# jluttine/junction-tree

Hardware: AMD Instinct MI355X
Metric: clique-potential GB/s (algorithmic bytes per propagate / time; messages/sec alongside), synthetic width-20 tree (higher is better)
Workload: dtype f32; 1 GPU; BASELINE.json configs[3]: 256 cliques, width 20, cardinality 2 (2^20-entry f32 potentials), 10 shared variables per edge, balanced binary tree; evidence_sets_per_rank=1, multiset=False, parallelism=1 GPU, launch_mode=flow, idle_plans=0, library=jtprop 0.6.0 (gfx950, HIP, RCCL p2p) src:c327fe1ab271

## Files before the change

include/jtprop.h:

```cpp
#ifndef JTPROP_H
#define JTPROP_H

#include <stddef.h>
#include <stdint.h>

#ifdef __cplusplus
extern "C" {
#endif

#define JTP_OK 0
#define JTP_EINVAL (-1)
#define JTP_EHIP (-2)
#define JTP_ECOMM (-3)
#define JTP_ENOMEM (-4)
#define JTP_EUNSUPPORTED (-5)

#define JTP_F32 0
#define JTP_F64 1

#define JTP_PLAN_ONLY 1u
#define JTP_KEEP_ROOT 4u
#define JTP_SPLIT_VARIANTS 2u

#define JTP_LEVEL_LAUNCHES 8u

#define JTP_FLOW_TICKETS 16u

#define JTP_SHARE_POTENTIALS 32u

#define JTP_MULTISET 64u

#define JTP_NO_COMPACT 128u

typedef struct jtp_plan jtp_plan;

typedef struct jtp_tree_desc {
    int32_t struct_size;
    int32_t n_vars;
    const int32_t *var_card;
    int32_t n_cliques;
    int32_t n_nodes;
    const int32_t *node_var_off;
    const int32_t *node_var_ids;
    const int32_t *parent_clique;
    const int32_t *parent_sep;
    int32_t dtype;
    int32_t device;
    int32_t n_batch;
    int32_t n_ranks;
    int32_t rank;
    const int32_t *clique_owner;
    uint32_t flags;
    int32_t lds_budget;
    int32_t block_log2;
    int32_t layout_policy;
    const int32_t *cover_off;
    const int32_t *cover_ids;
    int32_t fold_n;
    int32_t fold_pad;
    const int32_t *fold_cliques;
    const int32_t *fold_var_off;
    const int32_t *fold_var_ids;
} jtp_tree_desc;

typedef struct jtp_stats {
    int32_t struct_size;
    int32_t n_launches;
    int32_t n_messages;
    int32_t n_tasks;
    double  algorithmic_bytes;
    double  collect_ms;
    double  distribute_ms;
    double  kernel_ms[32];
    double  kernel_bytes[32];
    int32_t kernel_launches[32];
    int32_t flow_fallbacks;
    int32_t launch_mode;
    int32_t tickets_used;
    int32_t flow_propagates;
    double  device_bytes;
    int32_t storage_dtype;
    int32_t foreign_seen;
    double  f64_flops;
    double  f64_insts;
    double  algorithmic_bytes_full;
    double  fixed_bytes;
    int32_t n_unit_cliques;
    int32_t n_static_tables;
    int32_t flight_board;
    int32_t lean_refused;
} jtp_stats;


int jtp_plan_create(const jtp_tree_desc *desc, jtp_plan **out);
void jtp_plan_destroy(jtp_plan *plan);

const char *jtp_plan_describe(jtp_plan *plan);


int jtp_set_potential(jtp_plan *plan, int32_t batch, int32_t node, const void *host,
                      const int64_t *shape, int32_t host_dtype);

typedef struct jtp_factor {
    const void *host;
    int32_t n_vars;
    int32_t dtype;
    const int32_t *var_ids;
    const int64_t *shape;
} jtp_factor;

int jtp_set_potential_product(jtp_plan *plan, int32_t batch, int32_t clique, int32_t n_factors,
                              const jtp_factor *factors);

int jtp_set_potential_products(jtp_plan *plan, int32_t batch, int32_t n_cliques, const int32_t *cliques,
                               const int32_t *factor_off, const jtp_factor *factors);

int jtp_fill_synthetic(jtp_plan *plan, int32_t batch, uint64_t seed, const double *scale);

int jtp_set_evidence(jtp_plan *plan, int32_t batch, int32_t n, const int32_t *var_ids, const int32_t *states);


int jtp_propagate(jtp_plan *plan, int32_t batch_begin, int32_t batch_end);
int jtp_sync(jtp_plan *plan);


int jtp_get_belief(jtp_plan *plan, int32_t batch, int32_t node, void *host, int32_t host_dtype);

int jtp_get_marginal(jtp_plan *plan, int32_t batch, int32_t clique, const int32_t *out_vars,
                     int32_t n_out, double *host);

int jtp_get_marginals(jtp_plan *plan, int32_t batch, int32_t n, const int32_t *cliques,
                      const int32_t *var_off, const int32_t *var_ids, const int64_t *out_off,
                      double *host);

int jtp_get_z(jtp_plan *plan, int32_t batch, double *z);


int jtp_set_profiling(jtp_plan *plan, int32_t keep);
int jtp_set_profiling_granularity(jtp_plan *plan, int32_t per_launch);
int jtp_set_profiling_stride(jtp_plan *plan, int32_t stride);
int jtp_region_begin(jtp_plan *plan);
int jtp_region_end(jtp_plan *plan, double *ms);
int jtp_get_stats(jtp_plan *plan, jtp_stats *stats);
int jtp_get_launch_ms(jtp_plan *plan, double *ms, int32_t n);
int jtp_debug_read_msg(jtp_plan *plan, int32_t batch, int64_t off, int64_t n, double *host);
int jtp_debug_set(jtp_plan *plan, const char *knob, int64_t value);
const char *jtp_kernel_name(int32_t variant);


int jtp_comm_unique_id(void *id128);
int jtp_comm_init(int32_t rank, int32_t n_ranks, const void *id128, int32_t device);
int jtp_comm_destroy(void);
int jtp_comm_info(int32_t *n_ranks, int32_t *rank, int32_t *device);
int jtp_comm_selftest(int32_t n);


int jtp_device_count(int32_t *count);
int jtp_device_memory(int32_t device, uint64_t *free_bytes, uint64_t *total_bytes);

int jtp_host_alloc(void **ptr, size_t bytes);
int jtp_host_free(void *ptr);
const char *jtp_last_error(void);
const char *jtp_version(void);

#ifdef __cplusplus
}
#endif
#endif
```

junction-tree_amd/build.py:

```python
import os
import subprocess
import sys

HERE = os.path.dirname(os.path.abspath(__file__))
CSRC = os.path.join(HERE, "csrc")
LIBDIR = os.path.join(HERE, "junctiontree_amd", "lib")
LIB = os.path.join(LIBDIR, "libjtprop.so")
INST = ["jtp_inst_%s_%s.hip" % (fam, t) for fam in ("both", "bothm", "level", "mixc", "mix", "flow", "multi", "shape") for t in ("f32", "f64")]
SOURCES = ["jtp_plan.cpp", "jtp_engine.hip"] + INST
DEPS = SOURCES + ["jtp_internal.h", "jtp_plan.h", "jtp_kernels.hip.h", os.path.join("..", "..", "include", "jtprop.h")]


ID_FILE = os.path.join(LIBDIR, "BUILD_ID")


def source_id():
    import hashlib
    h = hashlib.sha256()
    for d in sorted(DEPS):
        with open(os.path.join(CSRC, d), "rb") as fh:
            h.update(d.encode() + b"\0" + fh.read())
    return h.hexdigest()[:12]


def built_id():
    try:
        with open(ID_FILE) as fh:
            return fh.read().split()[0].split("+")[0]
    except (OSError, IndexError):
        return None


def needs_build():
    if not os.path.exists(LIB):
        return True
    try:
        return built_id() != source_id()
    except OSError:
        return False


def build(force=False, verbose=True, extra=(), out=None, jobs=None):
    out = out or LIB
    if out == LIB and extra:
        raise SystemExit("experimental flags (%s) build to --out, not onto the product library" % " ".join(extra))
    if out == LIB and not force and not needs_build():
        return LIB
    from concurrent.futures import ThreadPoolExecutor
    import shutil
    import tempfile
    os.makedirs(LIBDIR, exist_ok=True)
    hipcc = os.environ.get("HIPCC", "/opt/rocm/bin/hipcc")
    sid = source_id() + ("+" + "".join(sorted(extra)).replace(" ", "") if extra else "")
    flags = ["-O3", "-std=c++17", "--offload-arch=gfx950", "-fPIC", "-Wall", "-Wno-unused-function", "-Wno-unused-variable",
             '-DJTP_SOURCE_ID="%s"' % sid] + list(extra)
    objdir = tempfile.mkdtemp(prefix="jtprop_build_")
    cache = os.path.join(LIBDIR, "objcache")
    os.makedirs(cache, exist_ok=True)
    import hashlib
    headers = {"jtp_plan.cpp": ["jtp_plan.h", "jtp_internal.h", os.path.join("..", "..", "include", "jtprop.h")],
               "jtp_engine.hip": ["jtp_plan.h", "jtp_internal.h", "jtp_kernels.hip.h", os.path.join("..", "..", "include", "jtprop.h")]}
    try:
        toolchain = subprocess.check_output([hipcc, "--version"], stderr=subprocess.STDOUT)
    except (OSError, subprocess.CalledProcessError):
        toolchain = hipcc.encode()
    try:
        def compile_one(src):
            obj = os.path.join(objdir, os.path.splitext(src)[0] + ".o")
            h = hashlib.sha256()
            h.update(toolchain)
            for d in [src] + headers.get(src, ["jtp_internal.h", "jtp_kernels.hip.h"]):
                with open(os.path.join(CSRC, d), "rb") as fh:
                    h.update(d.encode() + b"\0" + fh.read())
            tu_flags = [f for f in flags if not f.startswith("-DJTP_SOURCE_ID") or src == "jtp_engine.hip"]
            h.update(" ".join(tu_flags).encode())
            kept = os.path.join(cache, os.path.splitext(src)[0] + "." + h.hexdigest()[:16] + ".o")
            if os.path.exists(kept):
                shutil.copy(kept, obj)
                return obj
            cmd = [hipcc] + tu_flags + ["-c", os.path.join(CSRC, src), "-o", obj]
            if verbose:
                print(" ".join(cmd), flush=True)
            subprocess.check_call(cmd)
            mine = sorted((f for f in os.listdir(cache) if f.startswith(os.path.splitext(src)[0] + ".") and f.endswith(".o")),
                          key=lambda f: os.path.getmtime(os.path.join(cache, f)))
            for old in mine[:-3]:
                os.remove(os.path.join(cache, old))
            tmp_kept = kept + ".tmp%d" % os.getpid()
            shutil.copy(obj, tmp_kept)
            os.replace(tmp_kept, kept)
            return obj
# ... 34 lines not shown
```

junction-tree_amd/csrc/jtp_engine.hip:

```cpp
#include <dlfcn.h>
#include <fcntl.h>
#include <hip/hip_runtime.h>
#include <signal.h>
#include <sys/mman.h>
#include <sys/stat.h>
#include <unistd.h>

#include <cerrno>

#include <algorithm>
#include <atomic>
#include <cstdarg>
#include <cstdio>
#include <cstring>
#include <map>
#include <mutex>
#include <string>
#include <vector>

#include "jtp_kernels.hip.h"
#include "jtp_plan.h"


static thread_local std::string g_err;
// ... 74 lines not shown
typedef int (*Pop_t)(void);
static Push_t Push = nullptr;
static Pop_t Pop = nullptr;
static int state = 0;
static void load() {
    if (state != 0) return;
    state = -1;
    for (const char *n : {"librocprofiler-sdk-roctx.so.1", "librocprofiler-sdk-roctx.so", "libroctx64.so.4", "libroctx64.so"}) {
        void *h = dlopen(n, RTLD_NOW | RTLD_LOCAL);
        if (!h) continue;
        Push = (Push_t)dlsym(h, "roctxRangePushA");
        Pop = (Pop_t)dlsym(h, "roctxRangePop");
        if (Push && Pop) {
            state = 1;
            return;
        }
    }
}
struct Range {
    bool on;
    Range(bool enabled, const char *name) : on(enabled && state == 1) { if (on) Push(name); }
    ~Range() { if (on) Pop(); }
};
}

#define NCCL_TRY(expr)                                                                          \
    do {                                                                                        \
        int _r = (expr);                                                                        \
        if (_r != rccl::ncclSuccess)                                                            \
            return set_err(JTP_ECOMM, "%s failed: %s", #expr, rccl::GetErrorString(_r));         \
    } while (0)



static inline int mixk(const HostPlan &hp) { return hp.tmix ? (hp.tmix_compact ? 2 : 1) : 0; }

static bool flow_both() {
    static const bool on = !(getenv("JTP_FLOW_BOTH") && atoi(getenv("JTP_FLOW_BOTH")) == 0);
    return on;
}

template <typename T>
struct KernelTable {
    typedef void (*fn)(const JtTask *, const JtBlock *, const int *, const T *, T *, double *, JtFlow);
    static fn get(int variant, int tmix) {
        if (tmix == 2) {
            if (variant >= JT_K_COLLECT0 && variant <= JT_K_COLLECT3) return jt_collect_level_mix<T, true>;
            if (variant >= JT_K_DIST_P0C0 && variant <= JT_K_DIST_P1C3) return jt_distribute_level_mix<T, true>;
            if (variant == JT_K_COLLECT_LEVEL) return jt_collect_level_mix<T, true>;
            if (variant == JT_K_DISTRIBUTE_LEVEL) return jt_distribute_level_mix<T, true>;
            if (variant == JT_K_SINGLE || variant == JT_K_MARGINALS) return jt_single_mix<T, true>;
        }
        if (tmix) {
            if (variant >= JT_K_COLLECT0 && variant <= JT_K_COLLECT3) return jt_collect_level_mix<T, false>;
            if (variant >= JT_K_DIST_P0C0 && variant <= JT_K_DIST_P1C3) return jt_distribute_level_mix<T, false>;
            if (variant == JT_K_COLLECT_LEVEL) return jt_collect_level_mix<T, false>;
            if (variant == JT_K_DISTRIBUTE_LEVEL) return jt_distribute_level_mix<T, false>;
            if (variant == JT_K_SINGLE || variant == JT_K_MARGINALS) return jt_single_mix<T, false>;
        }
        switch (variant) {
            case JT_K_COLLECT0: return jt_collect<T, 0>;
            case JT_K_COLLECT1: return jt_collect<T, 1>;
            case JT_K_COLLECT2: return jt_collect<T, 2>;
            case JT_K_COLLECT3: return jt_collect<T, 3>;
            case JT_K_DIST_P0C0: return jt_distribute<T, 0, 0>;
            case JT_K_DIST_P0C1: return jt_distribute<T, 0, 1>;
            case JT_K_DIST_P0C2: return jt_distribute<T, 0, 2>;
            case JT_K_DIST_P0C3: return jt_distribute<T, 0, 3>;
            case JT_K_DIST_P1C0: return jt_distribute<T, 1, 0>;
            case JT_K_DIST_P1C1: return jt_distribute<T, 1, 1>;
            case JT_K_DIST_P1C2: return jt_distribute<T, 1, 2>;
            case JT_K_DIST_P1C3: return jt_distribute<T, 1, 3>;
            case JT_K_COLLECT_LEVEL: return jt_collect_level<T>;
            case JT_K_DISTRIBUTE_LEVEL: return jt_distribute_level<T>;
            case JT_K_REDUCE_LEVEL: return jt_reduce_level<T>;
            case JT_K_MULTI_COLLECT: return jt_multi_flow<T>;
            case JT_K_MULTI_DISTRIBUTE: return jt_multi_flow<T>;
            case JT_K_SINGLE: return jt_single<T>;
            case JT_K_MARGINALS: return jt_marginals<T>;
            case JT_K_LEAN_SINGLE: return jt_lean_single<T>;
        }
        return nullptr;
    }
    static fn get_flow(int phase, bool chain, int tmix, bool marg) {
        if (tmix == 2) return phase == 0 ? jt_collect_flow_mix<T, true> : jt_distribute_flow_mix<T, true>;
        if (tmix) return phase == 0 ? jt_collect_flow_mix<T, false> : jt_distribute_flow_mix<T, false>;
        if (phase == 2) return marg ? jt_propagate_flow_marg<T> : jt_propagate_flow<T>;
        if (phase == 1 && !chain && flow_both()) return marg ? jt_propagate_flow_marg<T> : jt_propagate_flow<T>;
        return phase == 0 ? jt_collect_flow<T> : (chain ? jt_distribute_flow_chain<T> : jt_distribute_flow<T>);
    }
};

static const char *k_names[JT_K_COUNT] = {
    "jt_collect<T, 0>", "jt_collect<T, 1>", "jt_collect<T, 2>", "jt_collect<T, 3>",
    "jt_distribute<T, 0, 0>", "jt_distribute<T, 0, 1>", "jt_distribute<T, 0, 2>", "jt_distribute<T, 0, 3>",
    "jt_distribute<T, 1, 0>", "jt_distribute<T, 1, 1>", "jt_distribute<T, 1, 2>", "jt_distribute<T, 1, 3>",
    "jt_collect_level<T>", "jt_distribute_level<T>", "jt_collect_flow<T>", "jt_distribute_flow<T>", "jt_reduce_level<T>",
    "jt_multi_flow<T>", "jt_multi_flow<T>", "jt_single<T>", "jt_propagate_flow<T>", "jt_marginals<T>", "jt_lean_single<T>",
};

struct BatchBuffers {
    void *psi = nullptr;
    void *bel = nullptr;
    double *msg = nullptr;
    double *fix = nullptr;
    uint32_t *ev = nullptr;
    bool ev_any = false;
    uint32_t *sync = nullptr;
    uint32_t epoch = 0;
    uint32_t flow_runs = 0;
    uint32_t ticket_runs = 0;
    bool unchecked = false;
    int64_t cur_off(int64_t half) const { return (epoch & 1u) ? half : 0; }
    int64_t fix_shift(int64_t cur) const { return fix ? (int64_t)(((intptr_t)fix - (intptr_t)msg) / 8) - cur : 0; }
};

struct MargBatch {
    int lean_nblocks = 0, lean_lds = 0;
    bool folded = false;
    JtMargDesc *d_descs_fold = nullptr;
    std::vector<JtTask> h_tasks;
    std::vector<int32_t> key;
    JtTask *d_tasks = nullptr;
    JtBlock *d_blocks = nullptr;
    int *d_itab = nullptr;
    JtMargDesc *d_descs = nullptr;
    double *scratch = nullptr, *stage = nullptr;
    int n = 0, nblocks = 0, lds = 0, max_grid_x = 1;
    int unit_nblocks = 0, unit_lds = 0;
    int64_t total_out = 0;
    std::vector<int64_t> elems;
    void release() {
        if (d_tasks) (void)hipFree(d_tasks);
        if (d_blocks) (void)hipFree(d_blocks);
        if (d_itab) (void)hipFree(d_itab);
        if (d_descs) (void)hipFree(d_descs);
        if (d_descs_fold) (void)hipFree(d_descs_fold);
        if (scratch) (void)hipFree(scratch);
        if (stage) (void)hipFree(stage);
    }
};

static std::atomic<int> g_inflight[64];

static std::map<std::pair<int, const void *>, int> g_lds_raised;
static std::mutex g_lds_mutex;
static hipError_t raise_lds(const void *func, int bytes) {
    if (bytes <= 64 * 1024) return hipSuccess;
    int dev = 0;
    hipError_t e = hipGetDevice(&dev);
    if (e != hipSuccess) return e;
    std::lock_guard<std::mutex> lock(g_lds_mutex);
    int &have = g_lds_raised[std::make_pair(dev, func)];
    if (have >= bytes) return hipSuccess;
    e = hipFuncSetAttribute(func, hipFuncAttributeMaxDynamicSharedMemorySize, bytes);
    if (e == hipSuccess) have = bytes;
    return e;
}

struct jtp_plan {
    HostPlan hp;
    bool device = false;
    bool widened = false;
    bool inflight = false;
    int launch_mode = 0;
    int tickets_used = 0;
    int foreign_seen = 0;
// ... 218 lines not shown
int jtp_device_memory(int32_t device, uint64_t *free_bytes, uint64_t *total_bytes) {
    size_t f = 0, t = 0;
    int before = 0;
    HIP_TRY(hipGetDevice(&before));
    HIP_TRY(hipSetDevice(device));
    const hipError_t e = hipMemGetInfo(&f, &t);
    (void)hipSetDevice(before);
    if (e != hipSuccess) return set_err(JTP_EHIP, "hipMemGetInfo failed: %s", hipGetErrorString(e));
    if (free_bytes) *free_bytes = f;
    if (total_bytes) *total_bytes = t;
    return JTP_OK;
}

const char *jtp_kernel_name(int32_t variant) {
    if (variant < 0 || variant >= JT_K_COUNT) return nullptr;
    return k_names[variant];
}


void jtp_plan_destroy(jtp_plan *pl) {
    if (!pl) return;
    if (pl->device) {
        (void)hipSetDevice(pl->hp.device);
        for (auto s : pl->streams) (void)hipStreamSynchronize(s);
        if (pl->inflight) {
            pl->inflight = false;
            (void)board::publish(pl->hp.device, --g_inflight[pl->hp.device & 63]);
        }
        if (pl->multiset) {
            if (!pl->bufs.empty()) {
                if (pl->bufs[0].psi) (void)hipFree(pl->bufs[0].psi);
                if (pl->bufs[0].bel) (void)hipFree(pl->bufs[0].bel);
            }
            if (pl->msg_all) (void)hipFree(pl->msg_all);
            if (pl->d_member) (void)hipFree(pl->d_member);
            if (pl->d_esum_oct) (void)hipFree(pl->d_esum_oct);
            if (pl->d_act_ids) (void)hipFree(pl->d_act_ids);
            if (pl->d_act_n) (void)hipFree(pl->d_act_n);
            if (pl->d_fanout) (void)hipFree(pl->d_fanout);
            if (pl->ev_all) (void)hipFree(pl->ev_all);
            if (pl->sync_all) (void)hipFree(pl->sync_all);
        } else
        for (auto &b : pl->bufs) {
            if (b.psi && (&b == &pl->bufs[0] || b.psi != pl->bufs[0].psi)) (void)hipFree(b.psi);
            if (b.bel) (void)hipFree(b.bel);
            if (b.msg) (void)hipFree(b.msg);
            if (b.fix && (&b == &pl->bufs[0] || b.fix != pl->bufs[0].fix)) (void)hipFree(b.fix);
            if (b.ev) (void)hipFree(b.ev);
            if (b.sync) (void)hipFree(b.sync);
        }
        if (pl->host_abort) (void)hipHostFree(pl->host_abort);
        for (auto &bt : pl->belief_tasks) {
            if (bt.d_task) (void)hipFree(bt.d_task);
            if (bt.d_blk) (void)hipFree(bt.d_blk);
            if (bt.d_tab) (void)hipFree(bt.d_tab);
        }
        for (MargBatch *mb : pl->marg_cache) {
            mb->release();
            delete mb;
        }
        if (pl->d_tasks) (void)hipFree(pl->d_tasks);
        if (pl->d_blocks) (void)hipFree(pl->d_blocks);
        for (int m = 0; m < 2; ++m)
            if (pl->d_init[m]) (void)hipFree(pl->d_init[m]);
        if (pl->d_itab) (void)hipFree(pl->d_itab);
        if (pl->stage) (void)hipFree(pl->stage);
        for (int i = 0; i < 2; ++i) {
            if (pl->up_stage[i]) (void)hipFree(pl->up_stage[i]);
            if (pl->up_ev[i]) (void)hipEventDestroy(pl->up_ev[i]);
        }
        if (pl->eval_stage) (void)hipFree(pl->eval_stage);
        if (pl->eval_host) (void)hipHostFree(pl->eval_host);
        if (pl->unit_scratch) (void)hipFree(pl->unit_scratch);
        for (auto e : pl->ev) (void)hipEventDestroy(e);
        for (auto e : pl->region_ev)
            if (e) (void)hipEventDestroy(e);
        for (auto s : pl->streams) (void)hipStreamDestroy(s);
    }
    delete pl;
}

static int zero_padding(jtp_plan *pl, double *msg, int nsets, hipStream_t s, int halves = 3);

int jtp_plan_create(const jtp_tree_desc *desc, jtp_plan **out) {
    if (!out) return set_err(JTP_EINVAL, "null output pointer");
    *out = nullptr;
    jtp_plan *pl = new jtp_plan();
    std::string err;
    int rc = jtp_build_plan(desc, pl->hp, err);
    for (int attempt = 1; attempt < 4 && rc == JTP_EUNSUPPORTED && desc; ++attempt) {
        jtp_tree_desc again = *desc;
        const bool relayout = (attempt & 1) && (desc->flags & JTP_MULTISET) && desc->layout_policy == 0;
        const bool pad = (attempt & 2) && !(desc->flags & JTP_NO_COMPACT);
        if (!relayout && !pad) continue;
        if ((attempt & 1) && !relayout) continue;
        if ((attempt & 2) && !pad) continue;
        if (relayout) again.layout_policy = 2;
        if (pad) again.flags |= JTP_NO_COMPACT;
        std::string err2;
        delete pl;
        pl = new jtp_plan();
        const int rc2 = jtp_build_plan(&again, pl->hp, err2);
        if (rc2 == JTP_OK) rc = rc2;
        else if (rc2 != JTP_EUNSUPPORTED) rc = rc2, err = err2;
    }
    if (rc == JTP_EUNSUPPORTED && desc && desc->dtype == JTP_F32 && !(desc->flags & JTP_MULTISET)) {
        for (int attempt = 0; attempt < 2 && rc == JTP_EUNSUPPORTED; ++attempt) {
            jtp_tree_desc again = *desc;
            again.dtype = JTP_F64;
            if (attempt == 1) {
                if (desc->flags & JTP_NO_COMPACT) break;
                again.flags |= JTP_NO_COMPACT;
            }
            std::string err2;
            delete pl;
            pl = new jtp_plan();
            const int rc2 = jtp_build_plan(&again, pl->hp, err2);
            if (rc2 == JTP_OK) rc = rc2, pl->widened = true;
            else if (rc2 != JTP_EUNSUPPORTED) rc = rc2, err = err2;
        }
    }
    if (rc == JTP_EUNSUPPORTED && desc && desc->cover_off && !(desc->flags & JTP_MULTISET)) {
        jtp_tree_desc again = *desc;
        again.cover_off = again.cover_ids = nullptr;
        jtp_plan *fresh = nullptr;
        const int rc2 = jtp_plan_create(&again, &fresh);
        delete pl;
        if (rc2 == JTP_OK) {
            fresh->hp.lean_refused = err.empty() ? std::string("unsupported") : err;
            *out = fresh;
        }
        return rc2;
    }
    if (rc != JTP_OK) {
        delete pl;
        return set_err(rc, "%s", err.c_str());
    }
    HostPlan &hp = pl->hp;
    pl->esize = hp.dtype == JTP_F32 ? 4 : 8;
    pl->multiset = hp.multiset;
    if (pl->multiset && !(hp.flags & JTP_SHARE_POTENTIALS)) {
        delete pl;
        return set_err(JTP_EINVAL, "JTP_MULTISET needs JTP_SHARE_POTENTIALS (the evidence sets of a group read one table)");
    }
    pl->flow = !(hp.flags & (JTP_LEVEL_LAUNCHES | JTP_SPLIT_VARIANTS)) && !(hp.knobs.debug & 1) && !hp.knobs.force_level_launches;
    if (hp.max_lds > 64 * 1024 && !pl->multiset && !hp.knobs.force_flow) pl->flow = false;
    pl->chain = hp.chain_plan;
    for (const HostPlan::FoldReq &fr : hp.folded) pl->marg_tasks = pl->marg_tasks || fr.task >= 0;
    if (hp.flags & JTP_PLAN_ONLY) {
        *out = pl;
        return JTP_OK;
    }
    pl->fake_comm = hp.n_ranks > 1 ? hp.knobs.fake_comm : 0;
    if (pl->fake_comm == 2 && (!rccl::comm || rccl::comm_size != 1)) {
        delete pl;
        return set_err(JTP_ECOMM, "JTP_FAKE_COMM=2 (exchange steps as RCCL groups in loop-back) needs a communicator of ONE rank: jtp_comm_init(0, 1, ...)");
    }
    if (hp.n_ranks > 1 && !pl->fake_comm && (!rccl::comm || rccl::comm_size != hp.n_ranks || rccl::comm_rank != hp.rank)) {
        delete pl;
        return set_err(JTP_ECOMM, "n_ranks=%d but jtp_comm_init was not called with a matching communicator", hp.n_ranks);
    }
    int ndev = 0;
    hipError_t e = hipGetDeviceCount(&ndev);
    if (e != hipSuccess || ndev <= 0) {
        delete pl;
        return set_err(JTP_EHIP, "no HIP device available (%s); libjtprop has no CPU fallback",
                       e != hipSuccess ? hipGetErrorString(e) : "device count is 0");
    }
#define CREATE_TRY(expr)                                                                                 \
    do {                                                                                                 \
        hipError_t _e = (expr);                                                                          \
        if (_e != hipSuccess) {                                                                          \
            set_err(_e == hipErrorOutOfMemory ? JTP_ENOMEM : JTP_EHIP, "%s failed: %s", #expr, hipGetErrorString(_e)); \
            jtp_plan_destroy(pl);                                                                        \
            return _e == hipErrorOutOfMemory ? JTP_ENOMEM : JTP_EHIP;                                    \
        }                                                                                                \
    } while (0)
    pl->device = true;
    pl->flow_debug = hp.knobs.flow_debug;
    pl->env_tickets = hp.knobs.flow_tickets != 0;
    pl->roctx = hp.knobs.roctx != 0;
    if (pl->roctx) roctx::load();
    CREATE_TRY(hipSetDevice(hp.device));
    const int nstreams = pl->multiset ? 1 : std::min(hp.n_batch, 16);
    pl->streams.resize(nstreams);
    for (auto &s : pl->streams) CREATE_TRY(hipStreamCreateWithFlags(&s, hipStreamNonBlocking));
    pl->bufs.resize(hp.n_batch);
    const size_t abytes = (size_t)std::max<int64_t>(hp.arena_elems, 256) * pl->esize;
    const size_t mbytes = (size_t)std::max<int64_t>(hp.msg_doubles, 2) * 8 * 2;
    const bool share_psi = (hp.flags & JTP_SHARE_POTENTIALS) != 0;
    if (pl->multiset) {
        const bool ef = hp.knobs.no_ef_share == 0 && ((hp.n_batch + JT_MSETS - 1) / JT_MSETS >= 8 || hp.knobs.no_ef_share < 0);
        pl->set0 = ef ? JT_MSETS : 0;
        pl->n_groups = (hp.n_batch + JT_MSETS - 1) / JT_MSETS + (pl->set0 ? 1 : 0);
        const size_t nsets = (size_t)pl->n_groups * JT_MSETS;
        pl->set_stride = (int64_t)(mbytes / 8);
        pl->ev_stride = (uint32_t)(2 * hp.pn.size());
        void *psi = nullptr, *bel = nullptr;
        CREATE_TRY(hipMalloc(&psi, abytes));
        pl->bufs[0].psi = psi;
        CREATE_TRY(hipMalloc(&bel, abytes));
        pl->bufs[0].bel = bel;
        CREATE_TRY(hipMemsetAsync(psi, 0, abytes, pl->streams[0]));
        CREATE_TRY(hipMemsetAsync(bel, 0, abytes, pl->streams[0]));
        CREATE_TRY(hipMalloc((void **)&pl->msg_all, mbytes * nsets));
        CREATE_TRY(hipMemsetD32Async((hipDeviceptr_t)pl->msg_all, (int)(uint32_t)(JT_UNWRITTEN & 0xffffffffu), mbytes * nsets / 4, pl->streams[0]));
        CREATE_TRY(hipMalloc((void **)&pl->ev_all, (size_t)pl->ev_stride * 4 * nsets));
        CREATE_TRY(hipMemsetAsync(pl->ev_all, 0, (size_t)pl->ev_stride * 4 * nsets, pl->streams[0]));
        CREATE_TRY(hipMalloc((void **)&pl->sync_all, (size_t)hp.sync_words * 4 * pl->n_groups));
        CREATE_TRY(hipMemsetAsync(pl->sync_all, 0, (size_t)hp.sync_words * 4 * pl->n_groups, pl->streams[0]));
        for (int b = 0; b < hp.n_batch; ++b) {
            BatchBuffers &bb = pl->bufs[b];
            bb.psi = psi;
            bb.bel = bel;
            bb.msg = pl->msg_all + (int64_t)(pl->set0 + b) * pl->set_stride;
            bb.ev = pl->ev_all + (size_t)(pl->set0 + b) * pl->ev_stride;
            bb.sync = pl->sync_all + (size_t)((pl->set0 + b) / JT_MSETS) * hp.sync_words;
        }
        pl->belief_tasks.resize(hp.pn.size());
        if (pl->set0) {
            const size_t cap = (size_t)pl->n_groups * JT_MSETS, nt = hp.tasks.size();
            CREATE_TRY(hipMalloc((void **)&pl->d_member, nt * cap));
            CREATE_TRY(hipMalloc((void **)&pl->d_act_ids, nt * cap * sizeof(uint16_t)));
            CREATE_TRY(hipMalloc((void **)&pl->d_act_n, nt * sizeof(int32_t)));
            CREATE_TRY(hipMalloc((void **)&pl->d_esum_oct, nt * (size_t)pl->n_groups));
            pl->act_dirty = true;
        }
    } else
    for (auto &b : pl->bufs) {
        if (share_psi && &b != &pl->bufs[0]) b.psi = pl->bufs[0].psi;
        else CREATE_TRY(hipMalloc(&b.psi, abytes));
        CREATE_TRY(hipMalloc(&b.bel, abytes));
        CREATE_TRY(hipMalloc((void **)&b.msg, mbytes));
        if (hp.fix_doubles > 0) {
            if (share_psi && &b != &pl->bufs[0]) b.fix = pl->bufs[0].fix;
            else {
                CREATE_TRY(hipMalloc((void **)&b.fix, (size_t)hp.fix_doubles * 8));
                CREATE_TRY(hipMemsetAsync(b.fix, 0, (size_t)hp.fix_doubles * 8, pl->streams[0]));
            }
        }
        CREATE_TRY(hipMemsetAsync(b.psi, 0, abytes, pl->streams[0]));
        CREATE_TRY(hipMemsetAsync(b.bel, 0, abytes, pl->streams[0]));
        CREATE_TRY(hipMemsetD32Async((hipDeviceptr_t)b.msg, (int)(uint32_t)(JT_UNWRITTEN & 0xffffffffu), mbytes / 4, pl->streams[0]));
        CREATE_TRY(hipMalloc((void **)&b.sync, (size_t)hp.sync_words * 4));
        CREATE_TRY(hipMemsetAsync(b.sync, 0, (size_t)hp.sync_words * 4, pl->streams[0]));
    }
    CREATE_TRY(hipHostMalloc((void **)&pl->host_abort, 64, hipHostMallocMapped));
    *pl->host_abort = 0;

    for (auto &b : pl->bufs) {
        if (&b != &pl->bufs[0] && b.psi == pl->bufs[0].psi) continue;
        for (const VirtualFill &vf : hp.virtual_fills) {
            const int64_t n = vf.d.phys_elems;
            const int grid = (int)std::min<int64_t>((n + 255) / 256, 4096);
            if (hp.dtype == JTP_F32) hipLaunchKernelGGL((jt_pack<float, float, 2>), dim3(grid), dim3(256), 0, pl->streams[0], vf.d, (const float *)nullptr, (float *)b.psi, 0ull, 1.0);
            else hipLaunchKernelGGL((jt_pack<double, double, 2>), dim3(grid), dim3(256), 0, pl->streams[0], vf.d, (const double *)nullptr, (double *)b.psi, 0ull, 1.0);
        }
        CREATE_TRY(hipGetLastError());
    }
    if (pl->multiset) {
        pl->ev_host.assign((size_t)pl->ev_stride * pl->n_groups * JT_MSETS, 0u);
        for (JtTask &tk : hp.tasks)
            if (tk.esum & 1) tk.esum |= 2, tk.esum_groups = ~0ull;
    }
    if (!hp.tasks.empty()) {
        CREATE_TRY(hipMalloc((void **)&pl->d_tasks, hp.tasks.size() * sizeof(JtTask)));
        CREATE_TRY(hipMemcpy(pl->d_tasks, hp.tasks.data(), hp.tasks.size() * sizeof(JtTask), hipMemcpyHostToDevice));
    }
    if (!hp.blocks.empty()) {
        CREATE_TRY(hipMalloc((void **)&pl->d_blocks, hp.blocks.size() * sizeof(JtBlock)));
        CREATE_TRY(hipMemcpy(pl->d_blocks, hp.blocks.data(), hp.blocks.size() * sizeof(JtBlock), hipMemcpyHostToDevice));
    }
    if (!hp.itab.empty()) {
        CREATE_TRY(hipMalloc((void **)&pl->d_itab, hp.itab.size() * sizeof(int32_t)));
        CREATE_TRY(hipMemcpy(pl->d_itab, hp.itab.data(), hp.itab.size() * sizeof(int32_t), hipMemcpyHostToDevice));
    }
    for (int m = 0; m < 2; ++m)
        if (!hp.init_blocks[m].empty()) {
            CREATE_TRY(hipMalloc((void **)&pl->d_init[m], hp.init_blocks[m].size() * sizeof(JtBlock)));
            CREATE_TRY(hipMemcpy(pl->d_init[m], hp.init_blocks[m].data(), hp.init_blocks[m].size() * sizeof(JtBlock), hipMemcpyHostToDevice));
        }
    auto kfunc = [&](int v) { return hp.dtype == JTP_F32 ? (const void *)KernelTable<float>::get(v, mixk(hp)) : (const void *)KernelTable<double>::get(v, mixk(hp)); };
    if (pl->multiset) {
        CREATE_TRY(raise_lds(kfunc(JT_K_MULTI_COLLECT), JT_RING_BYTES + JT_MSETS * (JT_MSETS > 8 ? JT_SETB_SMALL : JT_SETB_LARGE)));
    } else if (hp.max_lds > 64 * 1024) {
        for (int v = 0; v < JT_K_COUNT; ++v) {
            if (kfunc(v) == nullptr) continue;
            CREATE_TRY(raise_lds(kfunc(v), hp.max_lds));
        }
        for (int ph = 0; ph < 3; ++ph) {
            const void *f = hp.dtype == JTP_F32 ? (const void *)KernelTable<float>::get_flow(ph, pl->chain, mixk(hp), pl->marg_tasks) : (const void *)KernelTable<double>::get_flow(ph, pl->chain, mixk(hp), pl->marg_tasks);
            CREATE_TRY(raise_lds(f, hp.max_lds));
        }
    }
    {
        double b = 0;
        if (pl->multiset) {
            const size_t nsets = (size_t)pl->n_groups * JT_MSETS;
            b = 2.0 * abytes + (double)mbytes * nsets + (double)pl->ev_stride * 4 * nsets + (double)hp.sync_words * 4 * pl->n_groups;
        } else {
            const size_t npsi = share_psi ? 1 : pl->bufs.size();
            b = (double)abytes * (npsi + pl->bufs.size()) + ((double)mbytes + (double)hp.sync_words * 4) * pl->bufs.size() + (double)hp.fix_doubles * 8 * npsi;
        }
        b += (double)hp.tasks.size() * sizeof(JtTask) + (double)hp.blocks.size() * sizeof(JtBlock) + (double)hp.itab.size() * 4;
        pl->device_bytes = b;
    }
    if (pl->multiset) {
        if (int rc = zero_padding(pl, pl->msg_all, pl->n_groups * JT_MSETS, pl->streams[0])) {
            jtp_plan_destroy(pl);
            return rc;
        }
    } else
        for (auto &b : pl->bufs)
            if (int rc = zero_padding(pl, b.msg, 1, pl->streams[0])) {
                jtp_plan_destroy(pl);
                return rc;
            }
    CREATE_TRY(hipStreamSynchronize(pl->streams[0]));
#undef CREATE_TRY
    *out = pl;
    return JTP_OK;
}

const char *jtp_plan_describe(jtp_plan *pl) {
    if (!pl) return "";
    if (pl->hp.json.empty()) jtp_plan_to_json(pl->hp, pl->hp.tasks.size() <= 20000);
    return pl->hp.json.c_str();
}


static int check_writable(jtp_plan *pl, int batch) {
    if ((pl->hp.flags & JTP_SHARE_POTENTIALS) && batch != 0)
        return set_err(JTP_EINVAL, "the plan shares its potentials between evidence sets: set them through evidence set 0");
    return JTP_OK;
}

static int check_ready(jtp_plan *pl, int batch) {
    if (!pl) return set_err(JTP_EINVAL, "null plan");
    if (!pl->device) return set_err(JTP_EHIP, "plan was created with JTP_PLAN_ONLY: no device work possible");
    if (batch < 0 || batch >= pl->hp.n_batch) return set_err(JTP_EINVAL, "batch %d out of range [0,%d)", batch, pl->hp.n_batch);
    return JTP_OK;
}

int jtp_set_potential(jtp_plan *pl, int32_t batch, int32_t node, const void *host, const int64_t *shape,
                      int32_t host_dtype) {
    int rc = check_ready(pl, batch);
    if (rc) return rc;
    rc = check_writable(pl, batch);
    if (rc) return rc;
    pl->psi_dirty = true;
    HostPlan &hp = pl->hp;
    if (node < 0 || node >= hp.n_cliques) return set_err(JTP_EINVAL, "node %d is not a clique", node);
    if (!(hp.pn[node].owner == hp.rank || hp.pn[node].owner == hp.n_ranks)) return set_err(JTP_EINVAL, "clique %d belongs to rank %d", node, hp.pn[node].owner);
    if (host_dtype != JTP_F32 && host_dtype != JTP_F64) return set_err(JTP_EINVAL, "bad host dtype");
    const bool unit = hp.pn[node].unit;
    if (unit && hp.pn[node].stat < 0) {
        bool one = true;
        for (size_t i = 0; i < hp.node_vars[node].size(); ++i) one = one && (!shape || shape[i] == 1 || hp.card[hp.node_vars[node][i]] == 1);
        if (!shape) for (int v : hp.node_vars[node]) one = one && hp.card[v] == 1;
        const double v = !host ? 0.0 : (host_dtype == JTP_F32 ? (double)*(const float *)host : *(const double *)host);
        if (!one || v != 1.0)
            return set_err(JTP_EINVAL, "clique %d was described as depending on none of its variables (jtp_tree_desc.cover_*): its potential is 1", node);
        return JTP_OK;
    }
    JtPackDesc d = unit ? hp.stat_pack[node] : hp.pack[node];
    int64_t stride = 1;
    for (int i = d.nvars - 1; i >= 0; --i) {
        const int64_t len = shape ? shape[i] : d.card[i];
        if (len != d.card[i] && len != 1) {
            if (unit && len == hp.card[hp.node_vars[node][i]])
                return set_err(JTP_EINVAL, "clique %d axis %d has length %lld, but the clique was described as not depending on that variable (jtp_tree_desc.cover_*)", node, i, (long long)len);
            return set_err(JTP_EINVAL, "clique %d axis %d has length %lld, expected %d or 1", node, i, (long long)len, d.card[i]);
        }
        d.hstride[i] = (len == 1) ? 0 : stride;
        stride *= len;
    }
    const size_t hbytes = (size_t)stride * (host_dtype == JTP_F32 ? 4 : 8);
    HIP_TRY(hipSetDevice(hp.device));
    const int ui = (int)(pl->up_cursor++ & 1u);
    if (!pl->up_ev[ui]) HIP_TRY(hipEventCreateWithFlags(&pl->up_ev[ui], hipEventDisableTiming));
    if (pl->up_busy[ui]) {
        HIP_TRY(hipEventSynchronize(pl->up_ev[ui]));
        pl->up_busy[ui] = false;
    }
    if (pl->up_bytes[ui] < hbytes) {
        if (pl->up_stage[ui]) HIP_TRY(hipFree(pl->up_stage[ui]));
        pl->up_stage[ui] = nullptr;
        pl->up_bytes[ui] = 0;
        HIP_TRY(hipMalloc(&pl->up_stage[ui], std::max<size_t>(hbytes, 256)));
        pl->up_bytes[ui] = std::max<size_t>(hbytes, 256);
    }
    void *stage = pl->up_stage[ui];
    hipStream_t s = pl->streams[batch % pl->streams.size()];
    HIP_TRY(hipMemcpyAsync(stage, host, hbytes, hipMemcpyHostToDevice, s));
    BatchBuffers &b = pl->bufs[batch];
    if (unit) {
        if (host_dtype == JTP_F32) launch_pack<double, float>(d, (const float *)stage, b.fix, s);
        else launch_pack<double, double>(d, (const double *)stage, b.fix, s);
    } else if (hp.dtype == JTP_F32) {
        if (host_dtype == JTP_F32) launch_pack<float, float>(d, (const float *)stage, (float *)b.psi, s);
        else launch_pack<float, double>(d, (const double *)stage, (float *)b.psi, s);
    } else {
        if (host_dtype == JTP_F32) launch_pack<double, float>(d, (const float *)stage, (double *)b.psi, s);
        else launch_pack<double, double>(d, (const double *)stage, (double *)b.psi, s);
    }
    HIP_TRY(hipGetLastError());
    HIP_TRY(hipEventRecord(pl->up_ev[ui], s));
    pl->up_busy[ui] = true;
    return JTP_OK;
}

// ... 588 lines not shown
                hipLaunchKernelGGL(jt_multi_flow<float>, dim3(grid), dim3(JT_THREADS), lds, s, pl->d_tasks, pl->d_blocks + blk_off,
                                   pl->d_itab, (const float *)b0.psi, (float *)b0.bel, pl->msg_all, fl);
            else
                hipLaunchKernelGGL(jt_multi_flow<double>, dim3(grid), dim3(JT_THREADS), lds, s, pl->d_tasks, pl->d_blocks + blk_off,
                                   pl->d_itab, (const double *)b0.psi, (double *)b0.bel, pl->msg_all, fl);
        };
        for (const Step &st : (flow ? hp.flow_steps : hp.steps)) {
            if (st.kind != 0) continue;
            const int phase = flow ? hp.segments[st.first].phase : hp.launches[st.first].phase;
            if (prof && !mid_done && phase == 1) {
                HIP_TRY(hipEventRecord(pl->ev[ev_base + 1], s));
                mid_done = true;
            }
            if (flow) {
                const Segment &sg = hp.segments[st.first];
                int lds = 0;
                for (int i = sg.first_launch; i < sg.first_launch + sg.n_launch; ++i) lds = std::max(lds, multiset_lds(hp, hp.launches[i]));
                launch(sg.phase, sg.blk_off, sg.nblocks, lds, tickets ? sg.ticket_idx : -1, ticket_run * (uint32_t)sg.nblocks);
            } else {
                const Launch &L = hp.launches[st.first];
                launch(L.phase, L.blk_off, L.nblocks, multiset_lds(hp, L), -1, 0u);
            }
        }
        if (prof) {
            if (!mid_done) HIP_TRY(hipEventRecord(pl->ev[ev_base + 1], s));
            HIP_TRY(hipEventRecord(pl->ev[ev_base + 2], s));
            pl->prof_cursor++;
        }
        HIP_TRY(hipGetLastError());
        return JTP_OK;
    }
    const bool prof = pl->prof_steps > 0 && (pl->prof_calls++ % (unsigned)pl->prof_stride) == 0;
    const size_t ev_per_step = pl->prof_per_launch ? 2 * hp.launches.size() : 3;
    if (prof) {
        size_t need = ev_per_step * (size_t)pl->prof_steps;
        while (pl->ev.size() < need) {
            hipEvent_t e;
            HIP_TRY(hipEventCreate(&e));
            pl->ev.push_back(e);
        }
    }
    const size_t ev_base = prof ? ev_per_step * (size_t)(pl->prof_cursor % pl->prof_steps) : 0;
    for (int b = batch_begin; b < batch_end; ++b) {
        hipStream_t s = pl->streams[b % pl->streams.size()];
        BatchBuffers &bb = pl->bufs[b];
        const bool pb = prof && b == batch_begin;
        const bool per_launch = pb && pl->prof_per_launch;
        const bool per_phase = pb && !pl->prof_per_launch;
        bool mid_done = false;
        if (per_phase) HIP_TRY(hipEventRecord(pl->ev[ev_base + 0], s));
        const bool flow = pl->flow && !per_launch;
        const int64_t half = std::max<int64_t>(hp.msg_doubles, 2);
        bb.epoch++;
        JtFlow fl;
        memset(&fl, 0, sizeof fl);
        fl.sync = bb.sync;
        fl.host_abort = pl->host_abort;
        fl.cur_off = bb.cur_off(half);
        fl.oth_off = pl->flow ? half - fl.cur_off : -1;
        fl.dbg = pl->flow_debug;
        fl.ev = bb.ev_any ? bb.ev : nullptr;
        fl.fix_shift = bb.fix_shift(fl.cur_off);
        if (flow) {
            bb.flow_runs++;
            bb.unchecked = true;
        }
        const bool others = flow ? enter_flight(pl) : false;
        const bool tickets = (hp.flags & JTP_FLOW_TICKETS) != 0 || pl->streams.size() > 1 || pl->env_tickets || others;
        pl->launch_mode = flow ? (tickets ? 2 : 1) : 0;
        if (flow) pl->flow_propagates++, pl->tickets_used += tickets ? 1 : 0;
        const uint32_t ticket_run = bb.ticket_runs;
        if (flow && tickets) bb.ticket_runs++;
        for (const Step &st : (flow ? hp.flow_steps : hp.steps)) {
            if (st.kind == 0 && flow) {
                const Segment &sg = hp.segments[st.first];
                if (per_phase && !mid_done && sg.phase >= 1) {
                    HIP_TRY(hipEventRecord(pl->ev[ev_base + 1], s));
                    mid_done = true;
                }
                fl.ticket_idx = tickets ? (uint32_t)sg.ticket_idx : 0xffffffffu;
                fl.blk_base = (uint32_t)sg.blk_off;
                fl.ticket_base = ticket_run * (uint32_t)sg.nblocks;
                if (hp.dtype == JTP_F32)
                    hipLaunchKernelGGL(KernelTable<float>::get_flow(sg.phase, pl->chain, mixk(hp), pl->marg_tasks), dim3(sg.nblocks), dim3(JT_THREADS), sg.lds_bytes, s, pl->d_tasks,
                                       pl->d_blocks + sg.blk_off, pl->d_itab, (const float *)bb.psi, (float *)bb.bel, bb.msg, fl);
                else
                    hipLaunchKernelGGL(KernelTable<double>::get_flow(sg.phase, pl->chain, mixk(hp), pl->marg_tasks), dim3(sg.nblocks), dim3(JT_THREADS), sg.lds_bytes, s, pl->d_tasks,
                                       pl->d_blocks + sg.blk_off, pl->d_itab, (const double *)bb.psi, (double *)bb.bel, bb.msg, fl);
            } else if (st.kind == 0) {
                const Launch &L = hp.launches[st.first];
                if (per_phase && !mid_done && L.phase == 1) {
                    HIP_TRY(hipEventRecord(pl->ev[ev_base + 1], s));
                    mid_done = true;
                }
                if (per_launch) HIP_TRY(hipEventRecord(pl->ev[ev_base + 2 * st.first], s));
                fl.blk_base = (uint32_t)L.blk_off;
                launch_variant(pl, L.variant, L.nblocks, L.lds_bytes, s, pl->d_tasks, pl->d_blocks + L.blk_off, pl->d_itab, bb.psi, bb.bel, bb.msg, fl);
                if (per_launch) HIP_TRY(hipEventRecord(pl->ev[ev_base + 2 * st.first + 1], s));
            } else if (pl->fake_comm == 2) {
                std::vector<const CommOp *> sends, recvs;
                for (int i = st.first; i < st.first + st.count; ++i) (hp.comm[i].send ? sends : recvs).push_back(&hp.comm[i]);
                const size_t n = std::max(sends.size(), recvs.size());
                int64_t most = 0;
                for (int i = st.first; i < st.first + st.count; ++i) most = std::max(most, hp.comm[i].count);
                const int rc2 = ensure_stage(pl, (size_t)most * 8 * 2);
                if (rc2) return rc2;
                double *spare = (double *)pl->stage;
                NCCL_TRY(rccl::GroupStart());
                for (size_t k = 0; k < n; ++k) {
                    const CommOp *sd = k < sends.size() ? sends[k] : nullptr, *rv = k < recvs.size() ? recvs[k] : nullptr;
                    const int64_t cnt = rv ? rv->count : sd->count;
                    const double *src = sd && sd->count >= cnt ? bb.msg + fl.cur_off + sd->off : spare + most;
                    double *dst = rv ? bb.msg + fl.cur_off + rv->off : spare;
                    NCCL_TRY(rccl::Send(src, (size_t)cnt, rccl::ncclFloat64, rccl::comm_rank, rccl::comm, s));
                    NCCL_TRY(rccl::Recv(dst, (size_t)cnt, rccl::ncclFloat64, rccl::comm_rank, rccl::comm, s));
                }
                NCCL_TRY(rccl::GroupEnd());
            } else if (pl->fake_comm) {
                for (int i = st.first; i < st.first + st.count; ++i) {
                    const CommOp &op = hp.comm[i];
                    if (op.send) continue;
                    const int grid = (int)std::min<int64_t>((op.count + 255) / 256, 1024);
                    hipLaunchKernelGGL(jt_fill_value, dim3(grid), dim3(256), 0, s, bb.msg + fl.cur_off + op.off, op.count, 1.0);
                }
            } else {
                NCCL_TRY(rccl::GroupStart());
                for (int i = st.first; i < st.first + st.count; ++i) {
                    const CommOp &op = hp.comm[i];
                    if (op.send) NCCL_TRY(rccl::Send(bb.msg + fl.cur_off + op.off, (size_t)op.count, rccl::ncclFloat64, op.peer, rccl::comm, s));
                    else NCCL_TRY(rccl::Recv(bb.msg + fl.cur_off + op.off, (size_t)op.count, rccl::ncclFloat64, op.peer, rccl::comm, s));
                }
                NCCL_TRY(rccl::GroupEnd());
            }
        }
        if (per_phase) {
            if (!mid_done) HIP_TRY(hipEventRecord(pl->ev[ev_base + 1], s));
            HIP_TRY(hipEventRecord(pl->ev[ev_base + 2], s));
        }
        if (pb) pl->prof_cursor++;
    }
    HIP_TRY(hipGetLastError());
    return JTP_OK;
}

int jtp_sync(jtp_plan *pl) {
    if (!pl) return set_err(JTP_EINVAL, "null plan");
    if (!pl->device) return JTP_OK;
    HIP_TRY(hipSetDevice(pl->hp.device));
    for (auto s : pl->streams) HIP_TRY(hipStreamSynchronize(s));
    pl->eval_pending = false;
    pl->eval_cursor = 0;
    return check_flow(pl);
}


static bool readout_redirect(const jtp_plan *pl, int batch, JtTask &tk) {
    if (!pl->multiset || pl->set0 == 0 || pl->member_host.empty()) return false;
    const size_t cap = (size_t)pl->n_groups * JT_MSETS, slot = (size_t)(pl->set0 + batch);
    bool any = false;
    for (int k = 0; k < tk.n_in; ++k) {
        const int t = tk.msg[k].src_task;
        if (t >= 0 && !pl->member_host[(size_t)t * cap + slot]) tk.msg[k].off -= (int64_t)slot * pl->set_stride, any = true;
    }
    return any;
}

int jtp_get_belief(jtp_plan *pl, int32_t batch, int32_t node, void *host, int32_t host_dtype) {
    int rc = check_ready(pl, batch);
    if (rc) return rc;
    HostPlan &hp = pl->hp;
// ... 682 lines not shown
```

junction-tree_amd/csrc/jtp_internal.h:

```cpp
#pragma once
#include <stdint.h>

#define JT_MAX_IN 4
#define JT_MAX_OUT 3
#define JT_MAX_MSG (JT_MAX_IN + JT_MAX_OUT)
#define JT_NCOL 8
#define JT_MAX_HI 22
#define JT_MAX_BITS 31
#define JT_MAX_FREE 13
#define JT_THREADS 256
#define JT_REDUCE_ENTRIES 64
#ifndef JT_RING_BYTES
#define JT_RING_BYTES 16384
#endif
#define JT_STAGE_SCRATCH 2048
#define JT_MIN_ITER_LOG2 2
#ifndef JT_MIN_LOOP_LOG2
#define JT_MIN_LOOP_LOG2 1
#endif
#define JT_MAX_ITER_LOG2 6
#define JT_SYNC_ABORT 0
#define JT_SYNC_HDR 2
#define JT_UNWRITTEN 0x7FF8BEEF7FF8BEEFull
#define JT_MAX_VARS 32
#define JT_NO_ROW 0xFFFFFFFFu
#define JT_BLOCK_KEEP_ROWS 2u
#define JT_BLOCK_LEAN 4u
#define JT_BLOCK_FOLD 16u
#define JT_BLOCK_NULL 8u
#define JT_BLOCK_INVALID 1u
#ifndef JT_MSETS
#define JT_MSETS 8
#endif
#define JT_SETB_SMALL 4096
#define JT_SETB_LARGE 16384

struct JtMsg {
    int64_t off;
    int32_t npart;
    int32_t pstride;
    int32_t nfree;
    int32_t lds_off;
    int32_t e_w[2];
    int32_t t_w[8];
    int32_t red_e;
    int32_t red_lane;
    int32_t red_wave;
    int32_t e_dep;
    int32_t same_launch;
    int32_t fixed;
    int32_t src_task;
    int32_t pad_msg;
    int32_t f_w[JT_MAX_HI];
    int32_t f_p[JT_MAX_HI];
    uint8_t free_pos[16];
};

struct JtTask {
    int64_t psi_off;
    int64_t bel_off;
    int32_t nbits;
    int32_t nF, nA, nR;
    int32_t n_in, n_out;
    int32_t lds_bytes;
    int32_t pnode;
    int32_t real_bits;
    int32_t debug;
    int32_t kind;
    int32_t mode;
    int32_t setb;
    int32_t settle;
    int32_t esum;
    uint64_t esum_groups;
    int32_t unit;
    int32_t vgroups;
    int32_t keep_rows;
    uint32_t out_run;
    uint32_t f_x[JT_MAX_HI];
    uint32_t f_lx[JT_MAX_HI];
    uint8_t loop_pos[8];
    uint32_t first_x[8];
    int64_t itab_off;
    int32_t total;
    int32_t itab_lds;
    int64_t dbg_off;
    int64_t tmap_off;
    int32_t fold;
    int32_t pad_fold;
    int64_t lean_off;
    JtMsg msg[JT_MAX_MSG];
};

struct JtLeanMsg {
    int64_t off;
    int32_t nfree;
    int32_t lds_off;
    int32_t flags;
// ... 132 lines not shown
```

junction-tree_amd/csrc/jtp_kernels.hip.h:

```cpp
#pragma once
#include <hip/hip_runtime.h>

#include <type_traits>

#include "jtp_internal.h"

#ifndef JT_MIX_WAVES
#define JT_MIX_WAVES 4
#endif
#ifndef JT_UT
#define JT_UT 4
#endif
#ifndef JT_U
#define JT_U 4
#endif

template <typename T> struct JtVec;
template <> struct JtVec<float> { using type = float4; };
template <> struct JtVec<double> { using type = double2; };

__device__ __forceinline__ void jt_dma16(const void *gsrc, uint32_t lds_dst, bool reused = false) {
    unsigned keep;
    if (reused) {
        asm volatile("s_mov_b32 %0, m0\n\ts_mov_b32 m0, %2\n\ts_nop 0\n\tglobal_load_lds_dwordx4 %1, off\n\ts_mov_b32 m0, %0"
                     : "=&s"(keep)
                     : "v"(gsrc), "s"(lds_dst)
                     : "memory");
        return;
    }
#ifndef JT_TABLE_NO_NT
    asm volatile("s_mov_b32 %0, m0\n\ts_mov_b32 m0, %2\n\ts_nop 0\n\tglobal_load_lds_dwordx4 %1, off nt\n\ts_mov_b32 m0, %0"
                 : "=&s"(keep)
                 : "v"(gsrc), "s"(lds_dst)
                 : "memory");
    return;
#endif
    asm volatile("s_mov_b32 %0, m0\n\ts_mov_b32 m0, %2\n\ts_nop 0\n\tglobal_load_lds_dwordx4 %1, off\n\ts_mov_b32 m0, %0"
                 : "=&s"(keep)
                 : "v"(gsrc), "s"(lds_dst)
                 : "memory");
}
template <int N>
__device__ __forceinline__ void jt_wait_vmcnt() {
    asm volatile("s_waitcnt vmcnt(%0)" ::"n"(N) : "memory");
}

__device__ __forceinline__ double jt_shfl_xor(double v, int laneMask) {
    int lo = __double2loint(v), hi = __double2hiint(v);
    lo = __shfl_xor(lo, laneMask, 64);
    hi = __shfl_xor(hi, laneMask, 64);
    return __hiloint2double(hi, lo);
}

template <int N>
__device__ __forceinline__ double jt_row_down(double v) {
    int lo = __double2loint(v), hi = __double2hiint(v);
    lo = __builtin_amdgcn_update_dpp(0, lo, 0x100 + N, 0xf, 0xf, true);
    hi = __builtin_amdgcn_update_dpp(0, hi, 0x100 + N, 0xf, 0xf, true);
    return __hiloint2double(hi, lo);
}

template <int VEC>
__device__ __forceinline__ void jt_lane_sums(double (&a)[VEC], const int red_lane) {
    if (red_lane & 1) {
#pragma unroll
        for (int e = 0; e < VEC; ++e) a[e] += jt_row_down<1>(a[e]);
    }
    if (red_lane & 2) {
#pragma unroll
        for (int e = 0; e < VEC; ++e) a[e] += jt_row_down<2>(a[e]);
    }
    if (red_lane & 4) {
#pragma unroll
        for (int e = 0; e < VEC; ++e) a[e] += jt_row_down<4>(a[e]);
    }
    if (red_lane & 8) {
#pragma unroll
        for (int e = 0; e < VEC; ++e) a[e] += jt_row_down<8>(a[e]);
    }
#pragma unroll
    for (int b = 4; b < 6; ++b) {
        if ((red_lane >> b) & 1) {
            double t[VEC];
#pragma unroll
            for (int e = 0; e < VEC; ++e) t[e] = jt_shfl_xor(a[e], 1 << b);
#pragma unroll
            for (int e = 0; e < VEC; ++e) a[e] += t[e];
        }
    }
}

#define JT_NSTAMP 16
#ifdef JT_STAMPS
#define JT_STAMP_AT(slot, value) do { if ((dbg & 2) && threadIdx.x == 0) stamp_out[slot] = (double)(value); } while (0)
#else
#define JT_STAMP_AT(slot, value) do { } while (0)
#endif
#define JT_STAMP(slot) JT_STAMP_AT(slot, __builtin_amdgcn_s_memrealtime())

#define JT_FPOS(fp, b) (((fp)[(b) >> 2] >> (8 * ((b) & 3))) & 0xffu)

template <int N, typename F>
__device__ __forceinline__ void jt_static_for(F &&f) {
    if constexpr (N > 0) {
        jt_static_for<N - 1>(f);
        f(std::integral_constant<int, N - 1>{});
    }
}

__device__ __forceinline__ bool jt_unwritten(double v) { return (uint64_t)__double_as_longlong(v) == JT_UNWRITTEN; }

template <bool FLOW>
__device__ __forceinline__ double jt_msg_load(const double *p) {
    if constexpr (FLOW)
        return __longlong_as_double(__hip_atomic_load(reinterpret_cast<const long long *>(p), __ATOMIC_RELAXED, __HIP_MEMORY_SCOPE_AGENT));
    else
        return *p;
}

template <bool FLOW>
__device__ __forceinline__ double jt_msg_load(const double *p, bool through) {
    if constexpr (FLOW) return through ? jt_msg_load<true>(p) : *p;
    else return *p;
}

template <bool FLOW>
__device__ __forceinline__ void jt_msg_store(double *p, double v) {
    if constexpr (FLOW)
        __hip_atomic_store(reinterpret_cast<long long *>(p), __double_as_longlong(v), __ATOMIC_RELAXED, __HIP_MEMORY_SCOPE_AGENT);
    else
        *p = v;
}

template <bool FLOW>
__device__ __forceinline__ double jt_msg_settle(const double *p, double v, bool through, int attempt) {
#ifndef JT_NO_SETTLE
    if constexpr (FLOW) {
        if (attempt > 0 && through) {
            for (int spins = 0; spins < 24 && jt_unwritten(v); ++spins) {
                __builtin_amdgcn_s_sleep(2);
                v = jt_msg_load<true>(p);
            }
        }
    }
#endif
    return v;
}


__device__ __forceinline__ uint32_t jt_sub_lo(const uint32_t (&fp)[4], int nfree, int i) {
    uint32_t g = 0;
#pragma unroll
    for (int b = 0; b < 8; ++b)
        if (b < nfree) g += (((uint32_t)i >> b) & 1u) << JT_FPOS(fp, b);
    return g;
}
__device__ __forceinline__ uint32_t jt_sub_hi(const uint32_t (&fp)[4], int nfree, int lane) {
    uint32_t g = 0;
#pragma unroll
    for (int b = 8; b < JT_MAX_FREE; ++b)
        if (b < nfree) g += (((uint32_t)lane >> (b - 8)) & 1u) << JT_FPOS(fp, b);
    return g;
}

template <typename T, int NIN, int NOUT, int MODE, bool FLOW = false, bool EARLY_FLUSH = (MODE == 0), bool TMIX = false, bool KEEP = false, bool UNIT = false, bool BEL = !UNIT, bool VG = false>
__device__ __forceinline__ void jt_pass(const JtTask &tk, const JtBlock &bk, const int *__restrict__ itab,
                                        const T *__restrict__ psi_arena, T *__restrict__ bel_arena,
                                        double *__restrict__ msg_arena, const JtFlow &fl,
                                        uint32_t bindex, uint32_t *flow_ctl = nullptr, uint64_t t_entry = 0) {
    constexpr int VEC = 16 / sizeof(T);
    constexpr int EB = (VEC == 4) ? 2 : 1;
    constexpr int NMSG = NIN + NOUT;
    constexpr int NPAR = NIN - NOUT * (MODE == 1);
    constexpr int U = JT_U;
    constexpr int UT = TMIX ? JT_UT : U;
    static_assert((U == 4 || U == 8) && (1 << JT_MIN_ITER_LOG2) == 4 && JT_RING_BYTES == U * 4096, "the loop groups below are written out for four or eight slots");
    using VT = typename JtVec<T>::type;
    extern __shared__ __attribute__((aligned(16))) char smem[];

    const int tid = threadIdx.x;
    const int lane = tid & 63;
    const int wave = tid >> 6;
    static_assert(!VG || TMIX, "row groups are a form of mixed-radix rows");
    constexpr int ngrp = VG ? 2 : 1;
    int vt = tid, grp = 0;
    if constexpr (VG) {
        vt = (itab + tk.tmap_off + (1 << (EB + 8)))[tid & 127];
        grp = __builtin_amdgcn_readfirstlane(tid >> 7);
    }
    const int vlane = vt & 63, vwave = vt >> 6;

    const uint32_t xF = bk.xF + (uint32_t)tid * VEC;
    const T *psi = psi_arena + tk.psi_off;
    T *bel = bel_arena + (MODE == 1 ? tk.bel_off : 0);
#ifdef JT_EXPERIMENT
    const int total = (UNIT && (fl.dbg & 16)) ? U : tk.total;
#else
    const int total = tk.total;
#endif
    const int dbg = tk.debug;
#ifdef JT_STAMPS
    double *stamp_out = msg_arena + tk.dbg_off + (int64_t)(fl.blk_base + bindex) * JT_NSTAMP;
#endif
    JT_STAMP_AT(0, FLOW ? t_entry : __builtin_amdgcn_s_memrealtime());
    constexpr int NI = NIN > 0 ? NIN : 1, NO = NOUT > 0 ? NOUT : 1;
    int64_t sm_off[NI], sm_ps[NI];
    int sm_npart[NI], sm_nfree[NI], sm_lds[NI];
    bool sm_same[NI];
    uint32_t sm_fp[NI][4], sm_hiv[NI];
#pragma unroll
    for (int k = 0; k < NIN; ++k) {
        const JtMsg &m = tk.msg[k];
        const uint32_t *fpw = reinterpret_cast<const uint32_t *>(m.free_pos);
        const uint32_t fp[4] = {fpw[0], fpw[1], fpw[2], fpw[3]};
        sm_off[k] = m.off + bk.gbase[k] + (m.fixed ? fl.fix_shift : 0);
        sm_ps[k] = m.pstride;
#ifdef JT_EXPERIMENT
        sm_npart[k] = (UNIT && (fl.dbg & 32)) ? 1 : m.npart;
#else
        sm_npart[k] = m.npart;
#endif
        sm_nfree[k] = m.nfree;
        sm_lds[k] = m.lds_off;
        sm_same[k] = m.same_launch != 0;
        sm_fp[k][0] = fp[0], sm_fp[k][1] = fp[1], sm_fp[k][2] = fp[2], sm_fp[k][3] = fp[3];
        sm_hiv[k] = jt_sub_hi(fp, m.nfree, lane);
    }
    constexpr bool EARLY_OUT = EARLY_FLUSH;
    int64_t so_at[NO];
    int so_nfree[NO];
    uint32_t so_glo[NO], so_hiv[NO], so_fp[NO][4];
    uint32_t *park = flow_ctl != nullptr ? flow_ctl + 28 : nullptr;
#pragma unroll
    for (int j = 0; j < NOUT; ++j) {
        const JtMsg &m = tk.msg[JT_MAX_IN + j];
        const uint32_t *fpw = reinterpret_cast<const uint32_t *>(m.free_pos);
        const uint32_t fp[4] = {fpw[0], fpw[1], fpw[2], fpw[3]};
        const int64_t at = m.off + (int64_t)bk.pnum[j] * m.pstride + bk.gbase[JT_MAX_IN + j];
        if constexpr (EARLY_OUT) {
            so_at[j] = at;
            so_nfree[j] = m.nfree;
            so_fp[j][0] = fp[0], so_fp[j][1] = fp[1], so_fp[j][2] = fp[2], so_fp[j][3] = fp[3];
        } else if (park != nullptr && tid == 0) {
            park[8 * j + 0] = (uint32_t)at, park[8 * j + 1] = (uint32_t)((uint64_t)at >> 32), park[8 * j + 2] = (uint32_t)m.nfree;
            park[8 * j + 3] = fp[0], park[8 * j + 4] = fp[1], park[8 * j + 5] = fp[2], park[8 * j + 6] = fp[3];
        }
    }
    int rmask[NOUT > 0 ? NOUT : 1];
#pragma unroll
    for (int j = 0; j < NOUT; ++j) rmask[j] = (1 << ((tk.out_run >> (8 * j)) & 0xffu)) - 1;
    uint32_t ev_mask = 0, ev_val = 0;
    if (fl.ev != nullptr) {
        ev_mask = fl.ev[2 * tk.pnode];
        ev_val = fl.ev[2 * tk.pnode + 1];
    }
    uint32_t loop_pos[JT_MAX_ITER_LOG2];
#pragma unroll
    for (int t = 0; t < JT_MAX_ITER_LOG2; ++t) loop_pos[t] = t < tk.nA + tk.nR ? tk.loop_pos[t] : 31u;
    T *junk_row = bel_arena + ((size_t)1 << (EB + 8)) + (uint32_t)tid * VEC;
// ... 1316 lines not shown
        else jt_unit_distribute<T, false, false>(tk, bk, itab, psi, bel, msg, fl, blockIdx.x, nullptr, 0);
        return;
    }
    switch ((tk.n_in - tk.n_out) * 4 + tk.n_out) {
        case 0: jt_pass<T, 0, 0, 1>(tk, bk, itab, psi, bel, msg, fl, blockIdx.x); break;
        case 1: jt_pass<T, 1, 1, 1>(tk, bk, itab, psi, bel, msg, fl, blockIdx.x); break;
        case 2: jt_pass<T, 2, 2, 1>(tk, bk, itab, psi, bel, msg, fl, blockIdx.x); break;
        case 3: jt_pass<T, 3, 3, 1>(tk, bk, itab, psi, bel, msg, fl, blockIdx.x); break;
        case 4: jt_pass<T, 1, 0, 1>(tk, bk, itab, psi, bel, msg, fl, blockIdx.x); break;
        case 5: jt_pass<T, 2, 1, 1>(tk, bk, itab, psi, bel, msg, fl, blockIdx.x); break;
        case 6: jt_pass<T, 3, 2, 1>(tk, bk, itab, psi, bel, msg, fl, blockIdx.x); break;
        default: jt_pass<T, 4, 3, 1>(tk, bk, itab, psi, bel, msg, fl, blockIdx.x); break;
    }
}

__device__ __forceinline__ uint32_t jt_flow_ticket(const JtFlow &fl, uint32_t *flow_ctl) {
    if (fl.ticket_idx == 0xffffffffu) return blockIdx.x;
    if (threadIdx.x == 0)
        flow_ctl[0] = __hip_atomic_fetch_add(fl.sync + fl.ticket_idx, 1u, __ATOMIC_RELAXED, __HIP_MEMORY_SCOPE_AGENT) - fl.ticket_base;
    __syncthreads();
    return (uint32_t)__builtin_amdgcn_readfirstlane((int)flow_ctl[0]);
}

#ifndef JT_FLOW_WAVES
#define JT_FLOW_WAVES 4
#endif
template <typename T>
__global__ __launch_bounds__(JT_THREADS, JT_FLOW_WAVES) void jt_collect_flow(const JtTask *__restrict__ tasks,
                                                              const JtBlock *__restrict__ blk, const int *__restrict__ itab,
                                                              const T *__restrict__ psi, T *__restrict__ bel,
                                                              double *__restrict__ msg, JtFlow fl) {
    __shared__ uint32_t flow_ctl[28 + 8 * JT_MAX_OUT];
    const uint64_t t_entry = __builtin_amdgcn_s_memrealtime();
    const uint32_t ticket = jt_flow_ticket(fl, flow_ctl);
    const JtBlock &bk = blk[ticket];
    if (jt_lean_block<T>(bk, itab, msg, fl, flow_ctl)) return;
    const JtTask &tk = tasks[bk.task];
    if (tk.kind != 0) {
        jt_reduce<true>(tk, bk, msg, fl);
        return;
    }
    if (tk.unit) {
        jt_unit_collect<T, true, false>(tk, bk, itab, psi, bel, msg, fl, ticket, flow_ctl, t_entry);
        return;
    }
    switch (tk.n_in) {
        case 0: jt_pass<T, 0, 1, 0, true>(tk, bk, itab, psi, bel, msg, fl, ticket, flow_ctl, t_entry); break;
        case 1: jt_pass<T, 1, 1, 0, true>(tk, bk, itab, psi, bel, msg, fl, ticket, flow_ctl, t_entry); break;
        case 2: jt_pass<T, 2, 1, 0, true>(tk, bk, itab, psi, bel, msg, fl, ticket, flow_ctl, t_entry); break;
        default: jt_pass<T, 3, 1, 0, true>(tk, bk, itab, psi, bel, msg, fl, ticket, flow_ctl, t_entry); break;
    }
}

template <typename T, bool EARLY = false>
__device__ __forceinline__ void jt_distribute_flow_body(const JtTask *__restrict__ tasks, const JtBlock *__restrict__ blk,
                                                        const int *__restrict__ itab, const T *__restrict__ psi, T *__restrict__ bel,
                                                        double *__restrict__ msg, const JtFlow &fl, uint32_t *flow_ctl) {
    const uint64_t t_entry = __builtin_amdgcn_s_memrealtime();
    const uint32_t ticket = jt_flow_ticket(fl, flow_ctl);
    const JtBlock &bk = blk[ticket];
    if (jt_lean_block<T>(bk, itab, msg, fl, flow_ctl)) return;
    const JtTask &tk = tasks[bk.task];
    if (tk.kind != 0) {
        jt_reduce<true>(tk, bk, msg, fl);
        return;
    }
    if (tk.unit) {
        if (tk.mode == 0) jt_unit_collect<T, true, false>(tk, bk, itab, psi, bel, msg, fl, ticket, flow_ctl, t_entry);
        else jt_unit_distribute<T, true, false>(tk, bk, itab, psi, bel, msg, fl, ticket, flow_ctl, t_entry);
        return;
    }
    switch ((tk.n_in - tk.n_out) * 4 + tk.n_out) {
        case 0: jt_pass<T, 0, 0, 1, true, EARLY>(tk, bk, itab, psi, bel, msg, fl, ticket, flow_ctl, t_entry); break;
        case 1: jt_pass<T, 1, 1, 1, true, EARLY>(tk, bk, itab, psi, bel, msg, fl, ticket, flow_ctl, t_entry); break;
        case 2: jt_pass<T, 2, 2, 1, true, EARLY>(tk, bk, itab, psi, bel, msg, fl, ticket, flow_ctl, t_entry); break;
        case 3: jt_pass<T, 3, 3, 1, true, EARLY>(tk, bk, itab, psi, bel, msg, fl, ticket, flow_ctl, t_entry); break;
        case 4: jt_pass<T, 1, 0, 1, true, EARLY>(tk, bk, itab, psi, bel, msg, fl, ticket, flow_ctl, t_entry); break;
        case 5: jt_pass<T, 2, 1, 1, true, EARLY>(tk, bk, itab, psi, bel, msg, fl, ticket, flow_ctl, t_entry); break;
        case 6: jt_pass<T, 3, 2, 1, true, EARLY>(tk, bk, itab, psi, bel, msg, fl, ticket, flow_ctl, t_entry); break;
        default: jt_pass<T, 4, 3, 1, true, EARLY>(tk, bk, itab, psi, bel, msg, fl, ticket, flow_ctl, t_entry); break;
    }
}

template <typename T, bool FOLD>
__device__ __forceinline__ void jt_propagate_flow_body(const JtTask *__restrict__ tasks, const JtBlock *__restrict__ blk,
                                                       const int *__restrict__ itab, const T *__restrict__ psi, T *__restrict__ bel,
                                                       double *__restrict__ msg, const JtFlow &fl, uint32_t *flow_ctl) {
    const uint64_t t_entry = __builtin_amdgcn_s_memrealtime();
    const uint32_t ticket = jt_flow_ticket(fl, flow_ctl);
    const JtBlock &bk = blk[ticket];
    if (jt_lean_block<T, FOLD>(bk, itab, msg, fl, flow_ctl)) return;
    const JtTask &tk = tasks[bk.task];
    if (tk.kind != 0) {
        jt_reduce<true>(tk, bk, msg, fl);
        return;
    }
    if (tk.unit) {
        if (tk.mode == 0) jt_unit_collect<T, true, false>(tk, bk, itab, psi, bel, msg, fl, ticket, flow_ctl, t_entry);
        else jt_unit_distribute<T, true, false>(tk, bk, itab, psi, bel, msg, fl, ticket, flow_ctl, t_entry);
        return;
    }
    if (tk.mode == 0) {
        switch (tk.n_in) {
            case 0: jt_pass<T, 0, 1, 0, true, true, false, true>(tk, bk, itab, psi, bel, msg, fl, ticket, flow_ctl, t_entry); break;
            case 1: jt_pass<T, 1, 1, 0, true, true, false, true>(tk, bk, itab, psi, bel, msg, fl, ticket, flow_ctl, t_entry); break;
            case 2: jt_pass<T, 2, 1, 0, true, true, false, true>(tk, bk, itab, psi, bel, msg, fl, ticket, flow_ctl, t_entry); break;
            default: jt_pass<T, 3, 1, 0, true, true, false, true>(tk, bk, itab, psi, bel, msg, fl, ticket, flow_ctl, t_entry); break;
        }
        return;
    }
    switch ((tk.n_in - tk.n_out) * 4 + tk.n_out) {
        case 0: jt_pass<T, 0, 0, 1, true, false, false, true>(tk, bk, itab, psi, bel, msg, fl, ticket, flow_ctl, t_entry); break;
        case 1: jt_pass<T, 1, 1, 1, true, false, false, true>(tk, bk, itab, psi, bel, msg, fl, ticket, flow_ctl, t_entry); break;
        case 2: jt_pass<T, 2, 2, 1, true, false, false, true>(tk, bk, itab, psi, bel, msg, fl, ticket, flow_ctl, t_entry); break;
        case 3: jt_pass<T, 3, 3, 1, true, false, false, true>(tk, bk, itab, psi, bel, msg, fl, ticket, flow_ctl, t_entry); break;
        case 4: jt_pass<T, 1, 0, 1, true, false, false, true>(tk, bk, itab, psi, bel, msg, fl, ticket, flow_ctl, t_entry); break;
        case 5: jt_pass<T, 2, 1, 1, true, false, false, true>(tk, bk, itab, psi, bel, msg, fl, ticket, flow_ctl, t_entry); break;
        case 6: jt_pass<T, 3, 2, 1, true, false, false, true>(tk, bk, itab, psi, bel, msg, fl, ticket, flow_ctl, t_entry); break;
        default: jt_pass<T, 4, 3, 1, true, false, false, true>(tk, bk, itab, psi, bel, msg, fl, ticket, flow_ctl, t_entry); break;
    }
}

template <typename T>
__global__ __launch_bounds__(JT_THREADS, JT_FLOW_WAVES) void jt_propagate_flow(const JtTask *__restrict__ tasks, const JtBlock *__restrict__ blk,
                                                                   const int *__restrict__ itab, const T *__restrict__ psi,
                                                                   T *__restrict__ bel, double *__restrict__ msg, JtFlow fl) {
    __shared__ uint32_t flow_ctl[28 + 8 * JT_MAX_OUT];
    jt_propagate_flow_body<T, false>(tasks, blk, itab, psi, bel, msg, fl, flow_ctl);
}

template <typename T>
__global__ __launch_bounds__(JT_THREADS, JT_FLOW_WAVES) void jt_propagate_flow_marg(const JtTask *__restrict__ tasks, const JtBlock *__restrict__ blk,
                                                                        const int *__restrict__ itab, const T *__restrict__ psi,
                                                                        T *__restrict__ bel, double *__restrict__ msg, JtFlow fl) {
    __shared__ uint32_t flow_ctl[28 + 8 * JT_MAX_OUT];
    jt_propagate_flow_body<T, true>(tasks, blk, itab, psi, bel, msg, fl, flow_ctl);
}

template <typename T>
__global__ __launch_bounds__(JT_THREADS, JT_FLOW_WAVES) void jt_distribute_flow(const JtTask *__restrict__ tasks,
                                                                    const JtBlock *__restrict__ blk, const int *__restrict__ itab,
                                                                    const T *__restrict__ psi, T *__restrict__ bel,
                                                                    double *__restrict__ msg, JtFlow fl) {
    __shared__ uint32_t flow_ctl[28 + 8 * JT_MAX_OUT];
    jt_distribute_flow_body<T>(tasks, blk, itab, psi, bel, msg, fl, flow_ctl);
}

#ifndef JT_CHAIN_WAVES
#define JT_CHAIN_WAVES 3
#endif
template <typename T>
__global__ __launch_bounds__(JT_THREADS, JT_CHAIN_WAVES) void jt_distribute_flow_chain(const JtTask *__restrict__ tasks,
                                                                          const JtBlock *__restrict__ blk, const int *__restrict__ itab,
                                                                          const T *__restrict__ psi, T *__restrict__ bel,
                                                                          double *__restrict__ msg, JtFlow fl) {
    __shared__ uint32_t flow_ctl[28 + 8 * JT_MAX_OUT];
    #ifdef JT_CHAIN_NO_EARLY
    jt_distribute_flow_body<T, false>(tasks, blk, itab, psi, bel, msg, fl, flow_ctl);
#else
    jt_distribute_flow_body<T, true>(tasks, blk, itab, psi, bel, msg, fl, flow_ctl);
#endif
}

template <typename T, int NIN, int SETB, bool ESUM = false>
__device__ __forceinline__ void jt_mpass(const JtTask &tk, const JtBlock &bk, const int *__restrict__ itab,
                                         const T *__restrict__ psi_arena, double *__restrict__ msg0,
                                         const JtFlow &fl, uint32_t *flow_ctl, uint32_t bindex, const int sidv) {
    constexpr int G = JT_MSETS;
    constexpr int VEC = 16 / sizeof(T);
    constexpr int EB = (VEC == 4) ? 2 : 1;
    constexpr int TBITS = EB + 8;
    constexpr int U = JT_U;
    constexpr bool FLOW = true;
    using VT = typename JtVec<T>::type;
    extern __shared__ __attribute__((aligned(16))) char smem[];

    const int tid = threadIdx.x;
    const int lane = tid & 63;
    const int wave = tid >> 6;
    const uint32_t xF = bk.xF + (uint32_t)tid * VEC;
    const T *psi = psi_arena + tk.psi_off;
    const int total = tk.total;
    const int rmask = (1 << tk.nR) - 1;
    const int64_t sstride = fl.set_stride;
    int64_t soff[G];
#pragma unroll
    for (int s = 0; s < G; ++s) soff[s] = (int64_t)__builtin_amdgcn_readlane(sidv, s) * sstride;
#ifdef JT_STAMPS
    const int dbg = (fl.dbg & 0x80000000u) ? (tk.debug & ~2) : tk.debug;
    double *stamp_out = msg0 + tk.dbg_off + (int64_t)(fl.blk_base + bindex) * JT_NSTAMP;
#else
    const int dbg = tk.debug;
#endif
    JT_STAMP(0);

    const int *gtab = itab + tk.itab_off;
    const T *psi0 = psi_arena + bk.psi_x0 + (uint32_t)tid * VEC;
    const uint32_t ring_lds = (uint32_t)(uintptr_t)((__attribute__((address_space(3))) char *)smem) + (uint32_t)wave * (U * 1024);
    const char *ring = smem + wave * (U * 1024) + lane * 16;
    const T *zero_row = psi_arena + (uint32_t)tid * VEC;
    const bool chunk_ok = !(bk.flags & JT_BLOCK_INVALID);
#pragma unroll
    for (int u = 0; u < U; ++u)
        jt_dma16(bk.first_x[u] == JT_NO_ROW ? zero_row : psi0 + bk.first_x[u], __builtin_amdgcn_readfirstlane(ring_lds + u * 1024), fl.n_groups > 1);
    int trow[JT_NCOL];
    {
        const int r = lane < total ? lane : total - 1;
        const int4 a = *reinterpret_cast<const int4 *>(gtab + r * JT_NCOL);
        const int4 b = *reinterpret_cast<const int4 *>(gtab + r * JT_NCOL + 4);
        trow[0] = a.x; trow[1] = a.y; trow[2] = a.z; trow[3] = a.w;
        trow[4] = b.x; trow[5] = b.y; trow[6] = b.z; trow[7] = b.w;
    }

    JT_STAMP(1);
    uint32_t ev_m = 0, ev_v = 0;
    if (fl.ev != nullptr && lane < G) {
        ev_m = fl.ev[(size_t)sidv * fl.ev_stride + 2 * tk.pnode];
        ev_v = fl.ev[(size_t)sidv * fl.ev_stride + 2 * tk.pnode + 1];
    }
// ... 833 lines not shown
}

template <typename S>
__global__ __launch_bounds__(256) void jt_msg_unpack(JtPackDesc d, const double *__restrict__ up, int up_npart,
                                                     const double *__restrict__ dn, int dn_npart, int64_t pstride,
                                                     S *__restrict__ stage) {
    for (int64_t h = (int64_t)blockIdx.x * blockDim.x + threadIdx.x; h < d.host_elems;
         h += (int64_t)gridDim.x * blockDim.x) {
        const uint32_t x = jt_host_to_dev(d, h);
        double u = 0.0;
        for (int p = 0; p < up_npart; ++p) u += up[(int64_t)p * pstride + x];
        if (dn) {
            double w = 0.0;
            for (int p = 0; p < dn_npart; ++p) w += dn[(int64_t)p * pstride + x];
            u *= w;
        }
        stage[h] = (S)u;
    }
}

#ifndef JT_INST_TU
__global__ __launch_bounds__(256) void jt_marg_unpack(const JtMargDesc *__restrict__ descs, const double *__restrict__ scratch_buf,
                                                      double *__restrict__ stage, const double *__restrict__ arena_cur) {
    const JtMargDesc &m = descs[blockIdx.y];
    const double *scratch = m.in_arena ? arena_cur : scratch_buf;
    __shared__ double part[256];
    const int64_t ne = m.d.host_elems;
    if (ne <= 128 && gridDim.x == 1) {
        int w = 1;
        while (w < ne) w <<= 1;
        const int G = 256 / w, g = (int)threadIdx.x / w, h = (int)threadIdx.x % w;
        double u = 0.0;
        if (h < ne) {
            const uint32_t x = jt_host_to_dev(m.d, h);
            for (int p = g; p < m.npart; p += G) u += scratch[m.src_off + (int64_t)p * m.pstride + x];
        }
        part[threadIdx.x] = u;
        __syncthreads();
        if (g == 0 && h < ne) {
            double t = part[h];
            for (int k = 1; k < G; ++k) t += part[k * w + h];
            stage[m.dst_off + h] = t;
        }
        return;
    }
    for (int64_t h = (int64_t)blockIdx.x * blockDim.x + threadIdx.x; h < ne; h += (int64_t)gridDim.x * blockDim.x) {
        const uint32_t x = jt_host_to_dev(m.d, h);
        double u = 0.0;
        for (int p = 0; p < m.npart; ++p) u += scratch[m.src_off + (int64_t)p * m.pstride + x];
        stage[m.dst_off + h] = u;
    }
}
#endif

#define JT_KARGS(T) const JtTask *, const JtBlock *, const int *, const T *, T *, double *, JtFlow
#define JT_INST_FLOW(X, T)                                                   \
    X template __global__ void jt_collect_flow<T>(JT_KARGS(T));              \
    X template __global__ void jt_distribute_flow<T>(JT_KARGS(T));           \
    X template __global__ void jt_distribute_flow_chain<T>(JT_KARGS(T));
#define JT_INST_LEVEL(X, T)                                                  \
    X template __global__ void jt_collect_level<T>(JT_KARGS(T));             \
    X template __global__ void jt_distribute_level<T>(JT_KARGS(T));          \
    X template __global__ void jt_reduce_level<T>(JT_KARGS(T));              \
    X template __global__ void jt_single<T>(JT_KARGS(T));                    \
    X template __global__ void jt_lean_single<T>(JT_KARGS(T));               \
    X template __global__ void jt_marginals<T>(JT_KARGS(T));
#define JT_INST_SHAPE(X, T)                                                  \
    X template __global__ void jt_collect<T, 0>(JT_KARGS(T));                \
    X template __global__ void jt_collect<T, 1>(JT_KARGS(T));                \
    X template __global__ void jt_collect<T, 2>(JT_KARGS(T));                \
    X template __global__ void jt_collect<T, 3>(JT_KARGS(T));                \
    X template __global__ void jt_distribute<T, 0, 0>(JT_KARGS(T));          \
    X template __global__ void jt_distribute<T, 0, 1>(JT_KARGS(T));          \
    X template __global__ void jt_distribute<T, 0, 2>(JT_KARGS(T));          \
    X template __global__ void jt_distribute<T, 0, 3>(JT_KARGS(T));          \
    X template __global__ void jt_distribute<T, 1, 0>(JT_KARGS(T));          \
    X template __global__ void jt_distribute<T, 1, 1>(JT_KARGS(T));          \
    X template __global__ void jt_distribute<T, 1, 2>(JT_KARGS(T));          \
    X template __global__ void jt_distribute<T, 1, 3>(JT_KARGS(T));
#define JT_INST_MULTI(X, T) X template __global__ void jt_multi_flow<T>(JT_KARGS(T));
#define JT_INST_BOTH(X, T) JT_INST_PROPAGATE(X, T) JT_INST_PROPAGATE_MARG(X, T)
#define JT_INST_PROPAGATE(X, T) X template __global__ void jt_propagate_flow<T>(JT_KARGS(T));
#define JT_INST_PROPAGATE_MARG(X, T) X template __global__ void jt_propagate_flow_marg<T>(JT_KARGS(T));
#define JT_INST_MIX_V(X, T, V)                                                  \
    X template __global__ void jt_collect_level_mix<T, V>(JT_KARGS(T));         \
    X template __global__ void jt_distribute_level_mix<T, V>(JT_KARGS(T));      \
    X template __global__ void jt_single_mix<T, V>(JT_KARGS(T));                \
    X template __global__ void jt_collect_flow_mix<T, V>(JT_KARGS(T));          \
    X template __global__ void jt_distribute_flow_mix<T, V>(JT_KARGS(T));
#define JT_INST_MIX(X, T) JT_INST_MIX_V(X, T, false)
#define JT_INST_MIXC(X, T) JT_INST_MIX_V(X, T, true)
#ifndef JT_INST_TU
JT_INST_FLOW(extern, float)
JT_INST_FLOW(extern, double)
JT_INST_LEVEL(extern, float)
JT_INST_LEVEL(extern, double)
JT_INST_SHAPE(extern, float)
JT_INST_SHAPE(extern, double)
JT_INST_MULTI(extern, float)
JT_INST_MULTI(extern, double)
JT_INST_BOTH(extern, float)
JT_INST_BOTH(extern, double)
JT_INST_MIX(extern, float)
JT_INST_MIX(extern, double)
JT_INST_MIXC(extern, float)
JT_INST_MIXC(extern, double)
#endif
```

junction-tree_amd/csrc/jtp_plan.cpp:

```cpp
#include "jtp_plan.h"

#include <algorithm>
#include <cmath>
#include <cstdio>
#include <cstdlib>
#include <cstring>
#include <map>
#include <sstream>

namespace {

int ceil_log2(int k) {
    int b = 0;
    while ((1 << b) < k) ++b;
    return b;
}

int popc(uint32_t x) { return __builtin_popcount(x); }

struct MsgView {
    int psep = -1;
    bool up = true;
    int8_t dst[32];
    uint32_t mask = 0;
// ... 7 lines not shown
        err = _b;                                         \
        return code;                                      \
    } while (0)

int find_var(const std::vector<int> &vars, int v) {
    for (size_t i = 0; i < vars.size(); ++i)
        if (vars[i] == v) return (int)i;
    return -1;
}

MsgView make_view(const PNode &p, const PSep &s, int psep, bool up) {
    MsgView mv;
    mv.psep = psep;
    mv.up = up;
    mv.msg_bits = s.nbits;
    for (int i = 0; i < 32; ++i) mv.dst[i] = -1;
    for (size_t i = 0; i < s.vars.size(); ++i) {
        int j = find_var(p.vars, s.vars[i]);
        for (int t = 0; t < s.nb[i]; ++t) {
            mv.dst[p.pos[j] + t] = (int8_t)(s.pos[i] + t);
            mv.mask |= 1u << (p.pos[j] + t);
        }
    }
    return mv;
}

MsgView make_view(const PNode &p, const PStatic &s) {
    MsgView mv;
    mv.psep = -1;
    mv.up = true;
    mv.msg_bits = s.nbits;
    for (int i = 0; i < 32; ++i) mv.dst[i] = -1;
    for (size_t i = 0; i < s.vars.size(); ++i) {
        int j = find_var(p.vars, s.vars[i]);
        for (int t = 0; t < s.nb[i]; ++t) {
            mv.dst[p.pos[j] + t] = (int8_t)(s.pos[i] + t);
            mv.mask |= 1u << (p.pos[j] + t);
        }
    }
    return mv;
}

void order_a_bits(std::vector<int> &Ab, const std::vector<uint32_t> &outs) {
    auto klass = [&](int b) {
        uint32_t k = 0;
        for (size_t j = 0; j < outs.size(); ++j) k |= (outs[j] >> b & 1u) << j;
        return k;
    };
    int size[1 << JT_MAX_OUT] = {0};
    for (int b : Ab) ++size[klass(b)];
    std::stable_sort(Ab.begin(), Ab.end(), [&](int a, int b) {
        const uint32_t ka = klass(a), kb = klass(b);
        if (popc(ka) != popc(kb)) return popc(ka) < popc(kb);
        if (size[ka] != size[kb]) return size[ka] > size[kb];
        if (ka != kb) return ka < kb;
        return a < b;
    });
}

struct CostK {
    double wg = 1.5, stage_fix = 8.0, stage_bw = 4096.0, iter_c = 0.45, iter_d = 0.55, epi = 0.5, wave = 1.5, lane = 0.1,
           flush_fix = 1.0, flush_bw = 16384.0, bw = 5.0e6, red_fix = 4.0, red_bw = 5.0e6, overlap = 0.5, max_cu = 4, lds_cap = 150.0 * 1024;
    CostK() {
        auto g = [](const char *n, double &v) { if (const char *e = getenv(n)) v = atof(e); };
        g("JTP_COST_WG", wg), g("JTP_COST_STAGE_FIX", stage_fix), g("JTP_COST_STAGE_BW", stage_bw), g("JTP_COST_ITER_C", iter_c);
        g("JTP_COST_ITER_D", iter_d), g("JTP_COST_EPI", epi), g("JTP_COST_WAVE", wave), g("JTP_COST_LANE", lane);
        g("JTP_COST_FLUSH_FIX", flush_fix), g("JTP_COST_FLUSH_BW", flush_bw), g("JTP_COST_BW", bw), g("JTP_COST_RED_FIX", red_fix);
        g("JTP_COST_RED_BW", red_bw), g("JTP_COST_OVERLAP", overlap), g("JTP_COST_MAX_CU", max_cu), g("JTP_COST_LDS_CAP", lds_cap);
    }
};
const CostK &cost_k() {
    static const CostK k;
    return k;
}

struct CostEnv {
    int TB = 10, EB = 2, nbits = 0;
    bool dist = false;
    bool unit = false;
    int max_iter_log2 = JT_MAX_ITER_LOG2;
    double share = 1.0;
    double fill = 1.0;
    long lds_cap = 150 * 1024;
    int red_log2 = 6;
    bool chain = false;
    int min_loop_log2 = JT_MIN_ITER_LOG2;
    std::vector<uint32_t> units;
};

double task_cost_us(const CostEnv &e, const std::vector<uint32_t> &ins, const std::vector<uint32_t> &outs, uint32_t L, long *lds_out = nullptr) {
    const CostK &K = cost_k();
    const uint32_t tmask = (1u << e.TB) - 1u;
    const uint32_t himask = (e.nbits >= 32 ? ~0u : ((1u << e.nbits) - 1u)) & ~tmask;
    const uint32_t F = himask & ~L, cover = tmask | L;
    const int nL = popc(L);
    if (nL < e.min_loop_log2 || nL > e.max_iter_log2 || popc(F) > JT_MAX_HI) return 1e30;
    const double nwg = std::max(1.0, std::ldexp(e.fill, popc(F))), iters = std::ldexp(1.0, nL);
    long lds = e.unit ? 0 : JT_RING_BYTES;
    double stage = 0, flush = 0, red_bytes = 0, epi = 0;
    int n_red = 0;
    for (uint32_t m : ins) {
        const int fb = popc(m & cover);
        if (fb > JT_MAX_FREE) return 1e30;
        lds += (8L << fb) + JT_STAGE_SCRATCH;
        stage += 8.0 * (double)(1L << fb);
    }
    uint32_t allout = 0;
    for (uint32_t o : outs) allout |= o;
    std::vector<int> Ab;
    for (int b = e.TB; b < e.nbits; ++b)
        if ((L & allout) >> b & 1) Ab.push_back(b);
    if (outs.size() > 1) order_a_bits(Ab, outs);
    const int nR = popc(L & ~allout);
    const uint32_t wave_bits = 3u << (e.TB - 2), lane_bits = 63u << e.EB;
    for (uint32_t o : outs) {
        const int fb = popc(o & cover);
        if (fb > JT_MAX_FREE) return 1e30;
        lds += 8L << fb;
        flush += 8.0 * (double)(1L << fb);
        const int np = popc(F & ~o);
        if (np > 6) return 1e30;
        if (np >= e.red_log2) {
            red_bytes += (std::ldexp(1.0, np) + 1.0) * 8.0 * std::ldexp(1.0, popc(o));
            ++n_red;
        } else if (np) {
            red_bytes += std::ldexp(1.0, np) * 8.0 * std::ldexp(1.0, popc(o));
            if (e.chain) ++n_red;
        }
        int run = nR;
        for (int b : Ab) {
            if (o >> b & 1) break;
            ++run;
        }
        epi += std::ldexp(K.epi * (1.0 + K.wave * popc(~o & wave_bits)) + K.lane * popc(~o & lane_bits), nL - run);
    }
    if (lds > e.lds_cap || lds > (long)K.lds_cap) return 1e30;
    if (lds_out) *lds_out = lds;
    const double epilogues = 1.0;
    const double t_wg = K.wg + (ins.empty() ? 0.0 : K.stage_fix) + stage / K.stage_bw + iters * (e.dist ? K.iter_d : K.iter_c) + epilogues * epi +
                        (outs.empty() ? 0.0 : K.flush_fix) + flush / K.flush_bw;
    const int per_cu = (int)std::min((long)K.max_cu, std::max(1L, 160L * 1024 / (lds + 128)));
    const double conc = std::max(1.0, 256.0 * per_cu * e.share);
    const double t_lat = std::max(t_wg, nwg * t_wg / conc);
    const double bytes = nwg * (e.unit ? 0.0 : iters * 4096.0 * (e.dist ? 2.0 : 1.0)) + nwg * (0.5 * stage + flush);
    const double t_bw = bytes / (K.bw * e.share);
    double t = std::max(t_lat, t_bw) + K.overlap * std::min(t_lat, t_bw);
    if (n_red) t += K.red_fix;
    t += red_bytes / (K.red_bw * e.share);
    return t;
}

struct LoopChoice {
    uint32_t L = 0;
    double us = 1e30;
    long lds = 0;
};

LoopChoice search_loops(const CostEnv &e, const std::vector<uint32_t> &ins, const std::vector<uint32_t> &outs, bool exhaustive) {
    LoopChoice best;
    const int n = (int)e.units.size();
    auto consider = [&](uint32_t L) {
        long lds = 0;
        const double us = task_cost_us(e, ins, outs, L, &lds);
        if (us < best.us) best.L = L, best.us = us, best.lds = lds;
        return us;
    };
    if (exhaustive) {
        std::vector<std::pair<int, uint32_t>> stack;
        stack.push_back({0, 0u});
        while (!stack.empty()) {
            auto [i, L] = stack.back();
            stack.pop_back();
            if (i == n) {
                consider(L);
                continue;
            }
            stack.push_back({i + 1, L});
            if (popc(L | e.units[i]) <= e.max_iter_log2) stack.push_back({i + 1, L | e.units[i]});
        }
    } else {
        uint32_t L = 0;
        for (;;) {
            int pick = -1;
            double pick_us = 1e31;
            for (int i = 0; i < n; ++i) {
                if ((L & e.units[i]) || popc(L | e.units[i]) > e.max_iter_log2) continue;
                const double us = popc(L | e.units[i]) < e.min_loop_log2 ? 1e30 : consider(L | e.units[i]);
                double key = us;
                if (us >= 1e30) {
                    int cnt = 0;
                    for (uint32_t m : ins) cnt += (m & e.units[i]) != 0;
                    for (uint32_t o : outs) cnt += 2 * ((o & e.units[i]) != 0);
                    key = 1e30 + cnt;
                }
                if (key < pick_us) pick_us = key, pick = i;
            }
            if (pick < 0) break;
            L |= e.units[pick];
        }
    }
    return best;
}

bool high_digits_exist(const PNode &p, uint32_t x, uint32_t within) {
    if (x & within & p.pad_mask) return false;
    for (size_t g = 0; g < p.group_mask.size(); ++g) {
        if ((p.group_mask[g] & within) != p.group_mask[g]) continue;
        if ((int)((x & p.group_mask[g]) >> p.group_pos[g]) >= p.group_card[g]) return false;
    }
    return true;
}

int plan_loops(const HostPlan &hp, const PNode &p, JtTask &tk, std::vector<int32_t> &itab, int nbits, int real_bits,
               const std::vector<MsgView> &ins, const std::vector<MsgView> &outs, int block_log2, std::string &err,
               int strict_budget = 0, double share = 1.0) {
    const int TB = hp.TB;
    auto unit = [&](int b) {
        for (uint32_t g : p.group_mask)
            if (g >> b & 1) return g;
        return 1u << b;
    };
    const int budget = strict_budget > 0 ? strict_budget : (hp.lds_budget > 0 ? hp.lds_budget : 32 * 1024);
    const int PMAX_LOG2 = block_log2 <= 13 ? 6 : 3;
    const uint32_t himask = nbits >= 32 ? 0 : (((1u << nbits) - 1) & ~((1u << TB) - 1));
    uint32_t allout = 0, everyout = himask;
    for (auto &o : outs) {
        allout |= o.mask;
        everyout &= o.mask;
    }
    if (outs.empty()) everyout = 0;

    auto lds_of = [&](uint32_t F) {
        long total = 0;
        for (auto &m : ins) total += 8L << popc(m.mask & ~F);
        for (auto &m : outs) total += 8L << popc(m.mask & ~F);
        return total;
    };
    auto max_free = [&](uint32_t F) {
        int mx = 0;
        for (auto &m : ins) mx = std::max(mx, popc(m.mask & ~F));
        for (auto &m : outs) mx = std::max(mx, popc(m.mask & ~F));
        return mx;
    };
    auto part_log2 = [&](uint32_t F) {
        int mx = 0;
        for (auto &o : outs) mx = std::max(mx, popc(F & ~o.mask));
        return mx;
    };

    uint32_t F = 0;
    bool searched = false;
    if (p.layout == 4 && strict_budget == 0) {
        CostEnv e;
        e.TB = TB, e.EB = hp.EB, e.nbits = nbits, e.dist = tk.mode == 1, e.share = share, e.unit = tk.unit != 0;
        e.red_log2 = hp.knobs.reduce_min >= 0 ? std::max(0, ceil_log2(std::max(hp.knobs.reduce_min, 1))) : (hp.chain_plan ? 3 : 6);
        e.chain = hp.chain_plan;
        e.min_loop_log2 = hp.chain_plan ? JT_MIN_LOOP_LOG2 : JT_MIN_ITER_LOG2;
        e.max_iter_log2 = std::min(std::max(block_log2 - TB, JT_MIN_ITER_LOG2), JT_MAX_ITER_LOG2);
        if (hp.knobs.top_min_loop > 0 && share >= hp.knobs.top_share && !hp.chain_plan) {
            e.min_loop_log2 = std::max(e.min_loop_log2, std::min(hp.knobs.top_min_loop, nbits - TB));
            e.max_iter_log2 = std::max(e.max_iter_log2, e.min_loop_log2);
            const double lvl_rows = (double)p.phys_elems / std::max(share, 1e-9) / (double)(1 << TB);
            if (hp.knobs.top_rows2 > 0 && lvl_rows <= hp.knobs.top_rows2 && nbits - TB >= hp.knobs.top_loop2) {
                e.min_loop_log2 = std::max(hp.knobs.top_loop2, JT_MIN_LOOP_LOG2);
                e.max_iter_log2 = std::max(hp.knobs.top_loop2, JT_MIN_LOOP_LOG2);
            }
        }
        if (hp.lds_budget > 0) e.lds_cap = (tk.unit ? 0 : JT_RING_BYTES) + hp.lds_budget + JT_STAGE_SCRATCH * (long)ins.size();
        uint32_t seen = 0;
        for (int b = TB; b < nbits; ++b)
            if (!(seen >> b & 1)) e.units.push_back(unit(b)), seen |= unit(b);
        for (size_t g = 0; g < p.group_mask.size(); ++g) e.fill *= (double)p.group_card[g] / (double)(1 << popc(p.group_mask[g]));
        e.fill = std::ldexp(e.fill, -popc(p.pad_mask & himask));
        std::vector<uint32_t> im, om;
        for (auto &m : ins) im.push_back(m.mask);
        for (auto &o : outs) om.push_back(o.mask);
        LoopChoice ch = search_loops(e, im, om, true);
        if (getenv("JTP_PLAN_DEBUG") && nbits >= 24) {
            fprintf(stderr, "pnode %d mode %d nbits %d cap %d share %.3f best L %x us %.1f lds %ld\n", tk.pnode, tk.mode, nbits, e.max_iter_log2, e.share, ch.L, ch.us, ch.lds);
            for (int k = 2; k <= 6; ++k) { CostEnv e2 = e; e2.max_iter_log2 = k; LoopChoice c2 = search_loops(e2, im, om, true); fprintf(stderr, "   cap %d: L %x us %.1f lds %ld\n", k, c2.L, c2.us, c2.lds); }
        }
        if (ch.us < 1e30) F = himask & ~ch.L, searched = true;
    }
    bool down_to_four = strict_budget > 0;
    while (!searched && (lds_of(F) > budget || max_free(F) > JT_MAX_FREE)) {
        int best = -1;
        long best_lds = 0;
        int best_part = 0;
        for (int b = TB; b < nbits; ++b) {
            if (F >> b & 1) continue;
            if (nbits - popc(F | unit(b)) < TB + (down_to_four ? 2 : 3)) continue;
            long l = lds_of(F | unit(b));
            int pl = part_log2(F | unit(b));
            if (best < 0 || l < best_lds || (l == best_lds && pl < best_part)) {
                best = b, best_lds = l, best_part = pl;
            }
        }
        if (best < 0 || best_lds >= lds_of(F)) {
            if (strict_budget > 0) FAIL(JTP_EUNSUPPORTED, "message sub-boxes of one evidence set need %ld bytes of LDS (limit %d)", lds_of(F), strict_budget);
            if (lds_of(F) + (tk.unit ? 0 : JT_RING_BYTES) + JT_STAGE_SCRATCH * (long)ins.size() + 4096 <= 160 * 1024 && max_free(F) <= JT_MAX_FREE) break;
            if (!down_to_four) {
                down_to_four = true;
                continue;
            }
            FAIL(JTP_EUNSUPPORTED, "message sub-boxes do not fit in LDS (%ld bytes)", lds_of(F));
        }
        F |= unit(best);
    }
    block_log2 = std::max(block_log2, TB + JT_MIN_ITER_LOG2);
    block_log2 = std::min(block_log2, TB + JT_MAX_ITER_LOG2);
    while (!searched && nbits - popc(F) > block_log2) {
        int best = -1;
        auto fits = [&](int b) { return nbits - popc(F | unit(b)) >= TB + JT_MIN_ITER_LOG2; };
        for (int b = nbits - 1; b >= TB; --b)
            if (!(F >> b & 1) && (everyout & unit(b)) == unit(b) && fits(b)) {
                best = b;
                break;
            }
        if (best < 0) {
            int best_pl = 1 << 30, best_in = -1, best_cls = 9;
            for (int b = nbits - 1; b >= TB; --b) {
                if ((F >> b & 1) || !fits(b)) continue;
                int pl = part_log2(F | unit(b));
                int cls = (allout >> b & 1) ? 0 : 1;
                int nin = 0;
                for (auto &m : ins) nin += (m.mask >> b) & 1;
                if (cls < best_cls || (cls == best_cls && (pl < best_pl || (pl == best_pl && nin > best_in))))
                    best_cls = cls, best_pl = pl, best_in = nin, best = b;
            }
            if (best < 0) break;
            if (best_pl > PMAX_LOG2 && nbits - popc(F) <= TB + JT_MAX_ITER_LOG2) break;
        }
        F |= unit(best);
    }
    if (popc(F) > JT_MAX_HI) FAIL(JTP_EUNSUPPORTED, "too many chunk bits (%d)", popc(F));
    if (nbits - popc(F) > TB + JT_MAX_ITER_LOG2)
        FAIL(JTP_EUNSUPPORTED, "cannot split a table of %d index bits into workgroups of at most 64 rows without splitting a "
                               "variable stored at its true cardinality", nbits);

    std::vector<int> Fb, Ab, Rb;
    for (int b = TB; b < nbits; ++b) {
        if (F >> b & 1) Fb.push_back(b);
        else if (allout >> b & 1) Ab.push_back(b);
        else Rb.push_back(b);
    }
    {
        std::vector<uint32_t> om;
        for (auto &o : outs) om.push_back(o.mask);
        order_a_bits(Ab, om);
    }
    tk.nbits = nbits;
    tk.tmap_off = (hp.tmix || tk.unit) ? p.tmap_off : -1;
    tk.vgroups = (hp.tmix && !tk.unit && !p.vmap.empty()) ? 2 : 0;
    if (hp.tmix_compact && !tk.unit && tk.vgroups != 2) FAIL(JTP_EUNSUPPORTED, "internal: a task of clique %d without its list of logical threads in a compact plan", p.real);
    tk.real_bits = real_bits;
    tk.debug = hp.knobs.debug;
    tk.nF = (int)Fb.size();
    tk.nA = (int)Ab.size();
    tk.nR = (int)Rb.size();
    tk.n_in = (int)ins.size();
    tk.n_out = (int)outs.size();
    if (tk.nA > JT_MAX_HI || tk.nR > JT_MAX_HI) FAIL(JTP_EUNSUPPORTED, "too many loop bits");
    for (int j = 0; j < tk.nF; ++j) {
        tk.f_x[j] = (uint32_t)p.bitw[Fb[j]];
        tk.f_lx[j] = 1u << Fb[j];
    }
    for (int t = 0; t < tk.nR; ++t) tk.loop_pos[t] = (uint8_t)Rb[t];
    for (int t = 0; t < tk.nA; ++t) tk.loop_pos[tk.nR + t] = (uint8_t)Ab[t];
    tk.out_run = 0;
    for (size_t j = 0; j < outs.size(); ++j) {
        int run = tk.nR;
        for (int b : Ab) {
            if (outs[j].mask >> b & 1) break;
            ++run;
        }
        tk.out_run |= (uint32_t)run << (8 * j);
    }
    uint32_t loopmask = 0;
    for (int b : Rb) loopmask |= 1u << b;
    for (int b : Ab) loopmask |= 1u << b;

    int lds = tk.unit ? 0 : JT_RING_BYTES;
    std::vector<std::vector<int>> slotw;
    auto fill_msg = [&](JtMsg &jm, const MsgView &mv, bool is_out) {
        std::vector<int> sw(32, 0);
        std::vector<std::pair<int, int>> fr;
        for (int b = 0; b < nbits; ++b)
            if ((mv.mask >> b & 1) && !(F >> b & 1)) fr.push_back({mv.dst[b], b});
        std::sort(fr.begin(), fr.end());
        if (hp.knobs.lane_low > (is_out ? 1 : 0) && !hp.tmix)
            std::stable_partition(fr.begin(), fr.end(), [&](const std::pair<int, int> &x) { return x.second >= hp.EB && x.second < hp.EB + 5; });
        jm.nfree = (int)fr.size();
        jm.src_task = -1;
        for (size_t r = 0; r < fr.size(); ++r) {
            jm.free_pos[r] = (uint8_t)fr[r].first;
            sw[fr[r].second] = 1 << r;
        }
        for (int e = 0; e < 2; ++e) jm.e_w[e] = (e < hp.EB) ? sw[e] : 0;
        for (int t = 0; t < 8; ++t) jm.t_w[t] = sw[hp.EB + t];
        jm.e_dep = 0;
        for (int e = 0; e < hp.EB; ++e) jm.e_dep |= (mv.mask >> e & 1);
        jm.red_e = jm.red_lane = jm.red_wave = 0;
        if (is_out) {
            for (int e = 0; e < hp.EB; ++e) if (!(mv.mask >> e & 1)) jm.red_e |= 1 << e;
            for (int t = 0; t < 6; ++t) if (!(mv.mask >> (hp.EB + t) & 1)) jm.red_lane |= 1 << t;
            for (int t = 0; t < 2; ++t) if (!(mv.mask >> (hp.EB + 6 + t) & 1)) jm.red_wave |= 1 << t;
        }
        int pbit = 0;
        for (int j = 0; j < tk.nF; ++j) {
            int b = Fb[j];
            jm.f_w[j] = (mv.mask >> b & 1) ? (1 << mv.dst[b]) : 0;
            jm.f_p[j] = 0;
            if (is_out && !(mv.mask >> b & 1)) jm.f_p[j] = 1 << pbit++;
        }
        jm.npart = is_out ? (1 << pbit) : 1;
        jm.pstride = 1 << mv.msg_bits;
        jm.lds_off = lds;
        lds += 8 << jm.nfree;
        lds = (lds + 15) & ~15;
        slotw.push_back(sw);
    };
    for (int k = 0; k < tk.n_in; ++k) fill_msg(tk.msg[k], ins[k], false);
    for (int k = tk.n_in; k < JT_MAX_IN; ++k) slotw.push_back(std::vector<int>(32, 0));
    for (int k = 0; k < tk.n_out; ++k) fill_msg(tk.msg[JT_MAX_IN + k], outs[k], true);
    for (int k = tk.n_out; k < JT_MAX_OUT; ++k) slotw.push_back(std::vector<int>(32, 0));

    tk.total = 1 << (tk.nA + tk.nR);
    itab.assign((size_t)tk.total * JT_NCOL, 0);
    for (int i = 0; i < tk.total; ++i) {
        const int r = i & ((1 << tk.nR) - 1), a = i >> tk.nR;
        int64_t row[JT_NCOL] = {0, 0, 0, 0, 0, 0, 0, 0};
        uint32_t lx = 0;
        for (int t = 0; t < tk.nR; ++t)
            if (r >> t & 1) {
                row[0] += p.bitw[Rb[t]];
                lx |= 1u << Rb[t];
                for (int c = 1; c < JT_NCOL; ++c) row[c] += slotw[c - 1][Rb[t]];
            }
        for (int t = 0; t < tk.nA; ++t)
            if (a >> t & 1) {
                row[0] += p.bitw[Ab[t]];
                lx |= 1u << Ab[t];
                for (int c = 1; c < JT_NCOL; ++c) row[c] += slotw[c - 1][Ab[t]];
            }
        if (!high_digits_exist(p, lx, loopmask)) row[0] = (int64_t)JT_NO_ROW;
        for (int c = 0; c < JT_NCOL; ++c) itab[(size_t)i * JT_NCOL + c] = (int32_t)(uint32_t)row[c];
        if (i < 8) tk.first_x[i] = (uint32_t)row[0];
    }
    if (hp.tmix) {
        std::vector<int> live;
        for (int i = 0; i < tk.total; ++i)
            if ((uint32_t)itab[(size_t)i * JT_NCOL] != JT_NO_ROW) live.push_back(i);
        if (live.empty()) FAIL(JTP_EINVAL, "internal: a loop nest without rows");
        std::vector<int32_t> packed(live.size() * JT_NCOL);
        for (size_t r = 0; r < live.size(); ++r) {
            const int i = live[r];
            for (int c = 0; c < JT_NCOL; ++c) packed[r * JT_NCOL + c] = itab[(size_t)i * JT_NCOL + c];
            uint32_t w = (uint32_t)packed[r * JT_NCOL + 1 + JT_MAX_IN];
            if (w >= (1u << 16)) FAIL(JTP_EINVAL, "internal: sub-box offset %u does not fit 16 bits", w);
            w |= (uint32_t)i << 16;
            for (int j = 0; j < tk.n_out; ++j) {
                const int run = (tk.out_run >> (8 * j)) & 0xff;
                if (r + 1 == live.size() || (live[r + 1] >> run) != (i >> run)) w |= 1u << (24 + j);
            }
            packed[r * JT_NCOL + 1 + JT_MAX_IN] = (int32_t)w;
// ... 82 lines not shown
            ln.rmask = rmask;
            ln.red_e = mo.red_e, ln.red_lane = mo.red_lane, ln.red_wave = mo.red_wave;
            ln.out_pstride = mo.pstride;
        } else {
            fill(more.out[j - 1], mo, JT_MAX_IN + j);
            more.rmask[j - 1] = rmask;
            more.red_e[j - 1] = mo.red_e, more.red_lane[j - 1] = mo.red_lane, more.red_wave[j - 1] = mo.red_wave;
            more.out_pstride[j - 1] = mo.pstride;
        }
    }
    ln.n_in = tk.n_in;
    ln.n_out = tk.n_out;
    ln.total = tk.total;
    ln.settle = tk.settle;
    ln.tmap_off = tk.tmap_off;
    ln.itab_off = tk.itab_off;
    if (tk.tmap_off >= 0) {
        const int n_t = 1 << hp.TB;
        for (int x = 0; x < n_t; ++x)
            if (itab[(size_t)tk.tmap_off + x] < 0) ln.some_invalid = 1;
    }
    for (int i = 0; i < tk.total; ++i)
        if ((uint32_t)itab[(size_t)tk.itab_off + (size_t)i * JT_NCOL] == JT_NO_ROW) ln.some_norow = 1;
    while (itab.empty() || itab.size() % 16) itab.push_back(0);
    tk.lean_off = (int64_t)itab.size();
    const int32_t *w = reinterpret_cast<const int32_t *>(&ln);
    itab.insert(itab.end(), w, w + sizeof ln / 4);
    if (tk.n_out > 1) {
        const int32_t *w2 = reinterpret_cast<const int32_t *>(&more);
        itab.insert(itab.end(), w2, w2 + sizeof more / 4);
    }
}

PlanKnobs jtp_read_knobs() {
    PlanKnobs k;
    auto geti = [](const char *name, int dflt) { const char *v = getenv(name); return v ? atoi(v) : dflt; };
    auto getd = [](const char *name, double dflt) { const char *v = getenv(name); return v ? atof(v) : dflt; };
    k.debug = geti("JTP_DEBUG", 0);
    k.layout_policy = geti("JTP_LAYOUT_POLICY", -1);
    k.reduce_min = geti("JTP_REDUCE_MIN", -1);
    k.target_blocks_c = getd("JTP_TARGET_BLOCKS", 1024.0);
    k.target_set = getenv("JTP_TARGET_BLOCKS") != nullptr;
    k.target_blocks_d = getd("JTP_TARGET_BLOCKS_D", k.target_blocks_c);
    k.min_block_log2 = geti("JTP_MIN_BLOCK_LOG2", 13);
    k.multi_min_block_log2 = geti("JTP_MULTI_MIN_BLOCK_LOG2", 16);
    k.max_block_log2 = geti("JTP_MAX_BLOCK_LOG2", 16);
    k.max_block_log2_d = geti("JTP_MAX_BLOCK_LOG2_D", std::min(k.max_block_log2, 15));
    k.tiny_level_elems = getd("JTP_TINY_LEVEL_ELEMS", 2097152.0);
    k.force_level_launches = geti("JTP_FORCE_LEVEL_LAUNCHES", 0);
    k.force_flow = geti("JTP_FORCE_FLOW", 0);
    k.fake_comm = geti("JTP_FAKE_COMM", 0);
    k.flow_debug = (unsigned)geti("JTP_FLOW_DEBUG", 0);
    k.flow_tickets = geti("JTP_FLOW_TICKETS", 0);
    k.no_compact = geti("JTP_NO_COMPACT", 0);
    k.no_search = geti("JTP_NO_SEARCH", 0);
    k.search_all = geti("JTP_SEARCH_ALL", 1);
    k.roctx = geti("JTP_ROCTX", 0);
    k.merge_phases = geti("JTP_MERGE_PHASES", -1);
    k.no_tmix = geti("JTP_NO_TMIX", 0);
    k.tmix_fill = getd("JTP_TMIX_FILL", 0.6);
    k.no_tsplit = geti("JTP_NO_TSPLIT", 0);
    k.settle_level_elems = getd("JTP_SETTLE_LEVEL_ELEMS", 8388608.0);
    k.top_min_loop = geti("JTP_TOP_MIN_LOOP", 3);
    k.lane_low = geti("JTP_LANE_LOW", 2);
    k.longest_first = geti("JTP_LONGEST_FIRST", 1);
    k.top_share = getd("JTP_TOP_SHARE", 0.12);
    k.top_rows2 = getd("JTP_TOP_ROWS2", 2048.0);
    k.top_loop2 = geti("JTP_TOP_LOOP2", 2);
    k.keep_rows_mb = getd("JTP_KEEP_ROWS_MB", 128.0);
    k.esum_always = geti("JTP_EXPERIMENT_ESUM_ALWAYS", 0);
    k.marg_group = std::max(1, std::min(geti("JTP_MARG_GROUP", JT_MAX_OUT), JT_MAX_OUT));
    k.marg_block_log2 = geti("JTP_MARG_BLOCK_LOG2", 0);
    k.no_unit = geti("JTP_NO_UNIT", 0);
    k.keep_invalid = geti("JTP_KEEP_INVALID", 0);
    k.no_vgroups = geti("JTP_NO_VGROUPS", 0);
    k.unit_joint_down = geti("JTP_UNIT_JOINT_DOWN", 0);
    k.no_ef_share = geti("JTP_EF_SHARE", 0) ? -1 : geti("JTP_NO_EF_SHARE", 0);
    k.unit_ratio = getd("JTP_UNIT_RATIO", 4.0);
    k.no_lean = geti("JTP_NO_LEAN", 0);
    k.no_fold = geti("JTP_NO_FOLD", 0);
    k.fold = geti("JTP_FOLD", -1);
    if (k.fold == 0) k.no_fold = 1;
    k.fold_slots = geti("JTP_FOLD_SLOTS", 1024);
    return k;
}

struct PlanBuilder {
    const jtp_tree_desc *d;
    HostPlan &hp;
    std::string &err;
    int N = 0, NP = 0, esize = 4, ALL = 1, maxdepth = 0;
    std::vector<std::vector<double>> lvl_elems[2];
    std::vector<double> task_bytes;

    PlanBuilder(const jtp_tree_desc *desc, HostPlan &plan, std::string &e) : d(desc), hp(plan), err(e) {}
    bool mine(int pnode) const { return hp.pn[pnode].owner == hp.rank || hp.pn[pnode].owner == ALL; }
    double host_elems(const std::vector<int> &vars) const {
        double e = 1;
        for (int v : vars) e *= hp.card[v];
        return e;
    }
    int block_log2_for(int phase, int level, int owner, bool tiny_rule = true) const;
    int read_description();
    int link_nodes();
    int fold_marginals();
    int reroot();
    int decide_units();
    int binarise();
    int depths();
    int layouts();
    bool searched_order(int c, const std::vector<int> &host, const std::vector<int> &seps, std::vector<int> &order);
    bool wants_static(const PNode &p) const { return p.unit && p.real >= 0 && !p.cover.empty(); }
    int arenas();
    int level_work();
    int make_tasks();
    int messages();
    int schedule();
    int finish();
    int run() {
        int (PlanBuilder::*stages[])() = {&PlanBuilder::read_description, &PlanBuilder::link_nodes, &PlanBuilder::reroot,
                                          &PlanBuilder::decide_units, &PlanBuilder::binarise, &PlanBuilder::depths, &PlanBuilder::layouts,
                                          &PlanBuilder::arenas, &PlanBuilder::level_work, &PlanBuilder::make_tasks,
                                          &PlanBuilder::messages, &PlanBuilder::schedule, &PlanBuilder::finish};
        for (auto stage : stages) {
            const int rc = (this->*stage)();
            if (rc != JTP_OK) return rc;
        }
        return JTP_OK;
    }
};

int PlanBuilder::block_log2_for(int phase, int level, int owner, bool tiny_rule) const {
        if (hp.block_log2 > 0) return std::max(hp.block_log2, hp.TB);
        const double target = (phase == 0 ? hp.knobs.target_blocks_c : hp.knobs.target_blocks_d) * (hp.unit_dominated && !hp.knobs.target_set ? 2.0 : 1.0);
        const int lgmin = hp.multiset && hp.n_batch > JT_MSETS ? hp.knobs.multi_min_block_log2 : hp.knobs.min_block_log2;
        const int lgmax = phase == 1 && !hp.multiset ? hp.knobs.max_block_log2_d : hp.knobs.max_block_log2;
        const double tiny = hp.knobs.tiny_level_elems;
        if (tiny_rule && lvl_elems[phase][owner][level] <= tiny) return hp.TB + JT_MIN_ITER_LOG2;
        double want = lvl_elems[phase][owner][level] / target;
        int lg = lgmin;
        while (lg < lgmax && (double)(1 << (lg + 1)) <= want) ++lg;
        return std::max(lg, hp.TB);
    }

int PlanBuilder::read_description() {
    if (!d) FAIL(JTP_EINVAL, "null description");
    hp.knobs = jtp_read_knobs();
    if (d->struct_size != (int32_t)sizeof(jtp_tree_desc))
        FAIL(JTP_EINVAL, "jtp_tree_desc size mismatch (%d vs %zu)", d->struct_size, sizeof(jtp_tree_desc));
    if (d->n_cliques < 1 || d->n_vars < 0) FAIL(JTP_EINVAL, "empty tree");
    if (d->n_nodes != 2 * d->n_cliques - 1)
        FAIL(JTP_EINVAL, "n_nodes must be 2*n_cliques-1 (got %d for %d cliques)", d->n_nodes, d->n_cliques);
    if (d->dtype != JTP_F32 && d->dtype != JTP_F64) FAIL(JTP_EINVAL, "bad dtype %d", d->dtype);
    if (d->n_batch < 1) FAIL(JTP_EINVAL, "n_batch must be >= 1");
    if (d->n_ranks < 1 || d->rank < 0 || d->rank >= d->n_ranks) FAIL(JTP_EINVAL, "bad rank %d/%d", d->rank, d->n_ranks);

    hp.n_vars = d->n_vars;
    hp.n_cliques = d->n_cliques;
    hp.n_nodes = d->n_nodes;
    hp.dtype = d->dtype;
    hp.n_ranks = d->n_ranks;
    hp.rank = d->rank;
    hp.n_batch = d->n_batch;
    hp.device = d->device;
    hp.flags = d->flags;
    hp.lds_budget = d->lds_budget;
    hp.block_log2 = d->block_log2;
    hp.layout_policy = d->layout_policy;
    if (hp.knobs.layout_policy >= 0) hp.layout_policy = hp.knobs.layout_policy;
    hp.compact = !hp.knobs.no_compact && !(d->flags & JTP_NO_COMPACT);
    hp.multiset = (d->flags & JTP_MULTISET) != 0;
    if (hp.multiset) {
        if (d->n_ranks != 1) FAIL(JTP_EUNSUPPORTED, "multi-set plans run on one rank (evidence sets are independent: give every rank its own sets)");
        if (hp.layout_policy == 0) hp.layout_policy = 3;
    }
    hp.VEC = d->dtype == JTP_F32 ? 4 : 2;
    hp.EB = d->dtype == JTP_F32 ? 2 : 1;
    hp.TB = hp.EB + 8;
    N = d->n_cliques;
    esize = d->dtype == JTP_F32 ? 4 : 8;

    if ((d->n_vars > 0 && !d->var_card) || !d->node_var_off || !d->parent_clique || !d->parent_sep)
        FAIL(JTP_EINVAL, "null array in the description");
    hp.card.assign(d->var_card, d->var_card + d->n_vars);
    hp.vbits.resize(d->n_vars);
    for (int v = 0; v < d->n_vars; ++v) {
        if (hp.card[v] < 1) FAIL(JTP_EINVAL, "variable %d has cardinality %d", v, hp.card[v]);
        if (hp.card[v] > (1 << 28)) FAIL(JTP_EUNSUPPORTED, "variable %d has cardinality %d (max 2^28)", v, hp.card[v]);
        hp.vbits[v] = ceil_log2(hp.card[v]);
    }
    hp.node_vars.resize(d->n_nodes);
    if (d->node_var_off[0] != 0) FAIL(JTP_EINVAL, "node_var_off[0] must be 0 (got %d)", d->node_var_off[0]);
    if (d->node_var_off[d->n_nodes] > 0 && !d->node_var_ids) FAIL(JTP_EINVAL, "null array in the description");
    for (int n = 0; n < d->n_nodes; ++n) {
        int a = d->node_var_off[n], b = d->node_var_off[n + 1];
        if (a < 0 || b < a) FAIL(JTP_EINVAL, "node_var_off decreases at node %d (%d, %d)", n, a, b);
        if (b - a > JT_MAX_VARS) FAIL(JTP_EUNSUPPORTED, "node %d has %d variables (max %d)", n, b - a, JT_MAX_VARS);
        for (int i = a; i < b; ++i) {
            int v = d->node_var_ids[i];
            if (v < 0 || v >= d->n_vars) FAIL(JTP_EINVAL, "node %d: unknown variable %d", n, v);
            if (find_var(hp.node_vars[n], v) >= 0) FAIL(JTP_EINVAL, "node %d: variable %d listed twice", n, v);
            hp.node_vars[n].push_back(v);
        }
    }
    if (d->fold_n < 0 || (d->fold_n > 0 && (!d->fold_cliques || !d->fold_var_off))) FAIL(JTP_EINVAL, "null array in the description (fold_*)");
    if (d->fold_n > 0) {
        if (d->fold_var_off[0] != 0) FAIL(JTP_EINVAL, "fold_var_off[0] must be 0");
        for (int i = 0; i < d->fold_n; ++i) {
            const int c = d->fold_cliques[i], a = d->fold_var_off[i], b = d->fold_var_off[i + 1];
            if (c < 0 || c >= N) FAIL(JTP_EINVAL, "fold request %d: node %d is not a clique", i, c);
            if (b < a || b - a > JT_MAX_VARS || (b > a && !d->fold_var_ids)) FAIL(JTP_EINVAL, "fold request %d: bad variable list", i);
            for (int k = a; k < b; ++k)
                if (d->fold_var_ids[k] < 0 || d->fold_var_ids[k] >= hp.n_vars) FAIL(JTP_EINVAL, "fold request %d: variable %d out of range", i, d->fold_var_ids[k]);
        }
        hp.fold_cliques.assign(d->fold_cliques, d->fold_cliques + d->fold_n);
        hp.fold_var_off.assign(d->fold_var_off, d->fold_var_off + d->fold_n + 1);
        hp.fold_var_ids.assign(d->fold_var_ids, d->fold_var_ids + d->fold_var_off[d->fold_n]);
// ... 191 lines not shown

    return JTP_OK;
}

int PlanBuilder::depths() {
    maxdepth = 0;
    {
        std::vector<int> q{hp.root};
        hp.pn[hp.root].depth = 0;
        for (size_t i = 0; i < q.size(); ++i)
            for (int k : hp.pn[q[i]].children) {
                hp.pn[k].depth = hp.pn[q[i]].depth + 1;
                maxdepth = std::max(maxdepth, hp.pn[k].depth);
                q.push_back(k);
            }
    }

    return JTP_OK;
}

bool PlanBuilder::searched_order(int c, const std::vector<int> &host, const std::vector<int> &seps, std::vector<int> &order) {
    const PNode &p = hp.pn[c];
    const int n = (int)host.size(), TB = hp.TB;
    if (n == 0 || n > 31) return false;
    std::vector<int> cnt(n, 0), canon(n), rank_of(n);
    const bool has_static = wants_static(p);
    for (int i = 0; i < n; ++i) {
        for (int sp : seps) cnt[i] += find_var(hp.ps[sp].vars, host[i]) >= 0;
        if (has_static) cnt[i] += find_var(p.cover, host[i]) >= 0;
        canon[i] = i;
    }
    auto waste = [&](int i) { return (double)(1 << hp.vbits[host[i]]) / hp.card[host[i]]; };
    std::stable_sort(canon.begin(), canon.end(), [&](int a, int b) { return cnt[a] != cnt[b] ? cnt[a] < cnt[b] : waste(a) < waste(b); });
    for (int r = 0; r < n; ++r) rank_of[canon[r]] = r;
    int total_bits = 0;
    for (int v : host) total_bits += hp.vbits[v];
    if (total_bits <= TB || total_bits > JT_MAX_BITS) return false;
    auto bits_of = [&](uint32_t S) {
        int b = 0;
        for (int i = 0; i < n; ++i)
            if (S >> i & 1) b += hp.vbits[host[i]];
        return b;
    };
    auto valid = [&](uint32_t S) {
        if (!S) return false;
        int last = -1;
        for (int r = n - 1; r >= 0 && last < 0; --r)
            if (S >> canon[r] & 1) last = canon[r];
        const int b = bits_of(S);
        return b >= TB && b - hp.vbits[host[last]] < TB;
    };
    struct Eval { double us = 1e30; uint32_t Ld = 0, Lc = 0; };
    std::vector<int> idx;
    auto order_of = [&](uint32_t S) {
        idx.clear();
        for (int r = 0; r < n; ++r) if (S >> canon[r] & 1) idx.push_back(canon[r]);
        for (int r = 0; r < n; ++r) if (!(S >> canon[r] & 1)) idx.push_back(canon[r]);
    };
    std::vector<int> pos(n);
    auto evaluate = [&](uint32_t S) {
        Eval ev;
        order_of(S);
        int bit = 0;
        for (int i : idx) pos[i] = bit, bit += hp.vbits[host[i]];
        CostEnv e;
        e.TB = TB, e.EB = hp.EB, e.nbits = std::max(bit, TB + JT_MIN_ITER_LOG2);
        e.unit = p.unit;
        e.red_log2 = hp.knobs.reduce_min >= 0 ? std::max(0, ceil_log2(std::max(hp.knobs.reduce_min, 1))) : (hp.chain_plan ? 3 : 6);
        e.chain = hp.chain_plan;
        e.min_loop_log2 = hp.chain_plan ? JT_MIN_LOOP_LOG2 : JT_MIN_ITER_LOG2;
        uint32_t grouped = 0;
        for (int i : idx) {
            const int card = hp.card[host[i]], nb = hp.vbits[host[i]];
            if (pos[i] >= TB && (hp.compact || p.unit) && (card & (card - 1)) != 0) {
                const uint32_t g = ((1u << nb) - 1u) << pos[i];
                e.units.push_back(g), grouped |= g;
                e.fill *= (double)card / (double)(1 << nb);
            }
        }
        for (int b = TB; b < e.nbits; ++b)
            if (!(grouped >> b & 1)) e.units.push_back(1u << b);
        if (hp.compact || p.unit) e.fill = std::ldexp(e.fill, -(e.nbits - std::max(bit, TB)));
        std::sort(e.units.begin(), e.units.end());
        if (hp.lds_budget > 0) e.lds_cap = (p.unit ? 0 : JT_RING_BYTES) + hp.lds_budget + JT_STAGE_SCRATCH * 4L;
        uint32_t stat_mask = 0;
        if (has_static)
            for (int v : p.cover) {
                const int i = find_var(host, v);
                if (i >= 0) stat_mask |= ((1u << hp.vbits[v]) - 1u) << pos[i];
            }
        auto mask_of = [&](int sp) {
            uint32_t m = 0;
            for (int v : hp.ps[sp].vars) {
                const int i = find_var(host, v);
                if (i >= 0) m |= ((1u << hp.vbits[v]) - 1u) << pos[i];
            }
            return m;
        };
        std::vector<uint32_t> kids, none;
        for (int k : p.children) kids.push_back(mask_of(hp.pn[k].psep));
        const double elems = std::ldexp(1.0, e.nbits);
        ev.us = 0;
        if (c != hp.root && p.psep >= 0) {
            e.dist = false;
            e.max_iter_log2 = std::min(std::max(block_log2_for(0, p.depth, p.owner, false) - TB, JT_MIN_ITER_LOG2), JT_MAX_ITER_LOG2);
            e.share = std::min(1.0, elems / std::max(elems, lvl_elems[0][p.owner][p.depth]));
            std::vector<uint32_t> cin = kids;
            if (has_static) cin.push_back(stat_mask);
            LoopChoice ch = search_loops(e, cin, {mask_of(p.psep)}, false);
            ev.us += ch.us, ev.Lc = ch.L;
        }
        {
            e.dist = true;
            e.max_iter_log2 = std::min(std::max(block_log2_for(1, p.depth, p.owner, false) - TB, JT_MIN_ITER_LOG2), JT_MAX_ITER_LOG2);
            e.share = std::min(1.0, elems / std::max(elems, lvl_elems[1][p.owner][p.depth]));
            std::vector<uint32_t> ins;
            if (p.psep >= 0) ins.push_back(mask_of(p.psep));
            if (has_static) ins.push_back(stat_mask);
            ins.insert(ins.end(), kids.begin(), kids.end());
            LoopChoice ch = search_loops(e, ins, kids, false);
            ev.us += ch.us, ev.Ld = ch.L;
        }
        return ev;
    };
    uint32_t bestS = 0;
    Eval best;
    if (n <= 12) {
        for (uint32_t S = 1; S < (1u << n); ++S) {
            if (!valid(S)) continue;
            Eval ev = evaluate(S);
            if (ev.us < best.us) best = ev, bestS = S;
        }
    } else {
        uint32_t S = 0;
        for (int r = 0; r < n && bits_of(S) < TB; ++r) S |= 1u << canon[r];
        best = evaluate(S), bestS = S;
        for (int pass = 0; pass < 4; ++pass) {
            bool better = false;
            for (int i = 0; i < n; ++i) {
                if (!(bestS >> i & 1)) continue;
                for (int j = 0; j < n; ++j) {
                    if (bestS >> j & 1) continue;
                    const uint32_t S2 = (bestS & ~(1u << i)) | (1u << j);
                    if (!valid(S2)) continue;
                    Eval ev = evaluate(S2);
                    if (ev.us < best.us) {
                        best = ev, bestS = S2, better = true;
                        break;
                    }
                }
            }
            if (!better) break;
        }
    }
    if (best.us >= 1e30) return false;
    order_of(bestS);
    int bit = 0;
    for (int i : idx) pos[i] = bit, bit += hp.vbits[host[i]];
    auto klass = [&](int i) {
        const uint32_t m = ((1u << hp.vbits[host[i]]) - 1u) << pos[i];
        if (pos[i] < TB) return 0;
        return (m & best.Ld) ? 1 : (m & best.Lc) ? 2 : 3;
    };
    std::vector<int> fin = idx;
    std::stable_sort(fin.begin(), fin.end(), [&](int a, int b) { return klass(a) < klass(b); });
    order.clear();
    for (int i : fin) order.push_back(host[i]);
    return true;
}

int PlanBuilder::layouts() {
    for (int ph = 0; ph < 2; ++ph) lvl_elems[ph].assign(hp.n_ranks + 1, std::vector<double>(maxdepth + 1, 0.0));
    for (int c = 0; c < NP; ++c) {
        const PNode &p = hp.pn[c];
        int cb = 0;
        for (int v : (p.real >= 0 ? hp.node_vars[p.real] : p.vars)) cb += hp.vbits[v];
        const double e = std::ldexp(1.0, std::max(cb, hp.TB + JT_MIN_ITER_LOG2));
        if (c != hp.root) lvl_elems[0][p.owner][p.depth] += e;
        lvl_elems[1][p.owner][p.depth] += e;
    }
    {
        int tiny = 0;
        for (int c = 0; c < NP; ++c) tiny += lvl_elems[1][hp.pn[c].owner][hp.pn[c].depth] <= hp.knobs.tiny_level_elems;
        hp.chain_plan = 2 * tiny > NP;
    }
    for (int c = 0; c < NP; ++c) {
        PNode &p = hp.pn[c];
        std::vector<int> host = p.real >= 0 ? hp.node_vars[p.real] : p.vars;
        std::vector<int> seps;
        if (p.psep >= 0) seps.push_back(p.psep);
        for (int k : p.children) seps.push_back(hp.pn[k].psep);
        std::vector<int> order;
        int policy = hp.layout_policy;
        if (policy == 0 && !seps.empty()) {
            double msg_bytes = 0;
            for (int sp : seps) {
                int sb = 0;
                for (int v : hp.ps[sp].vars) sb += hp.vbits[v];
                msg_bytes += 8.0 * (double)((int64_t)1 << sb);
            }
            if (wants_static(p)) {
                int sb = 0;
                for (int v : p.cover) sb += hp.vbits[v];
                msg_bytes += 8.0 * (double)((int64_t)1 << sb);
            }
            int cb = 0;
            for (int v : host) cb += hp.vbits[v];
            const double r = msg_bytes / ((double)((int64_t)1 << std::max(cb, hp.TB + JT_MIN_ITER_LOG2)) * esize);
            const double thr = (double)cb / std::max<size_t>(host.size(), 1) >= 2.0 ? 0.04 : 0.12;
            policy = (r >= thr || (p.children.size() <= 1 && r >= 0.01)) ? 2 : 3;
            if ((policy == 2 || hp.knobs.search_all) && !hp.multiset && !hp.knobs.no_search) policy = 4;
        }
        if (policy == 4 && (seps.empty() || !searched_order(c, host, seps, order))) policy = 2, order.clear();
        p.layout = policy;
        if (policy == 4) {
        } else if (policy == 1 || seps.empty()) {
            order.assign(host.rbegin(), host.rend());
        } else if (policy == 2) {
            std::vector<std::pair<int, int>> keyed;
            for (size_t i = 0; i < host.size(); ++i) {
                int cnt = 0;
                for (int sp : seps) cnt += find_var(hp.ps[sp].vars, host[i]) >= 0;
                keyed.push_back({cnt, (int)i});
            }
            auto waste = [&](int i) { return (double)(1 << hp.vbits[host[i]]) / hp.card[host[i]]; };
            std::stable_sort(keyed.begin(), keyed.end(), [&](const std::pair<int, int> &a, const std::pair<int, int> &b) {
                return a.first != b.first ? a.first < b.first : waste(a.second) < waste(b.second);
            });
            for (auto &kv : keyed) order.push_back(host[kv.second]);
        } else {
            int nchild = (int)p.children.size();
            std::vector<int> priv, ponly, part, allc;
            int n_full = 0;
            for (size_t i = 0; i < host.size(); ++i) {
                int v = host[i];
                int in_parent = p.psep >= 0 && find_var(hp.ps[p.psep].vars, v) >= 0;
                int in_child = 0;
                for (int k : p.children) in_child += find_var(hp.ps[hp.pn[k].psep].vars, v) >= 0;
                if (!in_parent && !in_child) priv.push_back(v);
                else if ((nchild > 0 && in_child == nchild) || nchild == 0) {
                    if (in_parent && nchild > 0) allc.insert(allc.begin() + n_full++, v);
                    else allc.push_back(v);
                } else if (in_child == 0) ponly.push_back(v);
                else part.push_back(v);
            }
            for (std::vector<int> *cls : {&priv, &ponly, &part})
                std::stable_sort(cls->begin(), cls->end(), [&](int a, int b) {
                    return (double)(1 << hp.vbits[a]) / hp.card[a] < (double)(1 << hp.vbits[b]) / hp.card[b];
                });
            auto take = [&](std::vector<int> &from, int want_bits) {
                int got = 0;
                while (!from.empty() && got < want_bits) {
                    int v = from.front();
                    from.erase(from.begin());
                    order.push_back(v);
                    got += hp.vbits[v];
                }
                return got;
            };
            auto bits_of = [&](const std::vector<int> &l) {
                int b = 0;
                for (int v : l) b += hp.vbits[v];
                return b;
            };
            int got = take(priv, hp.EB);
            if (got < hp.EB) got += take(part, hp.EB - got);
            if (got < hp.EB) got += take(allc, hp.EB - got);
            if (got < hp.EB) got += take(ponly, hp.EB - got);
// ... 838 lines not shown
        for (int t : tasks)
            for (uint32_t f = 0; f < (1u << hp.tasks[t].nF); ++f) {
                hp.blocks.push_back(jtp_make_block(hp, hp.tasks[t], (uint32_t)t, f));
                hp.block_chunk.push_back(f);
            }
        pad_launch(L);
        L.nblocks = (int)(hp.blocks.size() - L.blk_off);
        Step st;
        st.kind = 0;
        st.first = (int)hp.launches.size();
        st.count = 1;
        hp.launches.push_back(L);
        hp.steps.push_back(st);
    };
    auto cut_children = [&](int child_level) {
        std::vector<int> v;
        for (int k : by_level(child_level)) {
            const PNode &ch = hp.pn[k];
            if (ch.parent >= 0 && hp.pn[ch.parent].owner != ch.owner) v.push_back(k);
        }
        return v;
    };
    for (int level = maxdepth; level >= 0; --level) {
        for (int k : cut_children(level + 1)) {
            const int po = hp.pn[hp.pn[k].parent].owner;
            if (hp.pn[k].owner != hp.rank && (po == hp.rank || po == ALL)) comm_op(0, hp.pn[k].psep, 1, hp.pn[k].owner);
        }
        if (level >= 1) {
            emit_launches(0, level);
            emit_reduce(0, level);
        }
        for (int c : cut_children(level)) {
            if (hp.pn[c].owner != hp.rank) continue;
            const int po = hp.pn[hp.pn[c].parent].owner;
            if (po == ALL) {
                for (int peer = 0; peer < hp.n_ranks; ++peer)
                    if (peer != hp.rank) comm_op(1, hp.pn[c].psep, 1, peer);
            } else comm_op(1, hp.pn[c].psep, 1, po);
        }
    }
    for (int level = 0; level <= maxdepth; ++level) {
        for (int c : cut_children(level)) {
            const int po = hp.pn[hp.pn[c].parent].owner;
            if (hp.pn[c].owner == hp.rank && po != ALL) comm_op(0, hp.pn[c].psep, 0, po);
        }
        emit_launches(1, level);
        emit_reduce(1, level);
        for (int k : cut_children(level + 1)) {
            const int po = hp.pn[hp.pn[k].parent].owner;
            if (po == hp.rank && hp.pn[k].owner != hp.rank) comm_op(1, hp.pn[k].psep, 0, hp.pn[k].owner);
        }
    }
    flush_comm();
    return JTP_OK;
}

int PlanBuilder::finish() {
    for (const Step &st : hp.steps) {
        if (st.kind == 1) {
            hp.flow_steps.push_back(st);
            continue;
        }
        const Launch &L = hp.launches[st.first];
        const bool extend = !hp.flow_steps.empty() && hp.flow_steps.back().kind == 0 && hp.segments.back().phase == L.phase;
        if (!extend) {
            Segment sg;
            sg.phase = L.phase;
            sg.first_launch = st.first;
            sg.blk_off = L.blk_off;
            sg.ticket_idx = JT_SYNC_HDR + (int)hp.segments.size();
            Step fs;
            fs.kind = 0;
            fs.first = (int)hp.segments.size();
            fs.count = 1;
            hp.segments.push_back(sg);
            hp.flow_steps.push_back(fs);
        }
        Segment &sg = hp.segments.back();
        sg.n_launch++;
        sg.nblocks += L.nblocks;
        sg.lds_bytes = std::max(sg.lds_bytes, L.lds_bytes);
    }
    {
        const bool merge = hp.knobs.merge_phases == 1 ||
                           (hp.knobs.merge_phases < 0 && !hp.multiset && !hp.chain_plan && !hp.tmix &&
                            (hp.staging_bytes * 8.0 <= hp.table_bytes || hp.unit_dominated));
        if (merge && !hp.multiset && !hp.tmix) {
            std::vector<Segment> segs;
            std::vector<Step> fsteps;
            for (const Step &st : hp.flow_steps) {
                if (st.kind == 0 && !fsteps.empty() && fsteps.back().kind == 0 && segs.back().phase == 0 && hp.segments[st.first].phase == 1) {
                    const Segment &b = hp.segments[st.first];
                    Segment &a = segs.back();
                    a.phase = 2;
                    a.n_launch += b.n_launch;
                    a.nblocks += b.nblocks;
                    a.lds_bytes = std::max(a.lds_bytes, b.lds_bytes);
                    continue;
                }
                Step fs = st;
                if (st.kind == 0) {
                    fs.first = (int)segs.size();
                    segs.push_back(hp.segments[st.first]);
                    segs.back().ticket_idx = JT_SYNC_HDR + (int)segs.size() - 1;
                }
                fsteps.push_back(fs);
            }
            hp.segments = segs;
            hp.flow_steps = fsteps;
        }
    }
    {
        std::vector<int> seg_of(hp.tasks.size(), -1);
        for (size_t g = 0; g < hp.segments.size(); ++g)
            for (int i = hp.segments[g].first_launch; i < hp.segments[g].first_launch + hp.segments[g].n_launch; ++i)
                for (int t : hp.launches[i].tasks) seg_of[t] = (int)g;
        for (size_t t = 0; t < hp.tasks.size(); ++t) {
            JtTask &tk = hp.tasks[t];
            const std::vector<int> &prod = hp.task_producers[t];
            for (int k = 0; k < tk.n_in && k < (int)prod.size(); ++k)
                tk.msg[k].same_launch = (prod[k] >= 0 && seg_of[t] >= 0 && seg_of[prod[k]] == seg_of[t]) ? 1 : 0;
        }
    }
    hp.sync_words = JT_SYNC_HDR + (int)hp.segments.size();
    if (hp.knobs.debug & 2) {
        hp.dbg_base = hp.msg_doubles;
        hp.msg_doubles += ((int64_t)hp.blocks.size() + 1) * 16;
        for (const Launch &L : hp.launches)
            for (int t : L.tasks) hp.tasks[t].dbg_off = hp.dbg_base;
    }
    hp.n_messages = 0;
    for (int c = 0; c < N; ++c)
        if (c != hp.root && (hp.owner[c] == hp.rank || (hp.owner[c] == ALL && hp.rank == 0))) hp.n_messages += 2;
    for (JtTask &tk : hp.tasks) jtp_make_lean(hp, tk, hp.itab, tk.fold != 0);
    for (HostPlan::FoldReq &fr : hp.folded)
        if (fr.task >= 0 && hp.tasks[fr.task].lean_off <= 0) fr.task = -1;
    for (JtBlock &b : hp.blocks) {
        const int64_t at = hp.tasks[b.task].lean_off;
        if (hp.tasks[b.task].fold) b.flags |= JT_BLOCK_FOLD;
        if (at > 0) b.flags |= JT_BLOCK_LEAN, b.first_x[5] = (uint32_t)hp.tasks[b.task].pnode, b.first_x[6] = (uint32_t)at, b.first_x[7] = (uint32_t)((uint64_t)at >> 32);
    }
    return JTP_OK;
}

int jtp_build_plan(const jtp_tree_desc *d, HostPlan &hp, std::string &err) {
    return PlanBuilder(d, hp, err).run();
}


static void neighbour_inputs(const HostPlan &hp, const PNode &p, std::vector<MsgView> &ins, std::vector<std::pair<int64_t, int>> &src,
                             std::vector<int> &from) {
    if (p.psep >= 0) {
        ins.push_back(make_view(p, hp.ps[p.psep], p.psep, false));
        src.push_back({hp.ps[p.psep].dn_roff, hp.ps[p.psep].dn_rnpart});
        from.push_back(-1);
    }
    if (p.stat >= 0) {
        ins.push_back(make_view(p, hp.statics[p.stat]));
        src.push_back({hp.statics[p.stat].off, -1});
        from.push_back(-1);
    }
    for (int k : p.children) {
        const PSep &sp = hp.ps[hp.pn[k].psep];
        ins.push_back(make_view(p, sp, hp.pn[k].psep, true));
        src.push_back({sp.up_roff, sp.up_rnpart});
        from.push_back(hp.pn[k].collect_task);
    }
}

int jtp_plan_marginal_task(const HostPlan &hp, int pnode, const std::vector<std::vector<int>> &out_vars,
                           JtTask &tk, std::vector<int32_t> &itab, std::vector<int> &out_bits, std::vector<int> &npart,
                           std::vector<JtBlock> &blocks, std::string &err, bool with_neighbours) {
    const PNode &p = hp.pn[pnode];
    if (out_vars.empty() || (int)out_vars.size() > JT_MAX_OUT) FAIL(JTP_EINVAL, "internal: %zu marginals in one task", out_vars.size());
    if (with_neighbours && out_vars.size() != 1 && !p.unit) FAIL(JTP_EINVAL, "internal: several marginals in one task of a multi-set plan");
    if (p.unit && !with_neighbours) FAIL(JTP_EINVAL, "internal: a unit clique keeps no belief table to marginalise");
    std::vector<PSep> seps(out_vars.size());
    out_bits.clear();
    for (size_t j = 0; j < out_vars.size(); ++j) {
        PSep &s = seps[j];
        s.vars.assign(out_vars[j].rbegin(), out_vars[j].rend());
        int bit = 0;
        for (int v : s.vars) {
            if (find_var(p.vars, v) < 0) FAIL(JTP_EINVAL, "variable %d is not in clique %d", v, p.real);
            s.pos.push_back(bit);
            s.nb.push_back(hp.vbits[v]);
            bit += hp.vbits[v];
        }
        s.nbits = bit;
        if (bit > 28) FAIL(JTP_EUNSUPPORTED, "marginal with %d index bits", bit);
        out_bits.push_back(bit);
    }
    memset(&tk, 0, sizeof tk);
    tk.pnode = pnode;
    tk.psi_off = p.unit ? 0 : p.arena_off;
    tk.bel_off = -1;
    tk.unit = p.unit ? 1 : 0;
    tk.mode = 0;
    std::vector<MsgView> ins, outs;
    std::vector<std::pair<int64_t, int>> src;
    std::vector<int> from;
    if (with_neighbours) neighbour_inputs(hp, p, ins, src, from);
    if ((int)ins.size() > JT_MAX_IN) FAIL(JTP_EUNSUPPORTED, "clique with %zu neighbours", ins.size());
    for (const PSep &s : seps) outs.push_back(make_view(p, s, -1, true));
    int real_bits = 0;
    for (int nb : p.nb) real_bits += nb;
    int rc = plan_loops(hp, p, tk, itab, p.nbits, real_bits, ins, outs, with_neighbours ? 14 : (hp.knobs.marg_block_log2 > 0 ? hp.knobs.marg_block_log2 : hp.TB + JT_MAX_ITER_LOG2), err);
    tk.itab_off = 0;
    if (rc != JTP_OK) return rc;
    if (hp.tmix || p.unit) {
        tk.tmap_off = (int64_t)itab.size();
        itab.insert(itab.end(), p.tmap.begin(), p.tmap.end());
        itab.insert(itab.end(), p.vmap.begin(), p.vmap.end());
    }
    for (size_t k = 0; k < src.size(); ++k) {
        tk.msg[k].off = src[k].first;
        tk.msg[k].npart = src[k].second < 0 ? 1 : src[k].second;
        tk.msg[k].fixed = src[k].second < 0 ? 1 : 0;
        tk.msg[k].same_launch = 0;
        tk.msg[k].src_task = from[k];
    }
    npart.clear();
    for (size_t j = 0; j < out_vars.size(); ++j) npart.push_back(tk.msg[JT_MAX_IN + j].npart);
    blocks.clear();
    for (uint32_t f = 0; f < (1u << tk.nF); ++f) blocks.push_back(jtp_make_block(hp, tk, 0u, f));
    return JTP_OK;
}

int jtp_plan_belief_task(const HostPlan &hp, int pnode, JtTask &tk, std::vector<int32_t> &itab,
                         std::vector<JtBlock> &blocks, std::string &err) {
    const PNode &p = hp.pn[pnode];
    memset(&tk, 0, sizeof tk);
    tk.pnode = pnode;
    tk.psi_off = p.unit ? 0 : p.arena_off;
    tk.bel_off = p.arena_off;
    tk.unit = p.unit ? 1 : 0;
    tk.mode = 1;
    std::vector<MsgView> ins, outs;
    std::vector<std::pair<int64_t, int>> src;
    std::vector<int> from;
    neighbour_inputs(hp, p, ins, src, from);
    if ((int)ins.size() > JT_MAX_IN) FAIL(JTP_EUNSUPPORTED, "clique with %zu neighbours", ins.size());
    int real_bits = 0;
    for (int nb : p.nb) real_bits += nb;
    int rc = plan_loops(hp, p, tk, itab, p.nbits, real_bits, ins, outs, 14, err);
    tk.itab_off = 0;
    if (rc != JTP_OK) return rc;
    if (hp.tmix || p.unit) {
        tk.tmap_off = (int64_t)itab.size();
        itab.insert(itab.end(), p.tmap.begin(), p.tmap.end());
        itab.insert(itab.end(), p.vmap.begin(), p.vmap.end());
    }
    for (size_t k = 0; k < src.size(); ++k) {
        tk.msg[k].off = src[k].first;
        tk.msg[k].npart = src[k].second < 0 ? 1 : src[k].second;
        tk.msg[k].fixed = src[k].second < 0 ? 1 : 0;
        tk.msg[k].same_launch = 0;
        tk.msg[k].src_task = from[k];
    }
    blocks.clear();
    for (uint32_t f = 0; f < (1u << tk.nF); ++f) blocks.push_back(jtp_make_block(hp, tk, 0u, f));
    return JTP_OK;
}


namespace {
template <typename It>
void json_list(std::ostringstream &o, It a, It b) {
    o << "[";
    for (It i = a; i != b; ++i) {
        if (i != a) o << ",";
        o << (long long)*i;
    }
    o << "]";
}
template <typename V>
void json_vec(std::ostringstream &o, const V &v) { json_list(o, v.begin(), v.end()); }

void json_msg(std::ostringstream &o, const JtMsg &m, int nF) {
    o << "{\"off\":" << m.off << ",\"npart\":" << m.npart << ",\"pstride\":" << m.pstride
      << ",\"nfree\":" << m.nfree << ",\"lds_off\":" << m.lds_off << ",\"e_w\":";
    json_list(o, m.e_w, m.e_w + 2);
    o << ",\"t_w\":";
    json_list(o, m.t_w, m.t_w + 8);
    o << ",\"red_e\":" << m.red_e << ",\"red_lane\":" << m.red_lane << ",\"red_wave\":" << m.red_wave
      << ",\"e_dep\":" << m.e_dep << ",\"same_launch\":" << m.same_launch << ",\"fixed\":" << m.fixed << ",\"f_w\":";
    json_list(o, m.f_w, m.f_w + nF);
    o << ",\"f_p\":";
    json_list(o, m.f_p, m.f_p + nF);
    o << ",\"free_pos\":";
    json_list(o, m.free_pos, m.free_pos + m.nfree);
    o << "}";
}
}

static std::string json_escape(const std::string &s) {
    std::string o;
    for (char c : s) {
        if (c == '"' || c == '\\') o += '\\', o += c;
        else if ((unsigned char)c < 0x20) o += ' ';
        else o += c;
    }
    return o;
}

void jtp_plan_to_json(HostPlan &hp, bool with_tasks) {
    std::ostringstream o;
    o << "{\"version\":1,\"dtype\":" << hp.dtype << ",\"VEC\":" << hp.VEC << ",\"EB\":" << hp.EB << ",\"TB\":" << hp.TB
      << ",\"n_cliques\":" << hp.n_cliques << ",\"n_ranks\":" << hp.n_ranks << ",\"rank\":" << hp.rank
      << ",\"root\":" << hp.root << ",\"arena_elems\":" << hp.arena_elems << ",\"msg_doubles\":" << hp.msg_doubles
      << ",\"dbg_base\":" << hp.dbg_base << ",\"max_lds\":" << hp.max_lds << ",\"alg_bytes\":" << (long long)hp.alg_bytes
      << ",\"staging_bytes\":" << (long long)hp.staging_bytes << ",\"table_bytes\":" << (long long)hp.table_bytes
      << ",\"compact\":" << (hp.compact ? 1 : 0) << ",\"tmix\":" << (hp.tmix ? 1 : 0) << ",\"host_table_elems\":" << (long long)hp.host_table_elems
      << ",\"multiset\":" << (hp.multiset ? 1 : 0) << ",\"alg_table_bytes\":" << (long long)hp.alg_table_bytes
      << ",\"alg_msg_bytes\":" << (long long)hp.alg_msg_bytes
      << ",\"n_messages\":" << hp.n_messages << ",\"n_tasks\":" << hp.tasks.size()
      << ",\"n_blocks\":" << hp.blocks.size() << ",\"tmix_compact\":" << (hp.tmix_compact ? 1 : 0) << ",\"lean\":" << (hp.lean ? 1 : 0) << ",\"has_unit\":" << (hp.has_unit ? 1 : 0)
      << ",\"lean_refused\":\"" << json_escape(hp.lean_refused) << "\",\"fix_doubles\":" << hp.fix_doubles << ",\"scratch_elems\":" << hp.scratch_elems << ",\"alg_bytes_full\":" << (long long)hp.alg_bytes_full;
    o << ",\"statics\":[";
    for (size_t i = 0; i < hp.statics.size(); ++i) {
        const PStatic &st = hp.statics[i];
        if (i) o << ",";
        o << "{\"pnode\":" << st.pnode << ",\"nbits\":" << st.nbits << ",\"off\":" << st.off << ",\"vars\":";
        json_vec(o, st.vars);
        o << ",\"pos\":";
        json_vec(o, st.pos);
        o << ",\"nb\":";
        json_vec(o, st.nb);
        o << "}";
    }
    o << "],\"pnodes\":[";
    for (size_t i = 0; i < hp.pn.size(); ++i) {
        const PNode &p = hp.pn[i];
        if (i) o << ",";
        o << "{\"real\":" << p.real << ",\"parent\":" << p.parent << ",\"psep\":" << p.psep << ",\"depth\":" << p.depth
          << ",\"owner\":" << p.owner << ",\"nbits\":" << p.nbits << ",\"arena_off\":" << p.arena_off
          << ",\"phys_elems\":" << p.phys_elems << ",\"pad_mask\":" << p.pad_mask << ",\"tmix\":" << (p.tmix ? 1 : 0) << ",\"trow\":" << p.trow
          << ",\"tpad_mask\":" << p.tpad_mask << ",\"tsplit\":" << p.tsplit << ",\"tsplit_lb\":" << p.tsplit_lb << ",\"tmap_off\":" << p.tmap_off << ",\"layout\":" << p.layout << ",\"collect_task\":" << p.collect_task << ",\"distribute_task\":" << p.distribute_task
          << ",\"unit\":" << (p.unit ? 1 : 0) << ",\"stat\":" << p.stat << ",\"cover\":";
        json_vec(o, p.cover);
        o << ",\"down_tasks\":";
        json_vec(o, p.down_tasks);
        if (hp.tmix || p.unit) {
            o << ",\"tmap\":";
            json_vec(o, p.tmap);
            o << ",\"vmap\":";
            json_vec(o, p.vmap);
        }
        o << ",\"bitw\":";
        json_vec(o, p.bitw);
        o << ",\"group_mask\":";
        json_vec(o, p.group_mask);
        o << ",\"group_pos\":";
        json_vec(o, p.group_pos);
        o << ",\"group_card\":";
        json_vec(o, p.group_card);
        {
            std::vector<int> cards;
            for (int v : p.vars) cards.push_back(hp.card[v]);
            o << ",\"card\":";
            json_vec(o, cards);
        }
        o << ",\"vars\":";
        json_vec(o, p.vars);
        o << ",\"pos\":";
        json_vec(o, p.pos);
        o << ",\"nb\":";
        json_vec(o, p.nb);
        o << ",\"children\":";
        json_vec(o, p.children);
        o << "}";
    }
    o << "],\"pack\":[";
    for (size_t i = 0; i < hp.pack.size(); ++i) {
        const JtPackDesc &pd = hp.pack[i];
        if (i) o << ",";
        o << "{\"pos\":";
        json_list(o, pd.pos, pd.pos + pd.nvars);
        o << ",\"nb\":";
        json_list(o, pd.nb, pd.nb + pd.nvars);
        o << ",\"card\":";
        json_list(o, pd.card, pd.card + pd.nvars);
        o << ",\"dstride\":";
        json_list(o, pd.dstride, pd.dstride + pd.nvars);
        o << ",\"dmod\":";
        json_list(o, pd.dmod, pd.dmod + pd.nvars);
        o << ",\"split_var\":" << pd.split_var << ",\"split_lb\":" << pd.split_lb << ",\"split_ds2\":" << pd.split_ds2 << ",\"split_mod2\":" << pd.split_mod2;
        o << ",\"phys_elems\":" << pd.phys_elems << "}";
    }
    o << "],\"pseps\":[";
    for (size_t i = 0; i < hp.ps.size(); ++i) {
        const PSep &s = hp.ps[i];
        if (i) o << ",";
        o << "{\"node\":" << s.node << ",\"child\":" << s.child << ",\"parent\":" << s.parent << ",\"nbits\":" << s.nbits
// ... 118 lines not shown
```

junction-tree_amd/csrc/jtp_plan.h:

```cpp
#pragma once
#include <stdint.h>
#include <string>
#include <vector>

#include "../../include/jtprop.h"
#include "jtp_internal.h"

struct PNode {
    int real = -1;
    std::vector<int> vars;
    std::vector<int> pos, nb;
    int nbits = 0;
    int parent = -1;
    int psep = -1;
    std::vector<int> children;
    int depth = 0;
    int layout = 0;
    int owner = 0;
    int64_t arena_off = -1;
    std::vector<int64_t> bitw;
    std::vector<uint32_t> group_mask;
    std::vector<int> group_pos, group_card;
    uint32_t pad_mask = 0;
    int64_t phys_elems = 0;
// ... 33 lines not shown
    int64_t blk_off = 0;
    int nblocks = 0;
    int lds_bytes = 0;
    double alg_bytes = 0;
};

struct CommOp {
    int send = 0;
    int psep = 0;
    int up = 0;
    int peer = 0;
    int64_t off = 0;
    int64_t count = 0;
};

struct Step {
    int kind = 0;
    int first = 0, count = 0;
};

struct Segment {
    int phase = 0;
    int first_launch = 0, n_launch = 0;
    int64_t blk_off = 0;
    int nblocks = 0;
    int lds_bytes = 0;
    int ticket_idx = 0;
};

struct PStatic {
    int pnode = -1;
    std::vector<int> vars, pos, nb;
    int nbits = 0;
    int64_t off = -1;
};

struct VirtualFill { JtPackDesc d; };

struct HostPlan;
JtBlock jtp_make_block(const HostPlan &hp, const JtTask &tk, uint32_t task_index, uint32_t chunk);
void jtp_make_lean(const HostPlan &hp, JtTask &tk, std::vector<int32_t> &itab, bool readout = false);

struct PlanKnobs {
    int debug = 0;
    int layout_policy = -1;
    int reduce_min = -1;
    double target_blocks_c = 1024.0, target_blocks_d = 1024.0;
    bool target_set = false;
    int min_block_log2 = 13, max_block_log2 = 16;
    int multi_min_block_log2 = 16;
    int max_block_log2_d = 15;
    double tiny_level_elems = 2097152.0;
    int force_level_launches = 0, force_flow = 0, fake_comm = 0;
    unsigned flow_debug = 0;
    int flow_tickets = 0;
    int no_compact = 0;
    int search_all = 1;
    int no_search = 0;
    int roctx = 0;
    int longest_first = 1;
    int lane_low = 2;
    int top_min_loop = 3;
    int top_loop2 = 2;
    double top_rows2 = 2048.0;
    double top_share = 0.12;
    double settle_level_elems = 8388608.0;
    int no_tmix = 0;
    int no_tsplit = 0;
    double tmix_fill = 0.6;
    int esum_always = 0;
    double keep_rows_mb = 128.0;
    int no_ef_share = 0;
    int unit_joint_down = 0;
    int no_vgroups = 0;
    int keep_invalid = 0;
    int no_unit = 0;
    int no_fold = 0;
    int fold = -1;
    int fold_slots = 1024;
    int no_lean = 0;
    double unit_ratio = 4.0;
    int marg_group = JT_MAX_OUT;
    int marg_block_log2 = 0;
    int merge_phases = -1;
};
PlanKnobs jtp_read_knobs();

struct HostPlan {
    PlanKnobs knobs;
    int n_vars = 0, n_cliques = 0, n_nodes = 0, dtype = 0, n_ranks = 1, rank = 0, n_batch = 1;
    int device = 0;
    uint32_t flags = 0;
    int lds_budget = 0, block_log2 = 0, layout_policy = 0;
    std::vector<int> card, vbits;
    std::vector<std::vector<int>> node_vars;
    std::vector<int> parent_clique, parent_sep, owner;
    int VEC = 4, EB = 2, TB = 10;
    int root = 0;
    std::vector<PNode> pn;
    std::vector<PSep> ps;
    std::vector<int> sep_of_node;
    std::vector<JtTask> tasks;
    std::vector<std::vector<int>> task_producers;
    std::vector<int> task_variant;
    std::vector<Launch> launches;
    std::vector<JtBlock> blocks;
    std::vector<int32_t> itab;
    std::vector<uint32_t> block_chunk;
    std::vector<JtBlock> init_blocks[2];
    std::vector<uint32_t> init_chunk[2];
    std::vector<VirtualFill> virtual_fills;
    std::vector<PStatic> statics;
    int64_t fix_doubles = 0;
    std::vector<JtPackDesc> stat_pack;
    struct FoldReq { int task = -1, j = 0, npart = 0, out_bits = 0; int64_t off = 0; };
    std::vector<int32_t> fold_key;
    std::vector<int32_t> fold_cliques, fold_var_off, fold_var_ids;
    std::vector<FoldReq> folded;
    bool lean = false;
    std::string lean_refused;
    bool has_unit = false;
    bool unit_dominated = false;
    std::vector<std::vector<int>> cover;
    int64_t scratch_elems = 0;
    double alg_bytes_full = 0;
    std::vector<CommOp> comm;
    std::vector<Step> steps;
    std::vector<Segment> segments;
    std::vector<Step> flow_steps;
    int sync_words = 0;
    std::vector<JtPackDesc> pack;
    int64_t arena_elems = 0;
    double host_table_elems = 0;
    bool compact = true;
    bool tmix_compact = false;
    bool tmix = false;
    int64_t msg_doubles = 0;
    int64_t dbg_base = -1;
    int max_lds = 0;
    bool chain_plan = false;
    double alg_bytes = 0;
    double alg_table_bytes = 0, alg_msg_bytes = 0;
    bool multiset = false;
    double staging_bytes = 0;
    double table_bytes = 0;
    int n_messages = 0;
    std::string json;
};

int jtp_build_plan(const jtp_tree_desc *desc, HostPlan &hp, std::string &err);

int jtp_plan_marginal_task(const HostPlan &hp, int pnode, const std::vector<std::vector<int>> &out_vars,
                           JtTask &task, std::vector<int32_t> &itab, std::vector<int> &out_bits, std::vector<int> &npart,
                           std::vector<JtBlock> &blocks, std::string &err, bool with_neighbours = false);

int jtp_plan_belief_task(const HostPlan &hp, int pnode, JtTask &task, std::vector<int32_t> &itab,
                         std::vector<JtBlock> &blocks, std::string &err);

void jtp_plan_to_json(HostPlan &hp, bool with_tasks);
```

junction-tree_amd/junctiontree_amd/_capi.py:

```python

import ctypes as C
import os

_HERE = os.path.dirname(os.path.abspath(__file__))
LIB_PATH = os.path.join(_HERE, "lib", "libjtprop.so")
LIB_PATH = os.environ.get("JTPROP_LIB", LIB_PATH)

JTP_OK, JTP_EINVAL, JTP_EHIP, JTP_ECOMM, JTP_ENOMEM, JTP_EUNSUPPORTED = 0, -1, -2, -3, -4, -5
JTP_F32, JTP_F64 = 0, 1
JTP_PLAN_ONLY = 1
JTP_SPLIT_VARIANTS = 2
JTP_KEEP_ROOT = 4
JTP_LEVEL_LAUNCHES = 8
JTP_SHARE_POTENTIALS = 32
JTP_FLOW_TICKETS = 16
JTP_MULTISET = 64
JTP_NO_COMPACT = 128
N_VARIANTS = 23
MAX_VARS = 32


class TreeDesc(C.Structure):
    _fields_ = [
        ("struct_size", C.c_int32),
        ("n_vars", C.c_int32),
        ("var_card", C.POINTER(C.c_int32)),
        ("n_cliques", C.c_int32),
        ("n_nodes", C.c_int32),
        ("node_var_off", C.POINTER(C.c_int32)),
        ("node_var_ids", C.POINTER(C.c_int32)),
        ("parent_clique", C.POINTER(C.c_int32)),
        ("parent_sep", C.POINTER(C.c_int32)),
        ("dtype", C.c_int32),
        ("device", C.c_int32),
        ("n_batch", C.c_int32),
        ("n_ranks", C.c_int32),
        ("rank", C.c_int32),
        ("clique_owner", C.POINTER(C.c_int32)),
        ("flags", C.c_uint32),
        ("lds_budget", C.c_int32),
        ("block_log2", C.c_int32),
        ("layout_policy", C.c_int32),
        ("cover_off", C.POINTER(C.c_int32)),
        ("cover_ids", C.POINTER(C.c_int32)),
        ("fold_n", C.c_int32),
        ("fold_pad", C.c_int32),
        ("fold_cliques", C.POINTER(C.c_int32)),
        ("fold_var_off", C.POINTER(C.c_int32)),
        ("fold_var_ids", C.POINTER(C.c_int32)),
    ]


class Factor(C.Structure):
    _fields_ = [
        ("host", C.c_void_p),
        ("n_vars", C.c_int32),
        ("dtype", C.c_int32),
        ("var_ids", C.POINTER(C.c_int32)),
        ("shape", C.POINTER(C.c_int64)),
    ]


class Stats(C.Structure):
    _fields_ = [
        ("struct_size", C.c_int32),
        ("n_launches", C.c_int32),
        ("n_messages", C.c_int32),
        ("n_tasks", C.c_int32),
        ("algorithmic_bytes", C.c_double),
        ("collect_ms", C.c_double),
        ("distribute_ms", C.c_double),
        ("kernel_ms", C.c_double * 32),
        ("kernel_bytes", C.c_double * 32),
        ("kernel_launches", C.c_int32 * 32),
        ("flow_fallbacks", C.c_int32),
        ("launch_mode", C.c_int32),
        ("tickets_used", C.c_int32),
        ("flow_propagates", C.c_int32),
        ("device_bytes", C.c_double),
        ("storage_dtype", C.c_int32),
        ("foreign_seen", C.c_int32),
        ("f64_flops", C.c_double),
        ("f64_insts", C.c_double),
        ("algorithmic_bytes_full", C.c_double),
        ("fixed_bytes", C.c_double),
        ("n_unit_cliques", C.c_int32),
        ("n_static_tables", C.c_int32),
        ("flight_board", C.c_int32),
        ("lean_refused", C.c_int32),
    ]


class JtpError(RuntimeError):
    """HIP / RCCL / allocation failure reported by libjtprop."""


class UnsupportedStructure(ValueError):
    """JTP_EUNSUPPORTED: a well-formed structure outside the engine's limits (a table beyond 2^31 entries, sub-boxes that
    no layout fits into the LDS of a CU, ...).  A ValueError, as every structural refusal is."""


_lib = None

SYMBOLS = {
    "jtp_plan_create": (C.c_int, [C.POINTER(TreeDesc), C.POINTER(C.c_void_p)]),
    "jtp_plan_destroy": (None, [C.c_void_p]),
    "jtp_plan_describe": (C.c_char_p, [C.c_void_p]),
    "jtp_set_potential": (C.c_int, [C.c_void_p, C.c_int32, C.c_int32, C.c_void_p,
                                    C.POINTER(C.c_int64), C.c_int32]),
    "jtp_set_potential_product": (C.c_int, [C.c_void_p, C.c_int32, C.c_int32, C.c_int32, C.POINTER(Factor)]),
    "jtp_set_potential_products": (C.c_int, [C.c_void_p, C.c_int32, C.c_int32, C.c_void_p, C.c_void_p, C.c_void_p]),
    "jtp_fill_synthetic": (C.c_int, [C.c_void_p, C.c_int32, C.c_uint64, C.POINTER(C.c_double)]),
    "jtp_set_evidence": (C.c_int, [C.c_void_p, C.c_int32, C.c_int32, C.POINTER(C.c_int32), C.POINTER(C.c_int32)]),
    "jtp_propagate": (C.c_int, [C.c_void_p, C.c_int32, C.c_int32]),
    "jtp_sync": (C.c_int, [C.c_void_p]),
    "jtp_get_belief": (C.c_int, [C.c_void_p, C.c_int32, C.c_int32, C.c_void_p, C.c_int32]),
    "jtp_get_marginal": (C.c_int, [C.c_void_p, C.c_int32, C.c_int32, C.POINTER(C.c_int32),
                                   C.c_int32, C.POINTER(C.c_double)]),
    "jtp_get_marginals": (C.c_int, [C.c_void_p, C.c_int32, C.c_int32, C.POINTER(C.c_int32), C.POINTER(C.c_int32),
                                    C.POINTER(C.c_int32), C.POINTER(C.c_int64), C.POINTER(C.c_double)]),
    "jtp_get_z": (C.c_int, [C.c_void_p, C.c_int32, C.POINTER(C.c_double)]),
    "jtp_set_profiling": (C.c_int, [C.c_void_p, C.c_int32]),
    "jtp_set_profiling_granularity": (C.c_int, [C.c_void_p, C.c_int32]),
    "jtp_set_profiling_stride": (C.c_int, [C.c_void_p, C.c_int32]),
    "jtp_region_begin": (C.c_int, [C.c_void_p]),
    "jtp_region_end": (C.c_int, [C.c_void_p, C.POINTER(C.c_double)]),
    "jtp_get_stats": (C.c_int, [C.c_void_p, C.POINTER(Stats)]),
    "jtp_get_launch_ms": (C.c_int, [C.c_void_p, C.POINTER(C.c_double), C.c_int32]),
    "jtp_debug_read_msg": (C.c_int, [C.c_void_p, C.c_int32, C.c_int64, C.c_int64, C.POINTER(C.c_double)]),
    "jtp_debug_set": (C.c_int, [C.c_void_p, C.c_char_p, C.c_int64]),
    "jtp_kernel_name": (C.c_char_p, [C.c_int32]),
    "jtp_comm_unique_id": (C.c_int, [C.c_void_p]),
    "jtp_comm_init": (C.c_int, [C.c_int32, C.c_int32, C.c_void_p, C.c_int32]),
    "jtp_comm_destroy": (C.c_int, []),
    "jtp_comm_info": (C.c_int, [C.POINTER(C.c_int32), C.POINTER(C.c_int32), C.POINTER(C.c_int32)]),
    "jtp_comm_selftest": (C.c_int, [C.c_int32]),
    "jtp_device_count": (C.c_int, [C.POINTER(C.c_int32)]),
    "jtp_device_memory": (C.c_int, [C.c_int32, C.POINTER(C.c_uint64), C.POINTER(C.c_uint64)]),
    "jtp_host_alloc": (C.c_int, [C.POINTER(C.c_void_p), C.c_size_t]),
    "jtp_host_free": (C.c_int, [C.c_void_p]),
    "jtp_last_error": (C.c_char_p, []),
    "jtp_version": (C.c_char_p, []),
}


def lib():
    global _lib
    if _lib is not None:
        return _lib
    if not os.path.exists(LIB_PATH):
        raise ImportError(
            "libjtprop.so not found at %s: build it with `python junction-tree_amd/build.py` "
            "(hipcc --offload-arch=gfx950).  There is no CPU fallback." % LIB_PATH)
    handle = C.CDLL(LIB_PATH)
    for name, (restype, argtypes) in SYMBOLS.items():
        try:
            fn = getattr(handle, name)
        except AttributeError:
            if "JTPROP_LIB" in os.environ:
                continue
            raise
        fn.restype = restype
        fn.argtypes = argtypes
    _lib = handle
    return _lib


def check(rc):
    if rc == JTP_OK:
        return
    msg = lib().jtp_last_error().decode("utf-8", "replace")
    if rc == JTP_EUNSUPPORTED:
        raise UnsupportedStructure(msg)
    if rc == JTP_EINVAL:
        raise ValueError(msg)
    if rc == JTP_ENOMEM:
        raise MemoryError(msg)
    raise JtpError(msg)


def device_count():
    n = C.c_int32(0)
    rc = lib().jtp_device_count(C.byref(n))
    return n.value if rc == JTP_OK else 0
```

junction-tree_amd/junctiontree_amd/engine.py:

```python

import ctypes as C
import json

import numpy as np

from . import _capi

__all__ = ["Plan", "flatten_tree", "plan_for", "cached_plan", "clear_plan_cache", "plan_cache_info", "set_plan_cache_budget"]


def flatten_tree(tree):
    order, parent, parent_sep, children = [], {}, {}, {}
    stack = [(tree, -1, -1)]
    while stack:
        sub, par, sep = stack.pop()
        c = sub[0]
        if c in parent:
            raise ValueError("clique index %r appears twice in the tree" % (c,))
        order.append(c)
        parent[c], parent_sep[c] = par, sep
        children[c] = [(entry[0], entry[1][0]) for entry in sub[1:]]
        for entry in reversed(sub[1:]):
            stack.append((entry[1], c, entry[0]))
    return order, parent, parent_sep, children
# ... 243 lines not shown
    def propagate(self, batch_begin=0, batch_end=None, sync=True):
        end = self.n_batch if batch_end is None else batch_end
        _capi.check(self._lib.jtp_propagate(self._handle, batch_begin, end))
        if sync:
            self.sync()

    def sync(self):
        _capi.check(self._lib.jtp_sync(self._handle))
        self.__dict__.pop("_uploads", None)

    def belief(self, node, batch=0, dtype=np.float64, out=None):
        if out is None:
            out = np.empty(self.node_shape[node], dtype=dtype)
        elif out.shape != tuple(self.node_shape[node]) or not out.flags["C_CONTIGUOUS"] or out.dtype not in (np.float32, np.float64):
            raise ValueError("`out` must be a C-contiguous float32/float64 array of shape %r" % (tuple(self.node_shape[node]),))
        host_dtype = _capi.JTP_F32 if out.dtype == np.float32 else _capi.JTP_F64
        _capi.check(self._lib.jtp_get_belief(self._handle, batch, self.abi_of[node],
                                             out.ctypes.data_as(C.c_void_p), host_dtype))
        return out

    def marginal(self, clique, labels, batch=0):
        shape = tuple(1 if lab in self._trivial else self.card[self.var_id[lab]] for lab in labels)
        labels = [lab for lab in labels if lab not in self._trivial]
        ids = _int_array([self.var_id[lab] for lab in labels])
        out = np.empty(shape, dtype=np.float64)
        _capi.check(self._lib.jtp_get_marginal(self._handle, batch, self.abi_of[clique],
                                               C.cast(ids, C.POINTER(C.c_int32)), len(labels),
                                               out.ctypes.data_as(C.POINTER(C.c_double))))
        return out

    def marginals(self, requests, batch=0):
        n = len(requests)
        if n == 0:
            return []
        cliques = _int_array([self.abi_of[c] for c, _ in requests])
        var_off, var_ids, out_off, shapes = [0], [], [0], []
        for _, labels in requests:
            ids = [self.var_id[lab] for lab in labels if lab not in self._trivial]
            var_ids += ids
            var_off.append(len(var_ids))
            shape = tuple(1 if lab in self._trivial else self.card[self.var_id[lab]] for lab in labels)
            shapes.append(shape)
            out_off.append(out_off[-1] + int(np.prod(shape, dtype=np.int64)) if shape else out_off[-1] + 1)
        flat = np.empty(out_off[-1], dtype=np.float64)
        offs = (C.c_int64 * (n + 1))(*out_off)
        _capi.check(self._lib.jtp_get_marginals(
            self._handle, batch, n, C.cast(cliques, C.POINTER(C.c_int32)),
            C.cast(_int_array(var_off), C.POINTER(C.c_int32)), C.cast(_int_array(var_ids), C.POINTER(C.c_int32)),
            C.cast(offs, C.POINTER(C.c_int64)), flat.ctypes.data_as(C.POINTER(C.c_double))))
        return [flat[out_off[i]:out_off[i + 1]].reshape(shapes[i]).copy() for i in range(n)]

    def z(self, batch=0):
        val = C.c_double(0.0)
        _capi.check(self._lib.jtp_get_z(self._handle, batch, C.byref(val)))
        return val.value

    def set_profiling(self, keep=1, per_launch=False, stride=1):
        _capi.check(self._lib.jtp_set_profiling_granularity(self._handle, 1 if per_launch else 0))
        _capi.check(self._lib.jtp_set_profiling_stride(self._handle, int(stride)))
        _capi.check(self._lib.jtp_set_profiling(self._handle, int(keep)))

    def region_begin(self):
        _capi.check(self._lib.jtp_region_begin(self._handle))

    def region_end(self):
        ms = C.c_double(0.0)
        _capi.check(self._lib.jtp_region_end(self._handle, C.byref(ms)))
        return ms.value

    def debug_set(self, knob, value):
        _capi.check(self._lib.jtp_debug_set(self._handle, knob.encode(), int(value)))

    def launch_ms(self):
        d = self.describe()
        n = len(d["launches"])
        buf = (C.c_double * max(n, 1))()
        rc = self._lib.jtp_get_launch_ms(self._handle, buf, n)
        if rc < 0:
            _capi.check(rc)
        return [dict(phase=L["phase"], level=L["level"], variant=L["variant"], nblocks=L["nblocks"],
                     ntasks=len(L["tasks"]), alg_bytes=L["alg_bytes"], ms=buf[i])
                for i, L in enumerate(d["launches"])]

    def stats(self):
        st = _capi.Stats()
        _capi.check(self._lib.jtp_get_stats(self._handle, C.byref(st)))
        tname = "float" if self.dtype == _capi.JTP_F32 else "double"
        kernels = {}
        for v in range(_capi.N_VARIANTS):
            if st.kernel_launches[v]:
                name = self._lib.jtp_kernel_name(v).decode().replace("<T", "<" + tname)
                k = kernels.setdefault(name, {"launches": 0, "ms": 0.0, "bytes": 0.0})
                k["launches"] += st.kernel_launches[v]
                k["ms"] += st.kernel_ms[v]
                k["bytes"] += st.kernel_bytes[v]
        return {"n_launches": st.n_launches, "n_messages": st.n_messages, "n_tasks": st.n_tasks,
                "algorithmic_bytes": st.algorithmic_bytes, "collect_ms": st.collect_ms,
                "distribute_ms": st.distribute_ms, "kernels": kernels, "flow_fallbacks": st.flow_fallbacks,
                "launch_mode": ("level", "flow", "flow_tickets")[st.launch_mode], "tickets_used": st.tickets_used,
                "flow_propagates": st.flow_propagates, "device_bytes": st.device_bytes, "f64_flops": st.f64_flops, "f64_insts": st.f64_insts,
                "foreign_seen": st.foreign_seen, "algorithmic_bytes_full": st.algorithmic_bytes_full, "fixed_bytes": st.fixed_bytes,
                "n_unit_cliques": st.n_unit_cliques, "n_static_tables": st.n_static_tables, "flight_board": st.flight_board}


_DIGEST_LIMIT = 1 << 20

_FACTOR_REC = np.dtype({"names": ["host", "n_vars", "dtype", "var_ids", "shape"], "formats": ["u8", "i4", "i4", "u8", "u8"],
                        "offsets": [0, 8, 12, 16, 24], "itemsize": C.sizeof(_capi.Factor)})


class _FactorTables:

    def __init__(self, plan, key):
        labels, f2c, shapes, all_f32 = key
        self.key = key
        self.labels, self.f2c, self.shapes, self.all_f32 = [list(l) for l in labels], list(f2c), list(shapes), all_f32
        self.np_dtype = np.float32 if all_f32 else np.float64
        n_f = len(labels)
        if len(f2c) != n_f or len(shapes) != n_f:
            raise ValueError("%d factors, %d clique assignments, %d value arrays" % (n_f, len(f2c), len(shapes)))
        pos_of = {c: i for i, c in enumerate(plan.cliques)}
        var_ids, var_off, shape_all = [], [0], []
        sizes = np.empty(n_f, dtype=np.int64)
        for f in range(n_f):
            if len(shapes[f]) != len(labels[f]):
                raise ValueError("factor %d has %d axes but %d variables" % (f, len(shapes[f]), len(labels[f])))
            for ax, lab in enumerate(labels[f]):
                if lab in plan._trivial:
                    if shapes[f][ax] != 1:
                        raise ValueError("axis %d of factor %d belongs to variable %r of cardinality 1 but has length %d"
                                         % (ax, f, lab, shapes[f][ax]))
                    continue
                try:
                    var_ids.append(plan.var_id[lab])
                except KeyError as exc:
                    raise KeyError(exc.args[0])
                shape_all.append(shapes[f][ax])
            var_off.append(len(var_ids))
            sizes[f] = int(np.prod(shapes[f], dtype=np.int64)) if len(shapes[f]) else 1
        self._var_ids = np.asarray(var_ids + [0], dtype=np.int32)
        self._shape = np.asarray(shape_all + [0], dtype=np.int64)
        var_off = np.asarray(var_off, dtype=np.int64)
        small = sizes * np.dtype(self.np_dtype).itemsize <= _DIGEST_LIMIT
        self.small_idx = np.flatnonzero(small)
        self.big_idx = np.flatnonzero(~small)
        self.small_off = np.zeros(n_f + 1, dtype=np.int64)
        np.cumsum(np.where(small, sizes, 0), out=self.small_off[1:])
        self.seg_start = self.small_off[self.small_idx]
        self.f_pos = np.asarray([pos_of[c] for c in f2c], dtype=np.int64)
        self.order = np.argsort(self.f_pos, kind="stable")
        n_c = len(plan.cliques)
        self.cliques = np.asarray([plan.abi_of[c] for c in plan.cliques], dtype=np.int32)
        self.factor_off = np.zeros(n_c + 1, dtype=np.int32)
        np.cumsum(np.bincount(self.f_pos, minlength=n_c), out=self.factor_off[1:])
        recs = np.zeros(max(n_f, 1), dtype=_FACTOR_REC)
        o = self.order
        recs["n_vars"][:n_f] = (var_off[1:] - var_off[:-1])[o]
        recs["dtype"][:n_f] = _capi.JTP_F32 if all_f32 else _capi.JTP_F64
        recs["var_ids"][:n_f] = self._var_ids.ctypes.data + 4 * var_off[:-1][o]
        recs["shape"][:n_f] = self._shape.ctypes.data + 8 * var_off[:-1][o]
        self.recs = recs
        self.n_f = n_f
        self.prev = None
        self.all_small_alike = bool(n_f > 0 and len(self.big_idx) == 0 and len(shapes[0]) >= 1 and all(tuple(sh) == tuple(shapes[0]) for sh in shapes))
        self.src = (None, None)
        self.is_small = small
        self.mine = np.asarray([plan.owns(c) for c in plan.cliques], dtype=bool)

    def stage(self, plan, arrs, named=None):
        n_f, item = self.n_f, np.dtype(self.np_dtype).itemsize
        dirty = np.ones(len(self.cliques), dtype=bool)
        if named is not None and self.prev is not None and not isinstance(named, str):
            idx = np.unique(np.asarray(list(named), dtype=np.int64))
            if len(idx) and (idx[0] < 0 or idx[-1] >= n_f):
                raise IndexError("changed: factor index out of range [0, %d)" % n_f)
            flat = self.prev
            for i in idx:
                if self.is_small[i]:
                    a = np.asarray(arrs[i])
                    if a.size != self.small_off[i + 1] - self.small_off[i]:
                        raise ValueError("factor %d changed its shape" % i)
                    flat[self.small_off[i]:self.small_off[i + 1]] = a.reshape(-1)
            dirty[:] = False
            dirty[self.f_pos[idx]] = True
            dirty[self.f_pos[self.big_idx]] = True
# ... 228 lines not shown
```

Measured before the change: 5406 GB/s.

## Add eight-slot deep LDS ring variant for merged flow propagate kernel

```diff
diff --git a/include/jtprop.h b/include/jtprop.h
--- a/include/jtprop.h
+++ b/include/jtprop.h
@@ -97,6 +97,8 @@
 
 const char *jtp_plan_describe(jtp_plan *plan);
 
+int jtp_plan_ring_slots(jtp_plan *plan);
+
 
 int jtp_set_potential(jtp_plan *plan, int32_t batch, int32_t node, const void *host,
                       const int64_t *shape, int32_t host_dtype);
diff --git a/junction-tree_amd/build.py b/junction-tree_amd/build.py
--- a/junction-tree_amd/build.py
+++ b/junction-tree_amd/build.py
@@ -6,7 +6,7 @@
 CSRC = os.path.join(HERE, "csrc")
 LIBDIR = os.path.join(HERE, "junctiontree_amd", "lib")
 LIB = os.path.join(LIBDIR, "libjtprop.so")
-INST = ["jtp_inst_%s_%s.hip" % (fam, t) for fam in ("both", "bothm", "level", "mixc", "mix", "flow", "multi", "shape") for t in ("f32", "f64")]
+INST = ["jtp_inst_%s_%s.hip" % (fam, t) for fam in ("both", "deep", "bothm", "level", "mixc", "mix", "flow", "multi", "shape") for t in ("f32", "f64")]
 SOURCES = ["jtp_plan.cpp", "jtp_engine.hip"] + INST
 DEPS = SOURCES + ["jtp_internal.h", "jtp_plan.h", "jtp_kernels.hip.h", os.path.join("..", "..", "include", "jtprop.h")]
 
diff --git a/junction-tree_amd/csrc/jtp_engine.hip b/junction-tree_amd/csrc/jtp_engine.hip
--- a/junction-tree_amd/csrc/jtp_engine.hip
+++ b/junction-tree_amd/csrc/jtp_engine.hip
@@ -180,7 +180,8 @@
         }
         return nullptr;
     }
-    static fn get_flow(int phase, bool chain, int tmix, bool marg) {
+    static fn get_flow(int phase, bool chain, int tmix, bool marg, bool deep = false) {
+        if (deep && phase == 2 && !tmix && !marg) return jt_propagate_flow_deep<T>;
         if (tmix == 2) return phase == 0 ? jt_collect_flow_mix<T, true> : jt_distribute_flow_mix<T, true>;
         if (tmix) return phase == 0 ? jt_collect_flow_mix<T, false> : jt_distribute_flow_mix<T, false>;
         if (phase == 2) return marg ? jt_propagate_flow_marg<T> : jt_propagate_flow<T>;
@@ -565,12 +566,16 @@
 
 static int zero_padding(jtp_plan *pl, double *msg, int nsets, hipStream_t s, int halves = 3);
 
-int jtp_plan_create(const jtp_tree_desc *desc, jtp_plan **out) {
+static int plan_create(const jtp_tree_desc *desc, jtp_plan **out, int max_ring_slots);
+
+int jtp_plan_create(const jtp_tree_desc *desc, jtp_plan **out) { return plan_create(desc, out, JT_DEEP_SLOTS); }
+
+static int plan_create(const jtp_tree_desc *desc, jtp_plan **out, const int max_ring_slots) {
     if (!out) return set_err(JTP_EINVAL, "null output pointer");
     *out = nullptr;
     jtp_plan *pl = new jtp_plan();
     std::string err;
-    int rc = jtp_build_plan(desc, pl->hp, err);
+    int rc = jtp_build_plan(desc, pl->hp, err, max_ring_slots);
     for (int attempt = 1; attempt < 4 && rc == JTP_EUNSUPPORTED && desc; ++attempt) {
         jtp_tree_desc again = *desc;
         const bool relayout = (attempt & 1) && (desc->flags & JTP_MULTISET) && desc->layout_policy == 0;
@@ -583,7 +588,7 @@
         std::string err2;
         delete pl;
         pl = new jtp_plan();
-        const int rc2 = jtp_build_plan(&again, pl->hp, err2);
+        const int rc2 = jtp_build_plan(&again, pl->hp, err2, max_ring_slots);
         if (rc2 == JTP_OK) rc = rc2;
         else if (rc2 != JTP_EUNSUPPORTED) rc = rc2, err = err2;
     }
@@ -598,7 +603,7 @@
             std::string err2;
             delete pl;
             pl = new jtp_plan();
-            const int rc2 = jtp_build_plan(&again, pl->hp, err2);
+            const int rc2 = jtp_build_plan(&again, pl->hp, err2, max_ring_slots);
             if (rc2 == JTP_OK) rc = rc2, pl->widened = true;
             else if (rc2 != JTP_EUNSUPPORTED) rc = rc2, err = err2;
         }
@@ -607,7 +612,7 @@
         jtp_tree_desc again = *desc;
         again.cover_off = again.cover_ids = nullptr;
         jtp_plan *fresh = nullptr;
-        const int rc2 = jtp_plan_create(&again, &fresh);
+        const int rc2 = plan_create(&again, &fresh, max_ring_slots);
         delete pl;
         if (rc2 == JTP_OK) {
             fresh->hp.lean_refused = err.empty() ? std::string("unsupported") : err;
@@ -665,6 +670,17 @@
     pl->roctx = hp.knobs.roctx != 0;
     if (pl->roctx) roctx::load();
     CREATE_TRY(hipSetDevice(hp.device));
+    if (hp.deep_ring()) {
+        const void *f = hp.dtype == JTP_F32 ? (const void *)KernelTable<float>::get_flow(2, false, 0, false, true)
+                                            : (const void *)KernelTable<double>::get_flow(2, false, 0, false, true);
+        int per_cu = 0;
+        const hipError_t oe = hipOccupancyMaxActiveBlocksPerMultiprocessor(&per_cu, f, JT_THREADS, (size_t)hp.max_lds);
+        if (oe != hipSuccess) (void)hipGetLastError();
+        if (oe != hipSuccess || per_cu < 3) {
+            jtp_plan_destroy(pl);
+            return plan_create(desc, out, JT_U);
+        }
+    }
     const int nstreams = pl->multiset ? 1 : std::min(hp.n_batch, 16);
     pl->streams.resize(nstreams);
     for (auto &s : pl->streams) CREATE_TRY(hipStreamCreateWithFlags(&s, hipStreamNonBlocking));
@@ -772,7 +788,7 @@
             CREATE_TRY(raise_lds(kfunc(v), hp.max_lds));
         }
         for (int ph = 0; ph < 3; ++ph) {
-            const void *f = hp.dtype == JTP_F32 ? (const void *)KernelTable<float>::get_flow(ph, pl->chain, mixk(hp), pl->marg_tasks) : (const void *)KernelTable<double>::get_flow(ph, pl->chain, mixk(hp), pl->marg_tasks);
+            const void *f = hp.dtype == JTP_F32 ? (const void *)KernelTable<float>::get_flow(ph, pl->chain, mixk(hp), pl->marg_tasks, hp.deep_ring()) : (const void *)KernelTable<double>::get_flow(ph, pl->chain, mixk(hp), pl->marg_tasks, hp.deep_ring());
             CREATE_TRY(raise_lds(f, hp.max_lds));
         }
     }
@@ -810,6 +826,8 @@
     if (pl->hp.json.empty()) jtp_plan_to_json(pl->hp, pl->hp.tasks.size() <= 20000);
     return pl->hp.json.c_str();
 }
+
+int jtp_plan_ring_slots(jtp_plan *pl) { return pl ? pl->hp.ring_slots : 0; }
 
 
 static int check_writable(jtp_plan *pl, int batch) {
@@ -1564,10 +1582,10 @@
                 fl.blk_base = (uint32_t)sg.blk_off;
                 fl.ticket_base = ticket_run * (uint32_t)sg.nblocks;
                 if (hp.dtype == JTP_F32)
-                    hipLaunchKernelGGL(KernelTable<float>::get_flow(sg.phase, pl->chain, mixk(hp), pl->marg_tasks), dim3(sg.nblocks), dim3(JT_THREADS), sg.lds_bytes, s, pl->d_tasks,
+                    hipLaunchKernelGGL(KernelTable<float>::get_flow(sg.phase, pl->chain, mixk(hp), pl->marg_tasks, hp.deep_ring()), dim3(sg.nblocks), dim3(JT_THREADS), sg.lds_bytes, s, pl->d_tasks,
                                        pl->d_blocks + sg.blk_off, pl->d_itab, (const float *)bb.psi, (float *)bb.bel, bb.msg, fl);
                 else
-                    hipLaunchKernelGGL(KernelTable<double>::get_flow(sg.phase, pl->chain, mixk(hp), pl->marg_tasks), dim3(sg.nblocks), dim3(JT_THREADS), sg.lds_bytes, s, pl->d_tasks,
+                    hipLaunchKernelGGL(KernelTable<double>::get_flow(sg.phase, pl->chain, mixk(hp), pl->marg_tasks, hp.deep_ring()), dim3(sg.nblocks), dim3(JT_THREADS), sg.lds_bytes, s, pl->d_tasks,
                                        pl->d_blocks + sg.blk_off, pl->d_itab, (const double *)bb.psi, (double *)bb.bel, bb.msg, fl);
             } else if (st.kind == 0) {
                 const Launch &L = hp.launches[st.first];
diff --git a/junction-tree_amd/csrc/jtp_inst_deep_f32.hip b/junction-tree_amd/csrc/jtp_inst_deep_f32.hip
--- /dev/null
+++ b/junction-tree_amd/csrc/jtp_inst_deep_f32.hip
@@ -0,0 +1,3 @@
+#define JT_INST_TU
+#include "jtp_kernels.hip.h"
+JT_INST_DEEP(, float)
diff --git a/junction-tree_amd/csrc/jtp_inst_deep_f64.hip b/junction-tree_amd/csrc/jtp_inst_deep_f64.hip
--- /dev/null
+++ b/junction-tree_amd/csrc/jtp_inst_deep_f64.hip
@@ -0,0 +1,3 @@
+#define JT_INST_TU
+#include "jtp_kernels.hip.h"
+JT_INST_DEEP(, double)
diff --git a/junction-tree_amd/csrc/jtp_internal.h b/junction-tree_amd/csrc/jtp_internal.h
--- a/junction-tree_amd/csrc/jtp_internal.h
+++ b/junction-tree_amd/csrc/jtp_internal.h
@@ -10,9 +10,15 @@
 #define JT_MAX_FREE 13
 #define JT_THREADS 256
 #define JT_REDUCE_ENTRIES 64
+#ifndef JT_U
+#define JT_U 4
+#endif
 #ifndef JT_RING_BYTES
 #define JT_RING_BYTES 16384
 #endif
+#define JT_DEEP_SLOTS 8
+#define JT_DEEP_RING_BYTES (JT_DEEP_SLOTS * 4096)
+#define JT_DEEP_LDS_CAP ((160 * 1024 / 3 - 4096) & ~511)
 #define JT_STAGE_SCRATCH 2048
 #define JT_MIN_ITER_LOG2 2
 #ifndef JT_MIN_LOOP_LOG2
diff --git a/junction-tree_amd/csrc/jtp_kernels.hip.h b/junction-tree_amd/csrc/jtp_kernels.hip.h
--- a/junction-tree_amd/csrc/jtp_kernels.hip.h
+++ b/junction-tree_amd/csrc/jtp_kernels.hip.h
@@ -10,9 +10,6 @@
 #endif
 #ifndef JT_UT
 #define JT_UT 4
-#endif
-#ifndef JT_U
-#define JT_U 4
 #endif
 
 template <typename T> struct JtVec;
@@ -163,7 +160,7 @@
     return g;
 }
 
-template <typename T, int NIN, int NOUT, int MODE, bool FLOW = false, bool EARLY_FLUSH = (MODE == 0), bool TMIX = false, bool KEEP = false, bool UNIT = false, bool BEL = !UNIT, bool VG = false>
+template <typename T, int NIN, int NOUT, int MODE, bool FLOW = false, bool EARLY_FLUSH = (MODE == 0), bool TMIX = false, bool KEEP = false, bool UNIT = false, bool BEL = !UNIT, bool VG = false, int RU = JT_U>
 __device__ __forceinline__ void jt_pass(const JtTask &tk, const JtBlock &bk, const int *__restrict__ itab,
                                         const T *__restrict__ psi_arena, T *__restrict__ bel_arena,
                                         double *__restrict__ msg_arena, const JtFlow &fl,
@@ -172,9 +169,10 @@
     constexpr int EB = (VEC == 4) ? 2 : 1;
     constexpr int NMSG = NIN + NOUT;
     constexpr int NPAR = NIN - NOUT * (MODE == 1);
-    constexpr int U = JT_U;
+    constexpr int U = RU;
     constexpr int UT = TMIX ? JT_UT : U;
-    static_assert((U == 4 || U == 8) && (1 << JT_MIN_ITER_LOG2) == 4 && JT_RING_BYTES == U * 4096, "the loop groups below are written out for four or eight slots");
+    static_assert((U == 4 || U == 8) && (1 << JT_MIN_ITER_LOG2) == 4, "the loop groups below are written out for four or eight slots");
+    static_assert(U * 4096 == (U == JT_U ? JT_RING_BYTES : JT_DEEP_RING_BYTES), "planner and kernels agree on the ring's size");
     using VT = typename JtVec<T>::type;
     extern __shared__ __attribute__((aligned(16))) char smem[];
 
@@ -1657,7 +1655,7 @@
     }
 }
 
-template <typename T, bool FOLD>
+template <typename T, bool FOLD, int RU = JT_U>
 __device__ __forceinline__ void jt_propagate_flow_body(const JtTask *__restrict__ tasks, const JtBlock *__restrict__ blk,
                                                        const int *__restrict__ itab, const T *__restrict__ psi, T *__restrict__ bel,
                                                        double *__restrict__ msg, const JtFlow &fl, uint32_t *flow_ctl) {
@@ -1677,22 +1675,22 @@
     }
     if (tk.mode == 0) {
         switch (tk.n_in) {
-            case 0: jt_pass<T, 0, 1, 0, true, true, false, true>(tk, bk, itab, psi, bel, msg, fl, ticket, flow_ctl, t_entry); break;
-            case 1: jt_pass<T, 1, 1, 0, true, true, false, true>(tk, bk, itab, psi, bel, msg, fl, ticket, flow_ctl, t_entry); break;
-            case 2: jt_pass<T, 2, 1, 0, true, true, false, true>(tk, bk, itab, psi, bel, msg, fl, ticket, flow_ctl, t_entry); break;
-            default: jt_pass<T, 3, 1, 0, true, true, false, true>(tk, bk, itab, psi, bel, msg, fl, ticket, flow_ctl, t_entry); break;
+            case 0: jt_pass<T, 0, 1, 0, true, true, false, true, false, true, false, RU>(tk, bk, itab, psi, bel, msg, fl, ticket, flow_ctl, t_entry); break;
+            case 1: jt_pass<T, 1, 1, 0, true, true, false, true, false, true, false, RU>(tk, bk, itab, psi, bel, msg, fl, ticket, flow_ctl, t_entry); break;
+            case 2: jt_pass<T, 2, 1, 0, true, true, false, true, false, true, false, RU>(tk, bk, itab, psi, bel, msg, fl, ticket, flow_ctl, t_entry); break;
+            default: jt_pass<T, 3, 1, 0, true, true, false, true, false, true, false, RU>(tk, bk, itab, psi, bel, msg, fl, ticket, flow_ctl, t_entry); break;
         }
         return;
     }
     switch ((tk.n_in - tk.n_out) * 4 + tk.n_out) {
-        case 0: jt_pass<T, 0, 0, 1, true, false, false, true>(tk, bk, itab, psi, bel, msg, fl, ticket, flow_ctl, t_entry); break;
-        case 1: jt_pass<T, 1, 1, 1, true, false, false, true>(tk, bk, itab, psi, bel, msg, fl, ticket, flow_ctl, t_entry); break;
-        case 2: jt_pass<T, 2, 2, 1, true, false, false, true>(tk, bk, itab, psi, bel, msg, fl, ticket, flow_ctl, t_entry); break;
-        case 3: jt_pass<T, 3, 3, 1, true, false, false, true>(tk, bk, itab, psi, bel, msg, fl, ticket, flow_ctl, t_entry); break;
-        case 4: jt_pass<T, 1, 0, 1, true, false, false, true>(tk, bk, itab, psi, bel, msg, fl, ticket, flow_ctl, t_entry); break;
-        case 5: jt_pass<T, 2, 1, 1, true, false, false, true>(tk, bk, itab, psi, bel, msg, fl, ticket, flow_ctl, t_entry); break;
-        case 6: jt_pass<T, 3, 2, 1, true, false, false, true>(tk, bk, itab, psi, bel, msg, fl, ticket, flow_ctl, t_entry); break;
-        default: jt_pass<T, 4, 3, 1, true, false, false, true>(tk, bk, itab, psi, bel, msg, fl, ticket, flow_ctl, t_entry); break;
+        case 0: jt_pass<T, 0, 0, 1, true, false, false, true, false, true, false, RU>(tk, bk, itab, psi, bel, msg, fl, ticket, flow_ctl, t_entry); break;
+        case 1: jt_pass<T, 1, 1, 1, true, false, false, true, false, true, false, RU>(tk, bk, itab, psi, bel, msg, fl, ticket, flow_ctl, t_entry); break;
+        case 2: jt_pass<T, 2, 2, 1, true, false, false, true, false, true, false, RU>(tk, bk, itab, psi, bel, msg, fl, ticket, flow_ctl, t_entry); break;
+        case 3: jt_pass<T, 3, 3, 1, true, false, false, true, false, true, false, RU>(tk, bk, itab, psi, bel, msg, fl, ticket, flow_ctl, t_entry); break;
+        case 4: jt_pass<T, 1, 0, 1, true, false, false, true, false, true, false, RU>(tk, bk, itab, psi, bel, msg, fl, ticket, flow_ctl, t_entry); break;
+        case 5: jt_pass<T, 2, 1, 1, true, false, false, true, false, true, false, RU>(tk, bk, itab, psi, bel, msg, fl, ticket, flow_ctl, t_entry); break;
+        case 6: jt_pass<T, 3, 2, 1, true, false, false, true, false, true, false, RU>(tk, bk, itab, psi, bel, msg, fl, ticket, flow_ctl, t_entry); break;
+        default: jt_pass<T, 4, 3, 1, true, false, false, true, false, true, false, RU>(tk, bk, itab, psi, bel, msg, fl, ticket, flow_ctl, t_entry); break;
     }
 }
 
@@ -1710,6 +1708,14 @@
                                                                         T *__restrict__ bel, double *__restrict__ msg, JtFlow fl) {
     __shared__ uint32_t flow_ctl[28 + 8 * JT_MAX_OUT];
     jt_propagate_flow_body<T, true>(tasks, blk, itab, psi, bel, msg, fl, flow_ctl);
+}
+
+template <typename T>
+__global__ __launch_bounds__(JT_THREADS, 3) void jt_propagate_flow_deep(const JtTask *__restrict__ tasks, const JtBlock *__restrict__ blk,
+                                                                    const int *__restrict__ itab, const T *__restrict__ psi,
+                                                                    T *__restrict__ bel, double *__restrict__ msg, JtFlow fl) {
+    __shared__ uint32_t flow_ctl[28 + 8 * JT_MAX_OUT];
+    jt_propagate_flow_body<T, false, JT_DEEP_SLOTS>(tasks, blk, itab, psi, bel, msg, fl, flow_ctl);
 }
 
 template <typename T>
@@ -2709,6 +2715,7 @@
 #define JT_INST_BOTH(X, T) JT_INST_PROPAGATE(X, T) JT_INST_PROPAGATE_MARG(X, T)
 #define JT_INST_PROPAGATE(X, T) X template __global__ void jt_propagate_flow<T>(JT_KARGS(T));
 #define JT_INST_PROPAGATE_MARG(X, T) X template __global__ void jt_propagate_flow_marg<T>(JT_KARGS(T));
+#define JT_INST_DEEP(X, T) X template __global__ void jt_propagate_flow_deep<T>(JT_KARGS(T));
 #define JT_INST_MIX_V(X, T, V)                                                  \
     X template __global__ void jt_collect_level_mix<T, V>(JT_KARGS(T));         \
     X template __global__ void jt_distribute_level_mix<T, V>(JT_KARGS(T));      \
@@ -2728,6 +2735,8 @@
 JT_INST_MULTI(extern, double)
 JT_INST_BOTH(extern, float)
 JT_INST_BOTH(extern, double)
+JT_INST_DEEP(extern, float)
+JT_INST_DEEP(extern, double)
 JT_INST_MIX(extern, float)
 JT_INST_MIX(extern, double)
 JT_INST_MIXC(extern, float)
diff --git a/junction-tree_amd/csrc/jtp_plan.cpp b/junction-tree_amd/csrc/jtp_plan.cpp
--- a/junction-tree_amd/csrc/jtp_plan.cpp
+++ b/junction-tree_amd/csrc/jtp_plan.cpp
@@ -113,6 +113,7 @@
     double share = 1.0;
     double fill = 1.0;
     long lds_cap = 150 * 1024;
+    long ring = JT_RING_BYTES;
     int red_log2 = 6;
     bool chain = false;
     int min_loop_log2 = JT_MIN_ITER_LOG2;
@@ -127,7 +128,7 @@
     const int nL = popc(L);
     if (nL < e.min_loop_log2 || nL > e.max_iter_log2 || popc(F) > JT_MAX_HI) return 1e30;
     const double nwg = std::max(1.0, std::ldexp(e.fill, popc(F))), iters = std::ldexp(1.0, nL);
-    long lds = e.unit ? 0 : JT_RING_BYTES;
+    long lds = e.unit ? 0 : e.ring;
     double stage = 0, flush = 0, red_bytes = 0, epi = 0;
     int n_red = 0;
     for (uint32_t m : ins) {
@@ -170,7 +171,7 @@
     const double epilogues = 1.0;
     const double t_wg = K.wg + (ins.empty() ? 0.0 : K.stage_fix) + stage / K.stage_bw + iters * (e.dist ? K.iter_d : K.iter_c) + epilogues * epi +
                         (outs.empty() ? 0.0 : K.flush_fix) + flush / K.flush_bw;
-    const int per_cu = (int)std::min((long)K.max_cu, std::max(1L, 160L * 1024 / (lds + 128)));
+    const int per_cu = (int)std::min(e.ring > JT_RING_BYTES ? 3L : (long)K.max_cu, std::max(1L, 160L * 1024 / (lds + 128)));
     const double conc = std::max(1.0, 256.0 * per_cu * e.share);
     const double t_lat = std::max(t_wg, nwg * t_wg / conc);
     const double bytes = nwg * (e.unit ? 0.0 : iters * 4096.0 * (e.dist ? 2.0 : 1.0)) + nwg * (0.5 * stage + flush);
@@ -251,7 +252,8 @@
             if (g >> b & 1) return g;
         return 1u << b;
     };
-    const int budget = strict_budget > 0 ? strict_budget : (hp.lds_budget > 0 ? hp.lds_budget : 32 * 1024);
+    int budget = strict_budget > 0 ? strict_budget : (hp.lds_budget > 0 ? hp.lds_budget : 32 * 1024);
+    if (hp.deep_ring() && strict_budget == 0) budget = std::min(budget, JT_DEEP_LDS_CAP - hp.ring_bytes() - JT_STAGE_SCRATCH * (int)ins.size());
     const int PMAX_LOG2 = block_log2 <= 13 ? 6 : 3;
     const uint32_t himask = nbits >= 32 ? 0 : (((1u << nbits) - 1) & ~((1u << TB) - 1));
     uint32_t allout = 0, everyout = himask;
@@ -297,7 +299,9 @@
                 e.max_iter_log2 = std::max(hp.knobs.top_loop2, JT_MIN_LOOP_LOG2);
             }
         }
-        if (hp.lds_budget > 0) e.lds_cap = (tk.unit ? 0 : JT_RING_BYTES) + hp.lds_budget + JT_STAGE_SCRATCH * (long)ins.size();
+        e.ring = hp.ring_bytes();
+        if (hp.lds_budget > 0) e.lds_cap = (tk.unit ? 0 : e.ring) + hp.lds_budget + JT_STAGE_SCRATCH * (long)ins.size();
+        if (hp.deep_ring()) e.lds_cap = std::min(e.lds_cap, (long)JT_DEEP_LDS_CAP);
         uint32_t seen = 0;
         for (int b = TB; b < nbits; ++b)
             if (!(seen >> b & 1)) e.units.push_back(unit(b)), seen |= unit(b);
@@ -329,7 +333,7 @@
         }
         if (best < 0 || best_lds >= lds_of(F)) {
             if (strict_budget > 0) FAIL(JTP_EUNSUPPORTED, "message sub-boxes of one evidence set need %ld bytes of LDS (limit %d)", lds_of(F), strict_budget);
-            if (lds_of(F) + (tk.unit ? 0 : JT_RING_BYTES) + JT_STAGE_SCRATCH * (long)ins.size() + 4096 <= 160 * 1024 && max_free(F) <= JT_MAX_FREE) break;
+            if (lds_of(F) + (tk.unit ? 0 : hp.ring_bytes()) + JT_STAGE_SCRATCH * (long)ins.size() + 4096 <= 160 * 1024 && max_free(F) <= JT_MAX_FREE) break;
             if (!down_to_four) {
                 down_to_four = true;
                 continue;
@@ -411,7 +415,7 @@
     for (int b : Rb) loopmask |= 1u << b;
     for (int b : Ab) loopmask |= 1u << b;
 
-    int lds = tk.unit ? 0 : JT_RING_BYTES;
+    int lds = tk.unit ? 0 : hp.ring_bytes();
     std::vector<std::vector<int>> slotw;
     auto fill_msg = [&](JtMsg &jm, const MsgView &mv, bool is_out) {
         std::vector<int> sw(32, 0);
@@ -660,6 +664,7 @@
     k.fold = geti("JTP_FOLD", -1);
     if (k.fold == 0) k.no_fold = 1;
     k.fold_slots = geti("JTP_FOLD_SLOTS", 1024);
+    k.ring_slots = geti("JTP_RING_SLOTS", 0);
     return k;
 }
 
@@ -710,7 +715,8 @@
 
 int PlanBuilder::block_log2_for(int phase, int level, int owner, bool tiny_rule) const {
         if (hp.block_log2 > 0) return std::max(hp.block_log2, hp.TB);
-        const double target = (phase == 0 ? hp.knobs.target_blocks_c : hp.knobs.target_blocks_d) * (hp.unit_dominated && !hp.knobs.target_set ? 2.0 : 1.0);
+        const double target = (phase == 0 ? hp.knobs.target_blocks_c : hp.knobs.target_blocks_d) * (hp.unit_dominated && !hp.knobs.target_set ? 2.0 : 1.0) *
+                              (hp.deep_ring() && !hp.knobs.target_set ? 0.75 : 1.0);
         const int lgmin = hp.multiset && hp.n_batch > JT_MSETS ? hp.knobs.multi_min_block_log2 : hp.knobs.min_block_log2;
         const int lgmax = phase == 1 && !hp.multiset ? hp.knobs.max_block_log2_d : hp.knobs.max_block_log2;
         const double tiny = hp.knobs.tiny_level_elems;
@@ -1068,7 +1074,9 @@
             if (!(grouped >> b & 1)) e.units.push_back(1u << b);
         if (hp.compact || p.unit) e.fill = std::ldexp(e.fill, -(e.nbits - std::max(bit, TB)));
         std::sort(e.units.begin(), e.units.end());
-        if (hp.lds_budget > 0) e.lds_cap = (p.unit ? 0 : JT_RING_BYTES) + hp.lds_budget + JT_STAGE_SCRATCH * 4L;
+        e.ring = hp.ring_bytes();
+        if (hp.lds_budget > 0) e.lds_cap = (p.unit ? 0 : e.ring) + hp.lds_budget + JT_STAGE_SCRATCH * 4L;
+        if (hp.deep_ring()) e.lds_cap = std::min(e.lds_cap, (long)JT_DEEP_LDS_CAP);
         uint32_t stat_mask = 0;
         if (has_static)
             for (int v : p.cover) {
@@ -1170,6 +1178,7 @@
         for (int c = 0; c < NP; ++c) tiny += lvl_elems[1][hp.pn[c].owner][hp.pn[c].depth] <= hp.knobs.tiny_level_elems;
         hp.chain_plan = 2 * tiny > NP;
     }
+    if (hp.deep_ring() && hp.knobs.ring_slots != JT_DEEP_SLOTS && (hp.chain_plan || hp.unit_dominated)) return JTP_REPLAN;
     for (int c = 0; c < NP; ++c) {
         PNode &p = hp.pn[c];
         std::vector<int> host = p.real >= 0 ? hp.node_vars[p.real] : p.vars;
@@ -2174,7 +2183,7 @@
         sg.lds_bytes = std::max(sg.lds_bytes, L.lds_bytes);
     }
     {
-        const bool merge = hp.knobs.merge_phases == 1 ||
+        const bool merge = hp.knobs.merge_phases == 1 || (hp.deep_ring() && hp.knobs.ring_slots == JT_DEEP_SLOTS && hp.knobs.merge_phases != 0) ||
                            (hp.knobs.merge_phases < 0 && !hp.multiset && !hp.chain_plan && !hp.tmix &&
                             (hp.staging_bytes * 8.0 <= hp.table_bytes || hp.unit_dominated));
         if (merge && !hp.multiset && !hp.tmix) {
@@ -2235,7 +2244,36 @@
     return JTP_OK;
 }
 
-int jtp_build_plan(const jtp_tree_desc *d, HostPlan &hp, std::string &err) {
+static bool deep_ring_ok(const HostPlan &hp) {
+    if (hp.n_ranks != 1 || hp.multiset || hp.tmix) return false;
+    if (hp.segments.size() != 1 || hp.segments[0].phase != 2) return false;
+    if (hp.max_lds > JT_DEEP_LDS_CAP) return false;
+    for (const JtTask &tk : hp.tasks)
+        if (tk.fold) return false;
+    if (hp.knobs.ring_slots == JT_DEEP_SLOTS) return true;
+    return !hp.chain_plan && !hp.unit_dominated && hp.staging_bytes * 8.0 <= hp.table_bytes;
+}
+
+int jtp_build_plan(const jtp_tree_desc *d, HostPlan &hp, std::string &err, int max_ring_slots) {
+    const PlanKnobs knobs = jtp_read_knobs();
+    const int asked = knobs.ring_slots;
+    if (asked != 0 && asked != JT_U && asked != JT_DEEP_SLOTS) {
+        err = "JTP_RING_SLOTS must be 4 or 8";
+        return JTP_EINVAL;
+    }
+    const bool try_deep = JT_U != JT_DEEP_SLOTS && max_ring_slots >= JT_DEEP_SLOTS && asked != JT_U && d && d->n_ranks == 1 &&
+                          !(d->flags & (JTP_MULTISET | JTP_LEVEL_LAUNCHES | JTP_SPLIT_VARIANTS)) && d->fold_n == 0 &&
+                          !knobs.force_level_launches && !(knobs.debug & 1);
+    if (try_deep) {
+        HostPlan deep;
+        deep.ring_slots = JT_DEEP_SLOTS;
+        std::string err2;
+        if (PlanBuilder(d, deep, err2).run() == JTP_OK && deep_ring_ok(deep)) {
+            hp = std::move(deep);
+            return JTP_OK;
+        }
+    }
+    hp = HostPlan();
     return PlanBuilder(d, hp, err).run();
 }
 
@@ -2401,7 +2439,7 @@
     o << "{\"version\":1,\"dtype\":" << hp.dtype << ",\"VEC\":" << hp.VEC << ",\"EB\":" << hp.EB << ",\"TB\":" << hp.TB
       << ",\"n_cliques\":" << hp.n_cliques << ",\"n_ranks\":" << hp.n_ranks << ",\"rank\":" << hp.rank
       << ",\"root\":" << hp.root << ",\"arena_elems\":" << hp.arena_elems << ",\"msg_doubles\":" << hp.msg_doubles
-      << ",\"dbg_base\":" << hp.dbg_base << ",\"max_lds\":" << hp.max_lds << ",\"alg_bytes\":" << (long long)hp.alg_bytes
+      << ",\"dbg_base\":" << hp.dbg_base << ",\"max_lds\":" << hp.max_lds << ",\"ring_slots\":" << hp.ring_slots << ",\"alg_bytes\":" << (long long)hp.alg_bytes
       << ",\"staging_bytes\":" << (long long)hp.staging_bytes << ",\"table_bytes\":" << (long long)hp.table_bytes
       << ",\"compact\":" << (hp.compact ? 1 : 0) << ",\"tmix\":" << (hp.tmix ? 1 : 0) << ",\"host_table_elems\":" << (long long)hp.host_table_elems
       << ",\"multiset\":" << (hp.multiset ? 1 : 0) << ",\"alg_table_bytes\":" << (long long)hp.alg_table_bytes
diff --git a/junction-tree_amd/csrc/jtp_plan.h b/junction-tree_amd/csrc/jtp_plan.h
--- a/junction-tree_amd/csrc/jtp_plan.h
+++ b/junction-tree_amd/csrc/jtp_plan.h
@@ -139,6 +139,7 @@
     double unit_ratio = 4.0;
     int marg_group = JT_MAX_OUT;
     int marg_block_log2 = 0;
+    int ring_slots = 0;
     int merge_phases = -1;
 };
 PlanKnobs jtp_read_knobs();
@@ -195,6 +196,9 @@
     int64_t msg_doubles = 0;
     int64_t dbg_base = -1;
     int max_lds = 0;
+    int ring_slots = JT_U;
+    bool deep_ring() const { return ring_slots != JT_U; }
+    int ring_bytes() const { return deep_ring() ? JT_DEEP_RING_BYTES : JT_RING_BYTES; }
     bool chain_plan = false;
     double alg_bytes = 0;
     double alg_table_bytes = 0, alg_msg_bytes = 0;
@@ -205,7 +209,8 @@
     std::string json;
 };
 
-int jtp_build_plan(const jtp_tree_desc *desc, HostPlan &hp, std::string &err);
+#define JTP_REPLAN 1000
+int jtp_build_plan(const jtp_tree_desc *desc, HostPlan &hp, std::string &err, int max_ring_slots = 8);
 
 int jtp_plan_marginal_task(const HostPlan &hp, int pnode, const std::vector<std::vector<int>> &out_vars,
                            JtTask &task, std::vector<int32_t> &itab, std::vector<int> &out_bits, std::vector<int> &npart,
diff --git a/junction-tree_amd/junctiontree_amd/_capi.py b/junction-tree_amd/junctiontree_amd/_capi.py
--- a/junction-tree_amd/junctiontree_amd/_capi.py
+++ b/junction-tree_amd/junctiontree_amd/_capi.py
@@ -106,6 +106,7 @@
     "jtp_plan_create": (C.c_int, [C.POINTER(TreeDesc), C.POINTER(C.c_void_p)]),
     "jtp_plan_destroy": (None, [C.c_void_p]),
     "jtp_plan_describe": (C.c_char_p, [C.c_void_p]),
+    "jtp_plan_ring_slots": (C.c_int, [C.c_void_p]),
     "jtp_set_potential": (C.c_int, [C.c_void_p, C.c_int32, C.c_int32, C.c_void_p,
                                     C.POINTER(C.c_int64), C.c_int32]),
     "jtp_set_potential_product": (C.c_int, [C.c_void_p, C.c_int32, C.c_int32, C.c_int32, C.POINTER(Factor)]),
diff --git a/junction-tree_amd/junctiontree_amd/engine.py b/junction-tree_amd/junctiontree_amd/engine.py
--- a/junction-tree_amd/junctiontree_amd/engine.py
+++ b/junction-tree_amd/junctiontree_amd/engine.py
@@ -349,6 +349,10 @@
                      ntasks=len(L["tasks"]), alg_bytes=L["alg_bytes"], ms=buf[i])
                 for i, L in enumerate(d["launches"])]
 
+    def ring_slots(self):
+        fn = getattr(self._lib, "jtp_plan_ring_slots", None)
+        return fn(self._handle) if fn is not None else 4
+
     def stats(self):
         st = _capi.Stats()
         _capi.check(self._lib.jtp_get_stats(self._handle, C.byref(st)))
@@ -367,7 +371,7 @@
                 "launch_mode": ("level", "flow", "flow_tickets")[st.launch_mode], "tickets_used": st.tickets_used,
                 "flow_propagates": st.flow_propagates, "device_bytes": st.device_bytes, "f64_flops": st.f64_flops, "f64_insts": st.f64_insts,
                 "foreign_seen": st.foreign_seen, "algorithmic_bytes_full": st.algorithmic_bytes_full, "fixed_bytes": st.fixed_bytes,
-                "n_unit_cliques": st.n_unit_cliques, "n_static_tables": st.n_static_tables, "flight_board": st.flight_board}
+                "n_unit_cliques": st.n_unit_cliques, "n_static_tables": st.n_static_tables, "flight_board": st.flight_board, "ring_slots": self.ring_slots()}
 
 
 _DIGEST_LIMIT = 1 << 20
```

After: 5265 GB/s. 0.974x the previous value.
